# TonyLianLong/LLM-groundedDiffusion

Measured on AMD Instinct MI355X. Metric: images/sec (50-step SD1.5 512^2, LMD+ guidance), higher is better.
Workload: dtype fp16; 1 GPU; LMD+ stage 2, 4 cached 2-box layouts/GPU/step (lmd_v0.1 cache), 50 DDIM steps, 512x512, sd14_gligen (SD1.4+GLIGEN architecture, seeded random weights), VAE decodes included; per-box masks = box masks; mask_refinement=box, layouts_per_gpu=4, num_inference_steps=50, parallelism=dp1, rccl_ranks=1, lanes_per_gpu=4, gemm_tuning=throughput

## Files before the change

include/lgd_hip.h:

```cpp
#ifndef LGD_HIP_H
#define LGD_HIP_H
#include <stdint.h>
#ifdef __cplusplus
extern "C" {
#endif

#define LGD_ABI_VERSION 12
int lgd_abi_version(void);
int lgd_set_option(const char* name, int value);
int lgd_get_option(const char* name);

#define LGD_EPI_GEGLU 1
#define LGD_EPI_OUT_F32 2
#define LGD_EPI_RES_F32 4
#define LGD_EPI_ROWNORM 8

typedef struct LgdGemmDesc {
  const void* a0;
  const void* a1;
  int64_t lda0, lda1;
  int32_t c0, c1;
  int32_t taps;
  int32_t hin, win, hout, wout, stride, ups;
  const void* w;
  int64_t ldw;
  int32_t M, N, K;
  int32_t nb_o, nb_i;
  int64_t a_bs_o, a_bs_i, w_bs_o, w_bs_i, c_bs_o, c_bs_i, r_bs_o, r_bs_i;
  const float* bias;
  const float* bias2;
  const void* res;
  int64_t ldr;
  float alpha;
  int32_t epi;
  void* c;
  int64_t ldc;
  int32_t splits;
  float* ws;
  int32_t tile;
  int32_t* cnt;
  const float* rowstat;
  const float* colsum;
  int32_t pair;
} LgdGemmDesc;
#define LGD_PAIR_HALF 1
#define LGD_PAIR_DUP 2

int lgd_gemm_f16(const LgdGemmDesc* desc , void* stream);
int lgd_gemm_check(const LgdGemmDesc* desc );

int lgd_conv_in_f16(const float* x_nchw, const void* w, const float* bias, void* y, int B, int Cin,
                    int L, int Cout, void* stream);
int lgd_conv_out_f16(const void* x, const void* w, const float* bias, float* y_nchw, int B, int Cin,
                     int L, int Cout, float out_scale, void* stream);

int lgd_groupnorm_f16(const void* x0, const void* x1, int c0, int c1, int B, int HW, int G,
                      float eps, const float* gamma, const float* beta, int silu, void* y,
                      float* part, int nchunk, float* stats, void* stream);
int lgd_groupnorm_pair_f16(const void* x0, const void* x1, int c0, int c1, int B, int HW, int G,
                           float eps, const float* gamma, const float* beta, int silu, void* y,
                           float* part, int nchunk, int pair, void* stream);
int lgd_groupnorm_bwd_f16(const void* gy, const void* x0, const void* x1, int c0, int c1, int B,
                          int HW, int G, const float* gamma, const float* beta, int silu,
                          const float* stats, void* gx0, void* gx1, float* part, int nchunk,
                          int accumulate, void* stream);

int lgd_layernorm_f16(const void* x, int64_t ldx, void* y, int64_t ldy, int rows, int C, float eps,
                      const float* gamma, const float* beta, float* stats, int rows_per_batch,
                      int64_t x_bs, int64_t y_bs, void* stream);
int lgd_layernorm_pair_f16(const void* x, int64_t ldx, void* y, int64_t ldy, int rows, int C, float eps,
                           const float* gamma, const float* beta, float* stats, int rows_per_batch,
                           int64_t x_bs, int64_t y_bs, int pair, void* stream);
int lgd_layernorm_bwd_f16(const void* gy, int64_t ldgy, const void* x, int64_t ldx, void* gx,
                          int64_t ldgx, int rows, int C, const float* gamma, const float* stats,
                          int rows_per_batch, int64_t gy_bs, int64_t x_bs, int64_t gx_bs,
                          int accumulate, void* stream);

int lgd_attn_fwd_f16(const void* q, int64_t ldq, int64_t q_bs, const void* k, int64_t ldk,
                     int64_t k_bs, const void* v, int64_t ldv, int64_t v_bs, void* o, int64_t ldo,
                     int64_t o_bs, float* lse, int B, int H, int Sq, int Sk, int d, float scale,
                     void* stream);
int lgd_attn_fwd_pair_f16(const void* q, int64_t ldq, int64_t q_bs, const void* k, int64_t ldk,
                          int64_t k_bs, const void* v, int64_t ldv, int64_t v_bs, void* o, int64_t ldo,
                          int64_t o_bs, float* lse, int B, int H, int Sq, int Sk, int d, float scale,
                          int pair, void* stream);
int lgd_attn_bwd_f16(const void* q, int64_t ldq, int64_t q_bs, const void* k, int64_t ldk,
                     int64_t k_bs, const void* v, int64_t ldv, int64_t v_bs, const void* o,
                     int64_t ldo, int64_t o_bs, const void* go, int64_t ldgo, int64_t go_bs,
                     const float* lse, float* delta, void* gq, int64_t ldgq, int64_t gq_bs, void* gk,
                     int64_t ldgk, int64_t gk_bs, void* gv, int64_t ldgv, int64_t gv_bs, int B, int H,
                     int Sq, int Sk, int d, float scale, void* stream);
int lgd_attn_bwd_keys_f16(const void* q, int64_t ldq, int64_t q_bs, const void* k, int64_t ldk,
                          int64_t k_bs, const void* v, int64_t ldv, int64_t v_bs, const void* o,
                          int64_t ldo, int64_t o_bs, const void* go, int64_t ldgo, int64_t go_bs,
                          const float* lse, float* delta, void* gq, int64_t ldgq, int64_t gq_bs, void* gk,
                          int64_t ldgk, int64_t gk_bs, void* gv, int64_t ldgv, int64_t gv_bs, int B, int H,
                          int Sq, int Sk, int Sk_grad, int d, float scale, void* stream);

int lgd_cross_attn_fwd_f16(const void* q, int64_t ldq, int64_t q_bs, const void* k, int64_t ldk,
                           int64_t k_bs, const void* v, int64_t ldv, int64_t v_bs, void* o,
                           int64_t ldo, int64_t o_bs, float* probs, int tok, int cond_only, int B,
                           int H, int Sq, int Sk, int d, float scale, void* stream);
int lgd_cross_attn_bwd_f16(const void* q, int64_t ldq, int64_t q_bs, const void* k, int64_t ldk,
                           int64_t k_bs, const void* v, int64_t ldv, int64_t v_bs, const void* go,
                           int64_t ldgo, int64_t go_bs, const float* gp, void* gq, int64_t ldgq,
                           int64_t gq_bs, int B, int H, int Sq, int Sk, int d, float scale,
                           void* stream);

int lgd_attn_causal_fwd_f16(const void* q, int64_t ldq, int64_t q_bs, const void* k, int64_t ldk, int64_t k_bs,
                            const void* v, int64_t ldv, int64_t v_bs, void* o, int64_t ldo, int64_t o_bs, int B,
                            int H, int S, int d, float scale, void* stream);

#define LGD_ATTN_OP_FWD 0
#define LGD_ATTN_OP_BWD 1
#define LGD_ATTN_OP_CROSS_BWD 2
int lgd_attn_plan(int op, int B, int H, int Sq, int Sk, int Sk_grad, int d, int probs, int causal, int pair,
                  int aligned);

int lgd_geglu_bwd_f16(const void* h, const void* gy, void* gh, int64_t rows, int n, void* stream);
int lgd_geglu_fwd_f16(const void* h, void* y, int64_t rows, int n, void* stream);
int lgd_quick_gelu_f16(const void* x, void* y, int64_t n, void* stream);
int lgd_nchw_to_nhwc8_f16(const float* x, void* y, int B, int C, int HW, void* stream);
int lgd_add_f16(const void* a, const void* b, void* y, int64_t n, void* stream);
int lgd_scale_f16(const void* x, void* y, float alpha, int64_t n, void* stream);
int lgd_image_u8_to_nhwc8_f16(const void* img, const float* table, void* y, int B, int HW, void* stream);
int lgd_vae_sample_f32(const void* moments, const float* noise, float* out, int B, int z, int HW, float scale,
                       void* stream);
int lgd_softmax_rows_f16(const void* x, void* y, int64_t rows, int n, float scale, void* stream);
int lgd_upsample2x_bwd_f16(const void* gy, void* gx, int B, int H, int W, int C, void* stream);

int lgd_cfg_ddim_step_f32(const float* eps, const float* x, float* x_out, const float* coef_table,
                          const int32_t* dyn, const float* frozen_ref, const float* mask, float* hist,
                          int B, int C, int HW, void* stream);
int lgd_cfg_multistep_step_f32(const float* eps, const float* x, float* x_out, float* x0_prev,
                               const float* coef_table, const int32_t* dyn, const float* frozen_ref,
                               const float* mask, float* hist, int B, int C, int HW, void* stream);
int lgd_cfg_plms_step_f32(const float* eps, const float* x, float* x_out, float* ets, float* cur_sample,
                          const float* coef_table, const int32_t* dyn, float* hist, int B, int C, int HW, void* stream);
int lgd_multidiffusion_step_f32(const float* eps, float* x_in, float* latent, const float* masks, const float* bg,
                                const float* noise, const int32_t* picks, const float* coef_table, const int32_t* dyn,
                                float* hist, int P, int Pp, int C, int HW, int n_steps, int n_boot, int prep,
                                void* stream);
int lgd_multidiffusion_views_f32(const float* eps, float* x_in, float* latent, float* value, float* count,
                                 const float* masks, const float* bg, const float* noise, const int32_t* picks,
                                 const float* coef_table, const int32_t* dyn, float* hist, int P, int Pp, int C, int Hp,
                                 int Wp, int V, int v0, int nv, int nvc, int n_steps, int n_boot, int indep_uncond,
                                 int normalization, int prep, void* stream);
int lgd_scale_rows_f32(const float* x, float* out, const float* table, const int32_t* dyn, int row_stride, int col,
                       int64_t n, int reps, void* stream);
int lgd_axpy_f32(const float* g, float* x, const float* coef_table, const int32_t* step_idx, int col,
                 const float* active, int64_t per_sample, int64_t n, void* stream);
int lgd_select_row_f32(const float* table, const int32_t* idx, float* out, int n, void* stream);

#define LGD_ACT_GELU 1
#define LGD_ACT_RELU 2
int lgd_act_f16(const void* x, void* y, int64_t n, int mode, void* stream);
int lgd_sam_relpos_qkv_f16(const void* qkv, const float* qkv_bias, const float* rel_h, const float* rel_w, int B,
                           int Hs, int Ws, int window, int NH, int d, int DA, float scale, void* qa, void* ka,
                           void* va, void* stream);
int lgd_sam_window_merge_f16(const void* oa, void* out, int B, int Hs, int Ws, int window, int NH, int d, int DA,
                             void* stream);

int lgd_ca_energy_f32(const float* const* maps, float* const* gmaps, const int32_t* map_hw,
                      const int32_t* items, const float* coefs, const float* masks, const float* refs,
                      int64_t refs_step_stride, const int32_t* dyn, const int32_t* groups, int n_groups,
                      int n_items, int n_samples, int H, int T, int max_hw, float grad_scale, float* partial,
                      float* loss, void* stream);

int lgd_boxdiff_energy_f32(const float* const* maps, float* const* gmaps, int n_maps, int side, const int32_t* items,
                           const float* masks, const float* smooth, const int32_t* groups, int n_samples,
                           int max_items, int H, int T, float loss_scale, float grad_scale, float* loss, void* stream);

#ifdef __cplusplus
}
#endif
#endif
```

llm-groundeddiffusion_amd/_lib.py:

```python
import ctypes as C
import os

import torch

_HERE = os.path.dirname(os.path.abspath(__file__))
LIB_PATH = os.path.join(_HERE, "liblgd_hip.so")
ABI_VERSION = 12

c_void_p, c_int, c_i64, c_float = C.c_void_p, C.c_int, C.c_int64, C.c_float


class LgdGemmDesc(C.Structure):
    _fields_ = [
        ("a0", c_void_p), ("a1", c_void_p),
        ("lda0", c_i64), ("lda1", c_i64),
        ("c0", C.c_int32), ("c1", C.c_int32),
        ("taps", C.c_int32),
        ("hin", C.c_int32), ("win", C.c_int32), ("hout", C.c_int32), ("wout", C.c_int32),
        ("stride", C.c_int32), ("ups", C.c_int32),
        ("w", c_void_p), ("ldw", c_i64),
        ("M", C.c_int32), ("N", C.c_int32), ("K", C.c_int32),
        ("nb_o", C.c_int32), ("nb_i", C.c_int32),
        ("a_bs_o", c_i64), ("a_bs_i", c_i64), ("w_bs_o", c_i64), ("w_bs_i", c_i64),
        ("c_bs_o", c_i64), ("c_bs_i", c_i64), ("r_bs_o", c_i64), ("r_bs_i", c_i64),
        ("bias", c_void_p), ("bias2", c_void_p),
        ("res", c_void_p), ("ldr", c_i64),
        ("alpha", c_float), ("epi", C.c_int32),
        ("c", c_void_p), ("ldc", c_i64),
        ("splits", C.c_int32), ("ws", c_void_p),
        ("tile", C.c_int32),
        ("cnt", c_void_p),
        ("rowstat", c_void_p), ("colsum", c_void_p),
        ("pair", C.c_int32),
    ]


EPI_GEGLU, EPI_OUT_F32, EPI_RES_F32, EPI_ROWNORM = 1, 2, 4, 8
PAIR_HALF, PAIR_DUP = 1, 2

_P, _I, _L, _F = c_void_p, c_int, c_i64, c_float
SIGNATURES = {
    "lgd_abi_version": [],
    "lgd_set_option": [C.c_char_p, _I],
    "lgd_get_option": [C.c_char_p],
    "lgd_gemm_f16": [C.POINTER(LgdGemmDesc), _P],
    "lgd_gemm_check": [C.POINTER(LgdGemmDesc)],
    "lgd_conv_in_f16": [_P, _P, _P, _P, _I, _I, _I, _I, _P],
    "lgd_conv_out_f16": [_P, _P, _P, _P, _I, _I, _I, _I, _F, _P],
    "lgd_groupnorm_f16": [_P, _P, _I, _I, _I, _I, _I, _F, _P, _P, _I, _P, _P, _I, _P, _P],
    "lgd_groupnorm_pair_f16": [_P, _P, _I, _I, _I, _I, _I, _F, _P, _P, _I, _P, _P, _I, _I, _P],
    "lgd_groupnorm_bwd_f16": [_P, _P, _P, _I, _I, _I, _I, _I, _P, _P, _I, _P, _P, _P, _P, _I, _I, _P],
    "lgd_layernorm_f16": [_P, _L, _P, _L, _I, _I, _F, _P, _P, _P, _I, _L, _L, _P],
    "lgd_layernorm_pair_f16": [_P, _L, _P, _L, _I, _I, _F, _P, _P, _P, _I, _L, _L, _I, _P],
    "lgd_layernorm_bwd_f16": [_P, _L, _P, _L, _P, _L, _I, _I, _P, _P, _I, _L, _L, _L, _I, _P],
    "lgd_attn_fwd_f16": [_P, _L, _L, _P, _L, _L, _P, _L, _L, _P, _L, _L, _P, _I, _I, _I, _I, _I, _F, _P],
    "lgd_attn_fwd_pair_f16": [_P, _L, _L, _P, _L, _L, _P, _L, _L, _P, _L, _L, _P, _I, _I, _I, _I, _I, _F, _I, _P],
    "lgd_attn_bwd_f16": [_P, _L, _L, _P, _L, _L, _P, _L, _L, _P, _L, _L, _P, _L, _L, _P, _P,
                         _P, _L, _L, _P, _L, _L, _P, _L, _L, _I, _I, _I, _I, _I, _F, _P],
    "lgd_attn_bwd_keys_f16": [_P, _L, _L, _P, _L, _L, _P, _L, _L, _P, _L, _L, _P, _L, _L, _P, _P,
                              _P, _L, _L, _P, _L, _L, _P, _L, _L, _I, _I, _I, _I, _I, _I, _F, _P],
    "lgd_cross_attn_fwd_f16": [_P, _L, _L, _P, _L, _L, _P, _L, _L, _P, _L, _L, _P, _I, _I,
                               _I, _I, _I, _I, _I, _F, _P],
    "lgd_cross_attn_bwd_f16": [_P, _L, _L, _P, _L, _L, _P, _L, _L, _P, _L, _L, _P, _P, _L, _L,
                               _I, _I, _I, _I, _I, _F, _P],
    "lgd_geglu_bwd_f16": [_P, _P, _P, _L, _I, _P],
    "lgd_geglu_fwd_f16": [_P, _P, _L, _I, _P],
    "lgd_add_f16": [_P, _P, _P, _L, _P],
    "lgd_softmax_rows_f16": [_P, _P, _L, _I, _F, _P],
    "lgd_scale_f16": [_P, _P, _F, _L, _P],
    "lgd_upsample2x_bwd_f16": [_P, _P, _I, _I, _I, _I, _P],
    "lgd_cfg_ddim_step_f32": [_P, _P, _P, _P, _P, _P, _P, _P, _I, _I, _I, _P],
    "lgd_cfg_multistep_step_f32": [_P, _P, _P, _P, _P, _P, _P, _P, _P, _I, _I, _I, _P],
    "lgd_cfg_plms_step_f32": [_P, _P, _P, _P, _P, _P, _P, _P, _I, _I, _I, _P],
    "lgd_multidiffusion_step_f32": [_P, _P, _P, _P, _P, _P, _P, _P, _P, _P, _I, _I, _I, _I, _I, _I, _I, _P],
    "lgd_multidiffusion_views_f32": [_P] * 12 + [_I] * 14 + [_P],
    "lgd_axpy_f32": [_P, _P, _P, _P, _I, _P, _L, _L, _P],
    "lgd_select_row_f32": [_P, _P, _P, _I, _P],
    "lgd_scale_rows_f32": [_P, _P, _P, _P, _I, _I, _L, _I, _P],
    "lgd_attn_causal_fwd_f16": [_P, _L, _L, _P, _L, _L, _P, _L, _L, _P, _L, _L, _I, _I, _I, _I, _F, _P],
    "lgd_attn_plan": [_I] * 11,
    "lgd_quick_gelu_f16": [_P, _P, _L, _P],
    "lgd_act_f16": [_P, _P, _L, _I, _P],
    "lgd_nchw_to_nhwc8_f16": [_P, _P, _I, _I, _I, _P],
    "lgd_image_u8_to_nhwc8_f16": [_P, _P, _P, _I, _I, _P],
    "lgd_vae_sample_f32": [_P, _P, _P, _I, _I, _I, _F, _P],
    "lgd_sam_relpos_qkv_f16": [_P, _P, _P, _P, _I, _I, _I, _I, _I, _I, _I, _F, _P, _P, _P, _P],
    "lgd_sam_window_merge_f16": [_P, _P, _I, _I, _I, _I, _I, _I, _I, _P],
    "lgd_ca_energy_f32": [_P, _P, _P, _P, _P, _P, _P, _L, _P, _P, _I, _I, _I, _I, _I, _I, _F, _P, _P, _P],
    "lgd_boxdiff_energy_f32": [_P, _P, _I, _I, _P, _P, _P, _P, _I, _I, _I, _I, _F, _F, _P, _P],
}

_lib = None


def load():
    global _lib
    if _lib is not None:
        return _lib
    if not os.path.exists(LIB_PATH):
        raise RuntimeError(
            f"{LIB_PATH} not found: build it with `python __graft_entry__.py` "
            "(there is no CPU/PyTorch fallback for the HIP kernels)")
    lib = C.CDLL(LIB_PATH)
    for name, argtypes in SIGNATURES.items():
        try:
            fn = getattr(lib, name)
        except AttributeError as e:
            raise RuntimeError(f"liblgd_hip.so does not export {name}") from e
        fn.argtypes = argtypes
        fn.restype = c_int
    if lib.lgd_abi_version() != ABI_VERSION:
        raise RuntimeError("liblgd_hip.so ABI version mismatch; rebuild")
    for item in filter(None, os.environ.get("LGD_OPTIONS", "").split(",")):
        name, _, value = item.partition("=")
        check(lib.lgd_set_option(name.strip().encode(), int(value)), f"lgd_set_option({name})")
    _lib = lib
    return lib


_ERR = {-1: "invalid argument", -2: "kernel launch failed", -3: "unsupported shape"}


def check(rc, name):
    if rc != 0:
        raise RuntimeError(f"{name} failed: {_ERR.get(rc, rc)}")
```

llm-groundeddiffusion_amd/csrc/attn.hip:

```cpp
#include <atomic>
#include "common.h"
#include "../../include/lgd_hip.h"
#include "attn_w4.h"
#include "attn_plan.h"
#include <stdlib.h>
#include <string.h>

namespace {

int g_attn32_nw = -1;
int attn32_nw() {
  if (g_attn32_nw < 0) { const char* e = getenv("LGD_ATTN32_NW"); g_attn32_nw = e ? atoi(e) : 8; }
  return g_attn32_nw;
}
int g_attn32_var = 0;
int attn32_var() { return g_attn32_var; }
int g_attn32 = -1;
int attn32_mode() {
  if (g_attn32 < 0) { const char* e = getenv("LGD_ATTN32"); g_attn32 = e ? atoi(e) : 1; }
  return g_attn32;
}

std::atomic<int> g_attn_w4{-1};
int attn_w4_mode() {
// ... 830 lines not shown
    for (int dt = 0; dt < NDT; ++dt)
#pragma unroll
      for (int r = 0; r < 16; ++r)
        if (dt == dt_l && r == r_l) lv = oacc[dt][r];
    l = __shfl(lv, h_l * 32 + qi, 64);
  }
  const int qrow = q0 + qi;
  if (qrow < a.Sq) {
    const float inv = 1.f / l;
    half_t* orow = a.o + (long)b * a.o_bs + (long)qrow * a.ldo + (long)h * d;
#pragma unroll
    for (int dt = 0; dt < NDT; ++dt)
#pragma unroll
      for (int g4 = 0; g4 < 4; ++g4) {
        const int dv = dt * 32 + g4 * 8 + hh * 4;
        if (dv < d) {
          half4_t o;
#pragma unroll
          for (int r = 0; r < 4; ++r) o[r] = (half_t)(oacc[dt][g4 * 4 + r] * inv);
          *reinterpret_cast<half4_t*>(orow + dv) = o;
          if (a.o_dup) *reinterpret_cast<half4_t*>(orow + a.o_dup + dv) = o;
        }
      }
    if (a.lse && hh == 0) {
      float* lp = a.lse + ((long)b * a.H + h) * a.Sq + qrow;
      const float lv2 = m_ref + log2f(l);
      *lp = lv2;
      if (a.lse_dup) lp[a.lse_dup] = lv2;
    }
  }
}

int attn_nw_env() {
  static const int nw_env = [] { const char* e = getenv("LGD_ATTN_NW"); return e ? atoi(e) : 0; }();
  return nw_env;
}
int attn160_wide_env() {
  static const int wide = [] { const char* e = getenv("LGD_ATTN160"); return e ? atoi(e) : 1; }();
  return wide;
}

int attn_dp_of(int d) { return d <= 32 ? 32 : d <= 64 ? 64 : d <= 96 ? 96 : d <= 128 ? 128 : d <= 160 ? 160 : d <= 192 ? 192 : 0; }

int plan_fwd(int B, int H, int Sq, int Sk, int d, bool two_pass) {
  const int DP = attn_dp_of(d);
  if (!DP) return LGD_ERR_UNSUPPORTED;
  if (two_pass) return attn_code(ATTN_FAM_TWOPASS, DP, 0);
  const long blocks256 = (long)((Sq + 255) / 256) * H * B;
  const int w4 = attn_w4_mode();
  if (w4 && d == 40 && (w4 == 2 || (blocks256 >= 256 && Sk >= 256)))
    return attn_code(ATTN_FAM_W4, 64, lgd_attn_w4_pipe() ? 1 : 0);
  if (DP == 64 || DP == 96) {
    const int a32 = attn32_mode();
    const int dk = ((d + 2 + 15) / 16) * 16;
    if (a32 && d % 8 == 0 && (a32 == 2 || (dk == 96 && blocks256 >= 128)) && (dk == 48 || dk == 96)) {
      const int var = attn32_var();
      const int sub = (attn32_nw() == 4 || (a32 != 2 && blocks256 < 256)) ? ATTN32_NW4
                      : var == 1 ? ATTN32_NW8_PF4 : var == 2 ? ATTN32_NW8_FREE : ATTN32_NW8;
      return attn_code(ATTN_FAM_SELF32, dk, sub);
    }
  }
  const int mode = (DP == 64 && d < 48) ? SELF_ONES3 : d < DP ? SELF_ONES : SELF_PLAIN;
  const bool qt2 = (long)((Sq + 127) / 128) * H * B >= 1024 && DP <= 96;
  if (qt2) {
    const int nw_env = attn_nw_env();
    const bool nw8 = nw_env ? nw_env == 8 : ((DP == 64 && d < 48) || DP == 96);
    return attn_code(ATTN_FAM_SELF, DP, 10 * mode + (nw8 && blocks256 >= 512 ? SELF_QT2_NW8 : SELF_QT2));
  }
  if (DP == 160 && attn160_wide_env() && d == DP && Sq >= 256 && (long)H * B * ((Sq + 63) / 64) > 256)
    return attn_code(ATTN_FAM_SELF, DP, 10 * SELF_PLAIN + SELF_QT2_NW8);
  return attn_code(ATTN_FAM_SELF, DP, 10 * mode + SELF_QT1);
}

template <int DP, bool ONES, int NDT>
void launch_self_shape(int shape, const AttnArgs& a, hipStream_t st) {
  const int gz = a.pair ? a.B / 2 : a.B;
  if constexpr (DP <= 96 || (DP == 160 && !ONES)) {
    if (shape == SELF_QT2_NW8) {
      hipLaunchKernelGGL((attn_self_kernel<DP, ONES, 2, NDT, 8>), dim3((a.Sq + 255) / 256, a.H, gz), dim3(512), 0, st, a);
      return;
    }
  }
  if constexpr (DP <= 96) {
    if (shape == SELF_QT2) {
      hipLaunchKernelGGL((attn_self_kernel<DP, ONES, 2, NDT>), dim3((a.Sq + 127) / 128, a.H, gz), dim3(256), 0, st, a);
      return;
    }
  }
  hipLaunchKernelGGL((attn_self_kernel<DP, ONES, 1, NDT>), dim3((a.Sq + 63) / 64, a.H, gz), dim3(256), 0, st, a);
}

template <int DP>
void launch_fwd_code(int code, const AttnArgs& a, hipStream_t st) {
  const int fam = attn_code_fam(code), sub = attn_code_sub(code);
  if (fam == ATTN_FAM_TWOPASS) {
    dim3 grid((a.Sq + 63) / 64, a.H, a.B);
    hipLaunchKernelGGL((attn_fwd_kernel<DP>), grid, dim3(256), 0, st, a);
    return;
  }
  if constexpr (DP == 64 || DP == 96) {
    if (fam == ATTN_FAM_SELF32) {
      constexpr int DK = DP == 64 ? 48 : 96, NDT = DP == 64 ? 2 : 3;
      const int gz = a.pair ? a.B / 2 : a.B;
      auto go = [&](auto kern, int nw) {
        dim3 g32((a.Sq + 32 * nw - 1) / (32 * nw), a.H, gz);
        hipLaunchKernelGGL(kern, g32, dim3(64 * nw), 0, st, a);
      };
      switch (sub) {
        case ATTN32_NW4: go(&attn_self32_kernel<DK, NDT, 4>, 4); return;
        case ATTN32_NW8_PF4: go(&attn_self32_kernel<DK, NDT, 8, 4, true>, 8); return;
        case ATTN32_NW8_FREE: go(&attn_self32_kernel<DK, NDT, 8, 2, false>, 8); return;
        default: go(&attn_self32_kernel<DK, NDT, 8>, 8); return;
      }
    }
  }
  const int mode = sub / 10, shape = sub % 10;
  if constexpr (DP == 64) {
    if (mode == SELF_ONES3) return launch_self_shape<DP, true, 3>(shape, a, st);
  }
  if (mode == SELF_PLAIN) launch_self_shape<DP, false, DP / 16>(shape, a, st);
  else launch_self_shape<DP, true, DP / 16>(shape, a, st);
}

int launch_attn(const AttnArgs& a, hipStream_t st, bool two_pass) {
  AttnW4Args w;
  w.q = a.q; w.ldq = a.ldq; w.q_bs = a.q_bs; w.k = a.k; w.ldk = a.ldk; w.k_bs = a.k_bs;
  w.v = a.v; w.ldv = a.ldv; w.v_bs = a.v_bs; w.o = a.o; w.ldo = a.ldo; w.o_bs = a.o_bs; w.lse = a.lse;
  w.B = a.B; w.H = a.H; w.Sq = a.Sq; w.Sk = a.Sk; w.d = a.d; w.scale_log2 = a.scale_log2;
  w.pair = a.pair; w.o_dup = a.o_dup; w.lse_dup = a.lse_dup;
  const int code = plan_fwd(a.B, a.H, a.Sq, a.Sk, a.d, two_pass);
  if (code < 0) return code;
  if (attn_code_fam(code) == ATTN_FAM_W4) return lgd_attn_w4_launch(w, st, attn_code_sub(code));
  switch (attn_dp_of(a.d)) {
    case 32: launch_fwd_code<32>(code, a, st); break;
    case 64: launch_fwd_code<64>(code, a, st); break;
    case 96: launch_fwd_code<96>(code, a, st); break;
    case 128: launch_fwd_code<128>(code, a, st); break;
    case 160: launch_fwd_code<160>(code, a, st); break;
    default: launch_fwd_code<192>(code, a, st); break;
  }
  return lgd_check_launch();
}

bool bad_view(const void* p, int64_t ld, int64_t bs, int d) {
  return (ld % 8) != 0 || (d % 8) != 0 || (bs % 8) != 0 || (reinterpret_cast<uintptr_t>(p) & 15) != 0;
}
bool bad_out(const void* p, int64_t ld, int64_t bs) {
  return (ld % 4) != 0 || (bs % 4) != 0 || (reinterpret_cast<uintptr_t>(p) & 7) != 0;
}

}

void lgd_gn_set_fused_hw(int hw);
void lgd_gn_set_slab(int on);
void lgd_ln_set_stream(int on);
void lgd_gn_set_apply_wgs(int n);

static std::atomic<int> g_cfg_pair{1};

extern "C" int lgd_get_option(const char* name) {
  if (name && !strcmp(name, "cfg_pair")) return g_cfg_pair.load(std::memory_order_relaxed);
  return LGD_ERR_ARG;
}

extern "C" int lgd_set_option(const char* name, int value) {
  if (!name) return LGD_ERR_ARG;
  if (!strcmp(name, "cfg_pair") && (value == 0 || value == 1)) { g_cfg_pair.store(value, std::memory_order_relaxed); return LGD_OK; }
  if (!strcmp(name, "gn_fused") && value >= 0 && value <= 4096) { lgd_gn_set_fused_hw(value); return LGD_OK; }
  if (!strcmp(name, "gn_slab") && (value == 0 || value == 1)) { lgd_gn_set_slab(value); return LGD_OK; }
  if (!strcmp(name, "ln_stream") && (value == 0 || value == 1)) { lgd_ln_set_stream(value); return LGD_OK; }
  if (!strcmp(name, "gn_apply_wgs") && value >= 64 && value <= 8192) { lgd_gn_set_apply_wgs(value); return LGD_OK; }
  if (!strcmp(name, "attn32")) { g_attn32 = value; return LGD_OK; }
  if (!strcmp(name, "attn_w4") && value >= 0 && value <= 2) { g_attn_w4.store(value, std::memory_order_relaxed); return LGD_OK; }
  if (!strcmp(name, "attn_w4_pipe") && (value == 0 || value == 1)) { lgd_attn_w4_set_pipe(value); return LGD_OK; }
  if (!strcmp(name, "attn32_nw") && (value == 4 || value == 8)) { g_attn32_nw = value; return LGD_OK; }
  if (!strcmp(name, "attn32_var") && value >= 0 && value <= 2) { g_attn32_var = value; return LGD_OK; }
  return LGD_ERR_ARG;
}

extern "C" int lgd_attn_fwd_f16(const void* q, int64_t ldq, int64_t q_bs, const void* k,
                                int64_t ldk, int64_t k_bs, const void* v, int64_t ldv, int64_t v_bs,
                                void* o, int64_t ldo, int64_t o_bs, float* lse, int B, int H, int Sq,
                                int Sk, int d, float scale, void* stream) {
  if (B < 1 || H < 1 || Sq < 1 || Sk < 1 || d < 8) return LGD_ERR_ARG;
  if (!attn_dp_of(d)) return LGD_ERR_UNSUPPORTED;
  if (bad_view(q, ldq, q_bs, d) || bad_view(k, ldk, k_bs, d) || bad_view(v, ldv, v_bs, d) || bad_out(o, ldo, o_bs)) return LGD_ERR_ARG;
  (void)hipGetLastError();
  AttnArgs a;
  a.q = (const half_t*)q; a.ldq = ldq; a.q_bs = q_bs;
  a.k = (const half_t*)k; a.ldk = ldk; a.k_bs = k_bs;
  a.v = (const half_t*)v; a.ldv = ldv; a.v_bs = v_bs;
  a.o = (half_t*)o; a.ldo = ldo; a.o_bs = o_bs;
  a.lse = lse; a.probs = nullptr; a.tok = -1; a.cond_only = 0; a.causal = 0;
  a.pair = 0; a.o_dup = 0; a.lse_dup = 0;
  a.B = B; a.H = H; a.Sq = Sq; a.Sk = Sk; a.d = d;
  a.scale_log2 = scale * 1.4426950408889634f;
  return launch_attn(a, reinterpret_cast<hipStream_t>(stream), false);
}

extern "C" int lgd_attn_fwd_pair_f16(const void* q, int64_t ldq, int64_t q_bs, const void* k,
                                     int64_t ldk, int64_t k_bs, const void* v, int64_t ldv, int64_t v_bs,
                                     void* o, int64_t ldo, int64_t o_bs, float* lse, int B, int H, int Sq,
                                     int Sk, int d, float scale, int pair, void* stream) {
  if (B < 2 || (B % 2) || H < 1 || Sq < 1 || Sk < 1 || d < 8) return LGD_ERR_ARG;
  if (pair != LGD_PAIR_HALF && pair != LGD_PAIR_DUP) return LGD_ERR_ARG;
  if (!attn_dp_of(d)) return LGD_ERR_UNSUPPORTED;
  if (bad_view(q, ldq, q_bs, d) || bad_view(k, ldk, k_bs, d) || bad_view(v, ldv, v_bs, d) || bad_out(o, ldo, o_bs)) return LGD_ERR_ARG;
  (void)hipGetLastError();
  AttnArgs a;
  a.q = (const half_t*)q; a.ldq = ldq; a.q_bs = q_bs;
  a.k = (const half_t*)k; a.ldk = ldk; a.k_bs = k_bs;
  a.v = (const half_t*)v; a.ldv = ldv; a.v_bs = v_bs;
  a.o = (half_t*)o; a.ldo = ldo; a.o_bs = o_bs;
  a.lse = lse; a.probs = nullptr; a.tok = -1; a.cond_only = 0; a.causal = 0;
  a.pair = pair;
  a.o_dup = pair == LGD_PAIR_DUP ? (long)(B / 2) * o_bs : 0;
  a.lse_dup = pair == LGD_PAIR_DUP ? (long)(B / 2) * H * Sq : 0;
  a.B = B; a.H = H; a.Sq = Sq; a.Sk = Sk; a.d = d;
  a.scale_log2 = scale * 1.4426950408889634f;
  return launch_attn(a, reinterpret_cast<hipStream_t>(stream), false);
}

extern "C" int lgd_cross_attn_fwd_f16(const void* q, int64_t ldq, int64_t q_bs, const void* k,
                                      int64_t ldk, int64_t k_bs, const void* v, int64_t ldv,
                                      int64_t v_bs, void* o, int64_t ldo, int64_t o_bs, float* probs,
                                      int tok, int cond_only, int B, int H, int Sq, int Sk, int d,
                                      float scale, void* stream) {
  if (B < 1 || H < 1 || Sq < 1 || Sk < 1 || d < 8) return LGD_ERR_ARG;
  if (!attn_dp_of(d)) return LGD_ERR_UNSUPPORTED;
  if (bad_view(q, ldq, q_bs, d) || bad_view(k, ldk, k_bs, d) || bad_view(v, ldv, v_bs, d) || bad_out(o, ldo, o_bs)) return LGD_ERR_ARG;
  if (cond_only && (B % 2)) return LGD_ERR_ARG;
  if (tok >= Sk) return LGD_ERR_ARG;
  (void)hipGetLastError();
  AttnArgs a;
  a.q = (const half_t*)q; a.ldq = ldq; a.q_bs = q_bs;
  a.k = (const half_t*)k; a.ldk = ldk; a.k_bs = k_bs;
  a.v = (const half_t*)v; a.ldv = ldv; a.v_bs = v_bs;
  a.o = (half_t*)o; a.ldo = ldo; a.o_bs = o_bs;
  a.lse = nullptr; a.probs = probs; a.tok = tok; a.cond_only = cond_only; a.causal = 0;
  a.pair = 0; a.o_dup = 0; a.lse_dup = 0;
  a.B = B; a.H = H; a.Sq = Sq; a.Sk = Sk; a.d = d;
  a.scale_log2 = scale * 1.4426950408889634f;
  hipStream_t st = reinterpret_cast<hipStream_t>(stream);
  return launch_attn(a, st, probs != nullptr);
}

extern "C" int lgd_attn_causal_fwd_f16(const void* q, int64_t ldq, int64_t q_bs, const void* k, int64_t ldk,
                                       int64_t k_bs, const void* v, int64_t ldv, int64_t v_bs, void* o,
                                       int64_t ldo, int64_t o_bs, int B, int H, int S, int d, float scale,
                                       void* stream) {
  if (B < 1 || H < 1 || S < 1 || d < 8) return LGD_ERR_ARG;
  if (!attn_dp_of(d)) return LGD_ERR_UNSUPPORTED;
  if (bad_view(q, ldq, q_bs, d) || bad_view(k, ldk, k_bs, d) || bad_view(v, ldv, v_bs, d) || bad_out(o, ldo, o_bs)) return LGD_ERR_ARG;
  (void)hipGetLastError();
  AttnArgs a;
  a.q = (const half_t*)q; a.ldq = ldq; a.q_bs = q_bs;
  a.k = (const half_t*)k; a.ldk = ldk; a.k_bs = k_bs;
  a.v = (const half_t*)v; a.ldv = ldv; a.v_bs = v_bs;
  a.o = (half_t*)o; a.ldo = ldo; a.o_bs = o_bs;
  a.lse = nullptr; a.probs = nullptr; a.tok = -1; a.cond_only = 0; a.causal = 1;
  a.pair = 0; a.o_dup = 0; a.lse_dup = 0;
  a.B = B; a.H = H; a.Sq = S; a.Sk = S; a.d = d;
  a.scale_log2 = scale * 1.4426950408889634f;
  return launch_attn(a, reinterpret_cast<hipStream_t>(stream), true);
}

extern "C" int lgd_attn_plan(int op, int B, int H, int Sq, int Sk, int Sk_grad, int d, int probs, int causal, int pair,
                             int aligned) {
  if (B < 1 || H < 1 || Sq < 1 || Sk < 1 || d < 8 || (d % 8)) return LGD_ERR_ARG;
  if (pair && (pair != LGD_PAIR_HALF && pair != LGD_PAIR_DUP)) return LGD_ERR_ARG;
  switch (op) {
    case LGD_ATTN_OP_FWD:
      if (causal && Sq != Sk) return LGD_ERR_ARG;
      if (pair && ((B % 2) || probs || causal)) return LGD_ERR_ARG;
      return plan_fwd(B, H, Sq, Sk, d, probs || causal);
    case LGD_ATTN_OP_BWD:
      if (Sk_grad < 1 || Sk_grad > Sk || probs || causal || pair) return LGD_ERR_ARG;
      return lgd_attn_bwd_plan(B, H, Sq, Sk, d);
    case LGD_ATTN_OP_CROSS_BWD:
      if (causal || pair) return LGD_ERR_ARG;
      return lgd_cross_attn_bwd_plan(Sk, d, aligned);
    default:
      return LGD_ERR_ARG;
  }
}
```

llm-groundeddiffusion_amd/csrc/gemm.hip:

```cpp
#include "common.h"
#include "../../include/lgd_hip.h"
#include <map>
#include <mutex>
#include <utility>
#include <stdlib.h>

namespace {

constexpr int BK = 64;
constexpr int LDS_LD = BK + 16;

struct GemmArgs {
  LgdGemmDesc d;
  int cin;
  int k_per_split;
  int group_m;
  long c_dup;
#ifdef LGD_GEMM_ABLATION
  int stagger;
#endif
};

__device__ __forceinline__ float4 ld_bias4(const float* p, int n) {
  return *reinterpret_cast<const float4*>(p + n);
}

__device__ __forceinline__ f32x4 rownorm4(const LgdGemmDesc& d, int m, int n_in, f32x4 v) {
  if (d.epi & LGD_EPI_ROWNORM) {
    const float2 st = *reinterpret_cast<const float2*>(d.rowstat + (long)m * 2);
    const float4 cs = *reinterpret_cast<const float4*>(d.colsum + n_in);
    v[0] = st.y * (v[0] - st.x * cs.x); v[1] = st.y * (v[1] - st.x * cs.y);
    v[2] = st.y * (v[2] - st.x * cs.z); v[3] = st.y * (v[3] - st.x * cs.w);
  }
  return v;
}

template <bool GEGLU>
__device__ __forceinline__ f32x4 epilogue_value4(const LgdGemmDesc& d, long r_off, int m, int n_out, f32x4 v, f32x4 g,
                                                 float4 bv, float4 bg, bool res_ready, half4_t res_pre) {
  v[0] += bv.x; v[1] += bv.y; v[2] += bv.z; v[3] += bv.w;
  if (GEGLU) {
    g[0] += bg.x; g[1] += bg.y; g[2] += bg.z; g[3] += bg.w;
#ifdef LGD_GEMM_ABLATION
    if (d.epi & (1 << 16)) {
#pragma unroll
      for (int r = 0; r < 4; ++r) v[r] = v[r] * g[r];
    } else
#endif
    {
      const f32x2_t g01 = gelu2_f((f32x2_t){g[0], g[1]}), g23 = gelu2_f((f32x2_t){g[2], g[3]});
      v[0] *= g01[0]; v[1] *= g01[1]; v[2] *= g23[0]; v[3] *= g23[1];
    }
  }
  const float alpha = d.alpha;
#pragma unroll
  for (int r = 0; r < 4; ++r) v[r] *= alpha;
  if (res_ready) {
#pragma unroll
    for (int r = 0; r < 4; ++r) v[r] += (float)res_pre[r];
  } else if (d.res) {
    if (d.epi & LGD_EPI_RES_F32) {
      const float* rp = reinterpret_cast<const float*>(d.res) + r_off + (long)m * d.ldr + n_out;
      float4 rv = *reinterpret_cast<const float4*>(rp);
      v[0] += rv.x; v[1] += rv.y; v[2] += rv.z; v[3] += rv.w;
    } else {
      const half_t* rp = reinterpret_cast<const half_t*>(d.res) + r_off + (long)m * d.ldr + n_out;
      half4_t rv = *reinterpret_cast<const half4_t*>(rp);
#pragma unroll
      for (int r = 0; r < 4; ++r) v[r] += (float)rv[r];
    }
  }
  return v;
}

template <bool GEGLU>
__device__ __forceinline__ void epilogue_store4(const LgdGemmDesc& d, long c_off, long r_off, int m,
                                                int n_out, f32x4 v, f32x4 g, float4 bv, float4 bg,
                                                bool res_ready = false,
                                                half4_t res_pre = (half4_t){0, 0, 0, 0}, long c_dup = 0) {
  v = epilogue_value4<GEGLU>(d, r_off, m, n_out, v, g, bv, bg, res_ready, res_pre);
  if (d.epi & LGD_EPI_OUT_F32) {
    float* cp = reinterpret_cast<float*>(d.c) + c_off + (long)m * d.ldc + n_out;
    *reinterpret_cast<float4*>(cp) = make_float4(v[0], v[1], v[2], v[3]);
    if (c_dup) *reinterpret_cast<float4*>(cp + c_dup) = make_float4(v[0], v[1], v[2], v[3]);
  } else {
    half_t* cp = reinterpret_cast<half_t*>(d.c) + c_off + (long)m * d.ldc + n_out;
    half4_t o;
#pragma unroll
    for (int r = 0; r < 4; ++r) o[r] = (half_t)v[r];
    *reinterpret_cast<half4_t*>(cp) = o;
    if (c_dup) *reinterpret_cast<half4_t*>(cp + c_dup) = o;
  }
}

__device__ __forceinline__ float4 ld_bias_sum4(const LgdGemmDesc& d, int n) {
  float4 b = make_float4(0.f, 0.f, 0.f, 0.f);
  if (d.bias) b = ld_bias4(d.bias, n);
  if (d.bias2) {
    float4 b2 = ld_bias4(d.bias2, n);
    b.x += b2.x; b.y += b2.y; b.z += b2.z; b.w += b2.w;
  }
  return b;
}

template <int MI, int NI>
__device__ __forceinline__ void gemm_epilogue(const GemmArgs& ga, f32x4 (&acc)[NI][MI], int m0, int n0,
                                              int wm, int wn, int lane, int batch, int split,
                                              long c_off, long r_off, int* lds_flag = nullptr) {
  const LgdGemmDesc& d = ga.d;
  const int m_l = lane & 15;
  const int n_l = (lane >> 4) * 4;
  if (d.splits > 1) {
    float* ws = ga.d.ws + ((long)batch * d.splits + split) * (long)d.M * d.N;
#pragma unroll
    for (int mi = 0; mi < MI; ++mi) {
      int m = m0 + wm * 16 * MI + mi * 16 + m_l;
      if (m >= d.M) continue;
#pragma unroll
      for (int ni = 0; ni < NI; ++ni) {
        int n = n0 + wn * 16 * NI + ni * 16 + n_l;
        if (n >= d.N) continue;
        f32x4 v = acc[ni][mi];
        *reinterpret_cast<float4*>(ws + (long)m * d.N + n) = make_float4(v[0], v[1], v[2], v[3]);
      }
    }
    if (!d.cnt || !lds_flag) return;
    asm volatile("s_waitcnt vmcnt(0)" ::: "memory");
    __syncthreads();
    int32_t* cnt = d.cnt + (long)batch * gridDim.x + blockIdx.x;
    if (threadIdx.x == 0) {
      __builtin_amdgcn_fence(__ATOMIC_RELEASE, "agent");
      asm volatile("s_waitcnt vmcnt(0)" ::: "memory");
      *lds_flag = __hip_atomic_fetch_add(cnt, 1, __ATOMIC_RELAXED, __HIP_MEMORY_SCOPE_AGENT);
    }
    __syncthreads();
    if (*lds_flag != d.splits - 1) return;
    if (threadIdx.x == 0) {
      __builtin_amdgcn_fence(__ATOMIC_ACQUIRE, "agent");
      __hip_atomic_store(cnt, 0, __ATOMIC_RELAXED, __HIP_MEMORY_SCOPE_AGENT);
    }
    __syncthreads();
    const float* w0 = ga.d.ws + (long)batch * d.splits * (long)d.M * d.N;
#pragma unroll
    for (int mi = 0; mi < MI; ++mi) {
      const int m = m0 + wm * 16 * MI + mi * 16 + m_l;
#pragma unroll
      for (int ni = 0; ni < NI; ++ni) {
        const int n = n0 + wn * 16 * NI + ni * 16 + n_l;
        f32x4 v = {0.f, 0.f, 0.f, 0.f};
        if (m < d.M && n < d.N) {
          for (int s2 = 0; s2 < d.splits; ++s2) {
            const float4 t = *reinterpret_cast<const float4*>(w0 + (long)s2 * d.M * d.N + (long)m * d.N + n);
            v[0] += t.x; v[1] += t.y; v[2] += t.z; v[3] += t.w;
          }
        }
        acc[ni][mi] = v;
      }
    }
  }
  const bool geglu = d.epi & LGD_EPI_GEGLU;
  if (geglu) {
    if constexpr (NI % 2 == 0) {
#pragma unroll
      for (int ni = 0; ni < NI; ni += 2) {
        const int n_in = n0 + wn * 16 * NI + ni * 16 + n_l;
        if (n_in >= d.N) continue;
        const int n_out = (n0 + wn * 16 * NI + ni * 16) / 2 + n_l;
        const float4 bv = ld_bias_sum4(d, n_in);
        float4 bg = make_float4(0.f, 0.f, 0.f, 0.f);
        if (d.bias) bg = ld_bias4(d.bias, n_in + 16);
#pragma unroll
        for (int mi = 0; mi < MI; ++mi) {
          const int m = m0 + wm * 16 * MI + mi * 16 + m_l;
          if (m < d.M)
            epilogue_store4<true>(d, c_off, r_off, m, n_out, rownorm4(d, m, n_in, acc[ni][mi]),
                                  rownorm4(d, m, n_in + 16, acc[ni + 1][mi]), bv, bg, false, (half4_t){0, 0, 0, 0}, ga.c_dup);
        }
      }
    }
    return;
  }
  const bool res16 = d.res && !(d.epi & LGD_EPI_RES_F32);
  constexpr int NCH = NI <= 5 ? NI : (NI % 5 == 0 ? 5 : 4);
  static_assert(NI % NCH == 0, "NI must split into equal prefetch rounds");
#pragma unroll
  for (int nc = 0; nc < NI; nc += NCH) {
    half4_t rpre[NCH][MI];
    if (res16) {
      const half_t* rb = reinterpret_cast<const half_t*>(d.res) + r_off;
#pragma unroll
      for (int nj = 0; nj < NCH; ++nj) {
        int n = n0 + wn * 16 * NI + (nc + nj) * 16 + n_l;
        if (n >= d.N) n = 0;
#pragma unroll
        for (int mi = 0; mi < MI; ++mi) {
          int m = m0 + wm * 16 * MI + mi * 16 + m_l;
          if (m >= d.M) m = d.M - 1;
          rpre[nj][mi] = *reinterpret_cast<const half4_t*>(rb + (long)m * d.ldr + n);
        }
      }
    }
#pragma unroll
    for (int nj = 0; nj < NCH; ++nj) {
      const int ni = nc + nj;
      const int n = n0 + wn * 16 * NI + ni * 16 + n_l;
      if (n >= d.N) continue;
      const float4 bv = ld_bias_sum4(d, n);
#pragma unroll
      for (int mi = 0; mi < MI; ++mi) {
        const int m = m0 + wm * 16 * MI + mi * 16 + m_l;
        if (m < d.M)
          epilogue_store4<false>(d, c_off, r_off, m, n, rownorm4(d, m, n, acc[ni][mi]), acc[ni][mi], bv, bv, res16,
                                 res16 ? rpre[nj][mi] : (half4_t){0, 0, 0, 0}, ga.c_dup);
      }
    }
  }
}

template <int MI, int NI, int WM, int WN, int STAGE_B, bool GEGLU, bool RES_PREFETCH>
__device__ __forceinline__ void gemm_epilogue_lds_generic(const GemmArgs& ga, f32x4 (&acc)[NI][MI], int m0, int n0, int wm,
                                                  int wn, int lane, int tid, long c_off, long r_off,
                                                  unsigned char* lds) {
  const LgdGemmDesc& d = ga.d;
  constexpr int NT = 64 * WM * WN;
  constexpr int BM = WM * 16 * MI, BN = WN * 16 * NI;
  constexpr int BN_OUT = GEGLU ? BN / 2 : BN;
  constexpr int NI_OUT = GEGLU ? NI / 2 : NI;
  constexpr int CROW = BN_OUT * 2 + 16;
  constexpr int R = (BM * CROW <= STAGE_B) ? 1 : ((BM / 2) * CROW <= STAGE_B) ? 2 : 4;
  static_assert(MI % R == 0 && (BM / R) * CROW <= STAGE_B, "staged rows must fit one ring stage");
  constexpr int MI_R = MI / R;
  constexpr int WROWS = 16 * MI_R;
  constexpr int RROWS = WM * WROWS;
  constexpr int CPR = BN_OUT / 8;
  const int m_l = lane & 15, n_l = (lane >> 4) * 4;
  const int n0_out = GEGLU ? n0 / 2 : n0;
  const int n_total_out = GEGLU ? d.N / 2 : d.N;
  const bool res16 = d.res && !(d.epi & LGD_EPI_RES_F32);
  half_t* cbase = reinterpret_cast<half_t*>(d.c) + c_off;
  float4 bv[NI_OUT], bg[NI_OUT];
  const bool rn = d.epi & LGD_EPI_ROWNORM;
  float4 cv[NI_OUT], cg[NI_OUT];
  float2 st[MI];
#pragma unroll
  for (int no = 0; no < NI_OUT; ++no) {
    const int n_out = n0_out + wn * 16 * NI_OUT + no * 16 + n_l;
    const int n_in = GEGLU ? n0 + wn * 16 * NI + no * 32 + n_l : n_out;
    bv[no] = make_float4(0.f, 0.f, 0.f, 0.f);
    bg[no] = bv[no];
    cv[no] = bv[no];
    cg[no] = bv[no];
#ifdef LGD_GEMM_ABLATION
    if (d.epi & (1 << 18)) continue;
#endif
    if (n_out < n_total_out) {
// ... 1181 lines not shown
#pragma unroll
      for (int i = 0; i < MH; ++i) af[kk][i] = (half8_t){1, 1, 1, 1, 1, 1, 1, 1};
#pragma unroll
      for (int i = 0; i < NI0; ++i) bf0[kk][i] = (half8_t){1, 1, 1, 1, 1, 1, 1, 1};
#pragma unroll
      for (int i = 0; i < NI1; ++i) bf1[kk][i] = (half8_t){1, 1, 1, 1, 1, 1, 1, 1};
    }
  }

#define LGD_PH_MMA(BF, NB, NOFF, MOFF)                                                                              \
  {                                                                                                                 \
    asm volatile("s_waitcnt lgkmcnt(0)" ::: "memory");                                                              \
    __builtin_amdgcn_sched_barrier(0);                                                                              \
    if constexpr (!(ABL & 32)) __builtin_amdgcn_s_setprio(1);                                                       \
    _Pragma("unroll") for (int kk = 0; kk < 2; ++kk)                                                                \
      _Pragma("unroll") for (int ni = 0; ni < NB; ++ni)                                                             \
        _Pragma("unroll") for (int mi = 0; mi < MH; ++mi)                                                           \
          if constexpr (ABL & 4) asm volatile("" : "+v"(acc[NOFF + ni][MOFF + mi]) : "v"(BF[kk][ni]), "v"(af[kk][mi]));                \
          else acc[NOFF + ni][MOFF + mi] = __builtin_amdgcn_mfma_f32_16x16x32_f16(BF[kk][ni], af[kk][mi], acc[NOFF + ni][MOFF + mi], 0, 0, 0); \
    if constexpr (!(ABL & 32)) __builtin_amdgcn_s_setprio(0);                                                       \
    __builtin_amdgcn_sched_barrier(0);                                                                              \
  }
#define LGD_PH_BAR()                        \
  {                                         \
    __builtin_amdgcn_sched_barrier(0);      \
    __builtin_amdgcn_s_barrier();           \
    __builtin_amdgcn_sched_barrier(0);      \
  }

  if (nk > 0) {
    {
      unsigned sa, sw; int tap;
      k_pos(0, sa, sw, tap);
      dma_b(0, 0, true, sw, false);
      dma_a(0, 0, true, sa, tap, false);
      dma_b(1, 0, true, sw, false);
      dma_a(1, 0, true, sa, tap, false);
      k_pos(1, sa, sw, tap);
      dma_b(0, STAGE_B, nk > 1, sw, false);
      dma_a(0, STAGE_B, nk > 1, sa, tap, false);
    }
#pragma unroll
    for (int ni = 0; ni < NI; ++ni)
#pragma unroll
      for (int mi = 0; mi < MI; ++mi) acc[ni][mi] = (f32x4){0.f, 0.f, 0.f, 0.f};
    asm volatile("s_waitcnt vmcnt(%0)" ::"n"(T_DMA) : "memory");
    LGD_PH_BAR();
    if (grp == 1 && !(ABL & 64)) LGD_PH_BAR();
    unsigned so_cur = 0, so_nxt = STAGE_B;
    int sdelta = STAGE_B;
    for (int kt = 0; kt < nk; ++kt) {
      unsigned sa1, sw1, sa2, sw2; int tap1, tap2;
      k_pos(kt + 1, sa1, sw1, tap1);
      k_pos(kt + 2, sa2, sw2, tap2);
      const bool live1 = kt + 1 < nk, live2 = kt + 2 < nk;
      if constexpr (!(ABL & 2)) lds_read_frags<0, 64 * 128>(bf0[0], b_ad0, seqB0{});
      if constexpr (!(ABL & 2)) lds_read_frags<0, 64 * 128>(bf0[1], b_ad1, seqB0{});
      if constexpr (!(ABL & 2)) lds_read_frags<0, 16 * 128>(af[0], a_ad0, seqA{});
      if constexpr (!(ABL & 2)) lds_read_frags<0, 16 * 128>(af[1], a_ad1, seqA{});
      dma_b(1, so_nxt, live1, sw1);
      asm volatile("s_waitcnt vmcnt(%0)" ::"n"(T_DMA) : "memory");
      LGD_PH_BAR();
      LGD_PH_MMA(bf0, NI0, 0, 0);
      LGD_PH_BAR();
      if constexpr (!(ABL & 2)) lds_read_frags<BQ0_B, 64 * 128>(bf1[0], b_ad0, seqB1{});
      if constexpr (!(ABL & 2)) lds_read_frags<BQ0_B, 64 * 128>(bf1[1], b_ad1, seqB1{});
      dma_a(1, so_nxt, live1, sa1, tap1);
      asm volatile("s_waitcnt vmcnt(%0)" ::"n"(T_DMA) : "memory");
      LGD_PH_BAR();
      LGD_PH_MMA(bf1, NI1, NI0, 0);
      LGD_PH_BAR();
      if constexpr (!(ABL & 2)) lds_read_frags<OFF_A1, 16 * 128>(af[0], a_ad0, seqA{});
      if constexpr (!(ABL & 2)) lds_read_frags<OFF_A1, 16 * 128>(af[1], a_ad1, seqA{});
      dma_b(0, so_cur, live2, sw2);
      LGD_PH_BAR();
      LGD_PH_MMA(bf1, NI1, NI0, MH);
      LGD_PH_BAR();
      dma_a(0, so_cur, live2, sa2, tap2);
      asm volatile("s_waitcnt vmcnt(%0)" ::"n"(T_DMA) : "memory");
      LGD_PH_BAR();
      LGD_PH_MMA(bf0, NI0, 0, MH);
      LGD_PH_BAR();
      a_ad0 += sdelta; a_ad1 += sdelta; b_ad0 += sdelta; b_ad1 += sdelta;
      sdelta = -sdelta;
      const unsigned t = so_cur; so_cur = so_nxt; so_nxt = t;
    }
    if (grp == 0 && !(ABL & 64)) LGD_PH_BAR();
    asm volatile("s_waitcnt vmcnt(0) lgkmcnt(0)" ::: "memory");
    LGD_PH_BAR();
  }
  else {
#pragma unroll
    for (int ni = 0; ni < NI; ++ni)
#pragma unroll
      for (int mi = 0; mi < MI; ++mi) acc[ni][mi] = (f32x4){0.f, 0.f, 0.f, 0.f};
  }
#undef LGD_PH_MMA
#undef LGD_PH_BAR

  if constexpr (ABL & 16) {
#pragma unroll
    for (int ni = 0; ni < NI; ++ni)
#pragma unroll
      for (int mi = 0; mi < MI; ++mi) asm volatile("" ::"v"(acc[ni][mi]));
    return;
  }
  if (d.splits > 1) {
    const int m_l = lane & 15, n_l = (lane >> 4) * 4;
    float* ws = d.ws + ((long)batch * d.splits + split) * (long)d.M * d.N;
#pragma unroll
    for (int mi = 0; mi < MI; ++mi) {
      const int m = m0 + grp * 16 * MI + mi * 16 + m_l;
      if (m >= d.M) continue;
#pragma unroll
      for (int ni = 0; ni < NI; ++ni) {
        const int n = n0 + wn * 16 * NI + ni * 16 + n_l;
        if (n >= d.N) continue;
        const f32x4 v = acc[ni][mi];
        *reinterpret_cast<float4*>(ws + (long)m * d.N + n) = make_float4(v[0], v[1], v[2], v[3]);
      }
    }
    return;
  }
#define LGD_EPI_LDS(G, RS, RNORM) \
  gemm_epilogue_lds<MI, NI, WM, WN, (MI * NI > 32 ? STAGE_B : 2 * STAGE_B), G, true, RS, RNORM>(ga, acc, m0, n0, grp, wn, lane, tid, c_off, r_off, lds)
  const bool rn_ = d.epi & LGD_EPI_ROWNORM;
  if (d.epi & LGD_EPI_GEGLU) {
    if constexpr (NI % 2 == 0) {
      if (rn_) LGD_EPI_LDS(true, false, true); else LGD_EPI_LDS(true, false, false);
    }
  } else if (d.res) {
    if (rn_) LGD_EPI_LDS(false, true, true); else LGD_EPI_LDS(false, true, false);
  } else {
    if (rn_) LGD_EPI_LDS(false, false, true); else LGD_EPI_LDS(false, false, false);
  }
#undef LGD_EPI_LDS
}

__global__ __launch_bounds__(256) void splitk_reduce_kernel(const GemmArgs ga) {
  const LgdGemmDesc& d = ga.d;
  const bool geglu = d.epi & LGD_EPI_GEGLU;
  const int n_out_cols = geglu ? d.N / 2 : d.N;
  const long groups_per_row = n_out_cols / 4;
  const long total = (long)d.M * groups_per_row;
  const int batch = blockIdx.z;
  const int b_o = batch / d.nb_i, b_i = batch - b_o * d.nb_i;
  const long c_off = b_o * d.c_bs_o + b_i * d.c_bs_i;
  const long r_off = b_o * d.r_bs_o + b_i * d.r_bs_i;
  const float* ws = d.ws + (long)batch * d.splits * (long)d.M * d.N;
  for (long idx = blockIdx.x * 256L + threadIdx.x; idx < total; idx += (long)gridDim.x * 256L) {
    int m = (int)(idx / groups_per_row);
    int gcol = (int)(idx - (long)m * groups_per_row) * 4;
    int n_in = geglu ? (gcol / 16) * 32 + (gcol % 16) : gcol;
    f32x4 v = {0.f, 0.f, 0.f, 0.f}, g = {0.f, 0.f, 0.f, 0.f};
    for (int s = 0; s < d.splits; ++s) {
      const float* p = ws + (long)s * d.M * d.N + (long)m * d.N + n_in;
      float4 t = *reinterpret_cast<const float4*>(p);
      v[0] += t.x; v[1] += t.y; v[2] += t.z; v[3] += t.w;
      if (geglu) {
        float4 u = *reinterpret_cast<const float4*>(p + 16);
        g[0] += u.x; g[1] += u.y; g[2] += u.z; g[3] += u.w;
      }
    }
    const float4 bv = ld_bias_sum4(d, n_in);
    v = rownorm4(d, m, n_in, v);
    if (geglu) {
      float4 bg = make_float4(0.f, 0.f, 0.f, 0.f);
      if (d.bias) bg = ld_bias4(d.bias, n_in + 16);
      epilogue_store4<true>(d, c_off, r_off, m, gcol, v, rownorm4(d, m, n_in + 16, g), bv, bg);
    } else {
      epilogue_store4<false>(d, c_off, r_off, m, gcol, v, g, bv, bv);
    }
  }
}

enum GemmLoop : int {
  LOOP_REG,
  LOOP_DMA,
  LOOP_DMA8,
  LOOP_PIPE,
  LOOP_PHASE,
};
enum : unsigned {
  TILE_GEGLU = 1,
  TILE_PLAIN = 2,
  TILE_ONE_SPLIT = 4,
  TILE_LDS_EPI = 8,
  TILE_CONV_SAME = 16,
  TILE_CNT = 32,
};
struct GemmTile {
  int code;
  GemmLoop loop;
  int bm, bn;
  unsigned flags;
};
constexpr unsigned TILE_STD = TILE_GEGLU | TILE_CNT;
constexpr GemmTile GEMM_TILES[] = {
    {1, LOOP_REG, 128, 128, TILE_STD},   {2, LOOP_REG, 128, 64, TILE_STD},     {3, LOOP_REG, 64, 128, TILE_STD},
    {4, LOOP_REG, 64, 64, TILE_STD},     {5, LOOP_REG, 32, 128, TILE_STD},     {6, LOOP_REG, 128, 160, TILE_CNT},
    {7, LOOP_REG, 64, 160, TILE_CNT},
    {17, LOOP_DMA, 128, 128, TILE_STD},  {18, LOOP_DMA, 128, 64, TILE_STD},    {19, LOOP_DMA, 64, 128, TILE_STD},
    {20, LOOP_DMA, 64, 64, TILE_STD},    {21, LOOP_DMA, 32, 128, TILE_STD},    {22, LOOP_DMA, 128, 160, TILE_CNT},
    {23, LOOP_DMA, 64, 160, TILE_CNT},
    {25, LOOP_DMA8, 256, 320, TILE_CNT}, {26, LOOP_DMA8, 256, 128, TILE_STD},
    {33, LOOP_PIPE, 256, 160, TILE_CNT}, {34, LOOP_PIPE, 256, 128, TILE_STD}, {35, LOOP_PIPE, 256, 64, TILE_STD},
    {37, LOOP_PIPE, 128, 160, TILE_CNT}, {38, LOOP_PIPE, 128, 128, TILE_STD}, {39, LOOP_PIPE, 128, 64, TILE_STD},
    {40, LOOP_PIPE, 64, 160, TILE_CNT},  {41, LOOP_PIPE, 64, 128, TILE_STD},  {42, LOOP_PIPE, 64, 64, TILE_STD},
    {44, LOOP_PIPE, 256, 256, TILE_GEGLU | TILE_PLAIN | TILE_ONE_SPLIT | TILE_LDS_EPI},
    {45, LOOP_PIPE, 128, 128, TILE_STD | TILE_PLAIN},
    {46, LOOP_PHASE, 256, 256, TILE_GEGLU | TILE_LDS_EPI | TILE_CONV_SAME},
    {47, LOOP_PHASE, 256, 320, TILE_LDS_EPI | TILE_CONV_SAME},
};

const GemmTile* gemm_check(const LgdGemmDesc& desc, GemmArgs& ga) {
  ga.d = desc;
  LgdGemmDesc& d = ga.d;
  if (d.M <= 0 || d.N <= 0 || d.K <= 0) return nullptr;
  if (d.taps != 1 && d.taps != 9) return nullptr;
  ga.cin = d.c0 + d.c1;
  if (d.K != d.taps * ga.cin) return nullptr;
  if ((d.c0 % 8) || (d.c1 % 8) || (d.N % 4) || (d.ldw % 8) || (d.lda0 % 8) || (d.lda1 % 8) ||
      (d.ldc % 4))
    return nullptr;
  if (d.c1 > 0 && !d.a1) return nullptr;
  if (d.res && (d.ldr % 4)) return nullptr;
  if (d.nb_o < 1) d.nb_o = 1;
  if (d.nb_i < 1) d.nb_i = 1;
  if (d.splits < 1) d.splits = 1;
  const bool geglu = d.epi & LGD_EPI_GEGLU;
  if (geglu && (d.N % 32)) return nullptr;
  if (d.splits > 1 && !d.ws) return nullptr;
  if ((d.epi & LGD_EPI_ROWNORM) && (!d.rowstat || !d.colsum || d.taps != 1 || d.nb_o * d.nb_i != 1 || d.c1 > 0))
    return nullptr;
  int ktiles = (d.K + BK - 1) / BK;
  int tps = (ktiles + d.splits - 1) / d.splits;
  ga.k_per_split = tps * BK;
  d.splits = (ktiles + tps - 1) / tps;

  int code = d.tile;
  if (code == 0) {
    long batches = (long)d.nb_o * d.nb_i * d.splits;
    auto wgs = [&](int bm, int bn) {
      return batches * ((d.M + bm - 1) / bm) * ((d.N + bn - 1) / bn);
    };
    if (d.M <= 32) code = 21;
    else if (!geglu && d.N % 160 == 0 && wgs(128, 160) >= 384) code = 22;
    else if (!geglu && d.N % 160 == 0 && wgs(64, 160) >= 256) code = 23;
    else if (wgs(128, 128) >= 384 && d.N % 128 == 0) code = 17;
    else if (wgs(64, 128) >= 256 && d.N % 128 == 0) code = 19;
    else code = 20;
  }
  const GemmTile* t = nullptr;
  for (const GemmTile& e : GEMM_TILES)
    if (e.code == code) t = &e;
  if (!t) return nullptr;
  const unsigned f = t->flags;
  if (geglu && !(f & TILE_GEGLU)) return nullptr;
  if (t->loop == LOOP_DMA8 && (d.K % BK)) return nullptr;
  if ((t->loop == LOOP_PIPE || t->loop == LOOP_PHASE) && ((d.K % BK) || (ga.cin % BK) || (d.c0 % BK))) return nullptr;
  if ((f & TILE_PLAIN) && (d.taps != 1 || d.c1 > 0)) return nullptr;
  if (t->loop == LOOP_PHASE) {
    if (d.c1 > 0 || d.nb_o * d.nb_i != 1) return nullptr;
    if (((long)d.M + 2L * d.win + 2) * d.lda0 * 2 + 2L * d.K >= (1L << 31) || (long)d.N * d.ldw * 2 >= (1L << 31))
      return nullptr;
  }
  if ((f & TILE_CONV_SAME) && d.taps == 9 && (d.stride != 1 || d.ups != 0 || d.hin != d.hout || d.win != d.wout))
    return nullptr;
  if ((f & TILE_ONE_SPLIT) && d.splits != 1) return nullptr;
  if ((f & TILE_LDS_EPI) && d.splits == 1) {
    const long c_off_max = (long)(d.nb_o - 1) * d.c_bs_o + (long)(d.nb_i - 1) * d.c_bs_i;
    if ((d.epi & LGD_EPI_OUT_F32) || (d.N & 7) || (d.ldc & 7) || (c_off_max & 7) || (d.c_bs_o & 7) || (d.c_bs_i & 7) ||
        (reinterpret_cast<uintptr_t>(d.c) & 15) || (d.res && (d.epi & (LGD_EPI_RES_F32 | LGD_EPI_GEGLU))))
      return nullptr;
  }
  if (d.splits > 1 && d.cnt && !(f & TILE_CNT)) return nullptr;
  ga.c_dup = 0;
  if (d.pair) {
    if ((d.pair != LGD_PAIR_HALF && d.pair != LGD_PAIR_DUP) || d.splits != 1 || d.nb_o * d.nb_i != 1 || (d.M & 1))
      return nullptr;
    d.M /= 2;
    if (d.pair == LGD_PAIR_DUP) {
      ga.c_dup = (long)d.M * d.ldc;
      if ((f & TILE_LDS_EPI) && (ga.c_dup & 7)) return nullptr;
    }
  }
  return t;
}

using GemmKernel = void (*)(GemmArgs);

int lds_kernel(GemmKernel kern, int smem, int threads, long* resident = nullptr) {
  static std::mutex mu;
  static std::map<std::pair<GemmKernel, int>, long> ready;
  int dev = 0;
  if (hipGetDevice(&dev) != hipSuccess) return LGD_ERR_LAUNCH;
  std::lock_guard<std::mutex> lock(mu);
  auto it = ready.find({kern, dev});
  if (it == ready.end()) {
    if (hipFuncSetAttribute(reinterpret_cast<const void*>(kern), hipFuncAttributeMaxDynamicSharedMemorySize, smem) !=
        hipSuccess)
      return LGD_ERR_LAUNCH;
    it = ready.emplace(std::make_pair(kern, dev), -1L).first;
  }
  if (resident) {
    if (it->second < 0) {
      int per_cu = 0, cus = 0;
      if (hipDeviceGetAttribute(&cus, hipDeviceAttributeMultiprocessorCount, dev) != hipSuccess ||
          hipOccupancyMaxActiveBlocksPerMultiprocessor(&per_cu, reinterpret_cast<const void*>(kern), threads, smem) !=
              hipSuccess)
        return LGD_ERR_LAUNCH;
      it->second = (long)(cus / 8) * 8 * (per_cu > 0 ? per_cu : 1);
    }
    *resident = it->second;
  }
  return LGD_OK;
}

template <int MI, int NI, int WM = 2>
int launch_gemm(const GemmArgs& ga, hipStream_t st, bool dma) {
  constexpr int BM = WM * 16 * MI, BN = 32 * NI;
  const LgdGemmDesc& d = ga.d;
  long tiles = (long)((d.M + BM - 1) / BM) * ((d.N + BN - 1) / BN);
  dim3 grid((unsigned)tiles, 1, (unsigned)(d.nb_o * d.nb_i * d.splits));
  if constexpr (WM == 2) {
    if (dma) hipLaunchKernelGGL((gemm_dma_kernel<MI, NI, 2>), grid, dim3(256), 0, st, ga);
    else hipLaunchKernelGGL((gemm_kernel<MI, NI>), grid, dim3(256), 0, st, ga);
  } else {
    hipLaunchKernelGGL((gemm_dma_kernel<MI, NI, WM>), grid, dim3(128 * WM), 0, st, ga);
  }
  return lgd_check_launch();
}

template <int MI, int NI, int WM, int WN, int NS, bool CM>
int launch_gemm_pipe_cm(const GemmArgs& ga, hipStream_t st) {
  constexpr int BM = WM * 16 * MI, BN = WN * 16 * NI;
  constexpr int SMEM = NS * (BM + BN) * BK * 2;
  constexpr int THREADS = 64 * WM * WN;
  constexpr bool HAS_PERSIST = !CM && !(MI == 4 && NI == 5) && NS != 2;
  const LgdGemmDesc& d = ga.d;
  long tiles = (long)((d.M + BM - 1) / BM) * ((d.N + BN - 1) / BN);
  GemmKernel kern = &gemm_pipe_kernel<MI, NI, WM, WN, NS, CM>;
  long resident = 0;
  if constexpr (HAS_PERSIST) {
    static const bool persist_on = [] { const char* e = getenv("LGD_GEMM_PERSIST"); return !(e && e[0] == '0'); }();
    if (persist_on)
      if (int rc = lds_kernel(&gemm_pipe_kernel<MI, NI, WM, WN, NS, false, true>, SMEM, THREADS, &resident)) return rc;
  }
  const bool persist = resident > 0 && d.nb_o * d.nb_i * d.splits == 1 && tiles > resident && d.K <= 10 * BK && d.taps == 1;
  dim3 grid((unsigned)(persist ? resident : tiles), 1, (unsigned)(d.nb_o * d.nb_i * d.splits));
  if constexpr (HAS_PERSIST)
    if (persist) kern = &gemm_pipe_kernel<MI, NI, WM, WN, NS, false, true>;
#ifdef LGD_GEMM_ABLATION
  static const int abl = [] { const char* e = getenv("LGD_GEMM_ABL"); return e ? atoi(e) : 0; }();
  if (abl) {
    switch (abl) {
      case 1: kern = &gemm_pipe_kernel<MI, NI, WM, WN, NS, CM, false, 1>; break;
      case 2: kern = &gemm_pipe_kernel<MI, NI, WM, WN, NS, CM, false, 2>; break;
      case 3: kern = &gemm_pipe_kernel<MI, NI, WM, WN, NS, CM, false, 3>; break;
      case 4: kern = &gemm_pipe_kernel<MI, NI, WM, WN, NS, CM, false, 4>; break;
      case 6: kern = &gemm_pipe_kernel<MI, NI, WM, WN, NS, CM, false, 6>; break;
      case 8: kern = &gemm_pipe_kernel<MI, NI, WM, WN, NS, CM, false, 8>; break;
      case 11: kern = &gemm_pipe_kernel<MI, NI, WM, WN, NS, CM, false, 11>; break;
      case 16: kern = &gemm_pipe_kernel<MI, NI, WM, WN, NS, CM, false, 16>; break;
      case 17: kern = &gemm_pipe_kernel<MI, NI, WM, WN, NS, CM, false, 17>; break;
      case 20: kern = &gemm_pipe_kernel<MI, NI, WM, WN, NS, CM, false, 20>; break;
      default: return lgd_check_launch();
    }
  }
#endif
  if (int rc = lds_kernel(kern, SMEM, THREADS)) return rc;
  hipLaunchKernelGGL(kern, grid, dim3(THREADS), SMEM, st, ga);
  return lgd_check_launch();
}

template <int MI, int NI, int WM, int WN, int NS>
int launch_gemm_pipe(const GemmArgs& ga, hipStream_t st) {
  const LgdGemmDesc& d = ga.d;
  static const int no_cm = [] { const char* e = getenv("LGD_GEMM_NO_CM"); return (e && e[0] == '1') ? 1 : 0; }();
  if constexpr (NS != 2) {
    if (d.taps == 9 && d.stride == 1 && d.ups == 0 && d.c1 == 0 && !no_cm)
      return launch_gemm_pipe_cm<MI, NI, WM, WN, NS, true>(ga, st);
  }
  return launch_gemm_pipe_cm<MI, NI, WM, WN, NS, false>(ga, st);
}

template <int MI, int NI>
int launch_gemm_phase(const GemmArgs& ga, hipStream_t st) {
  constexpr int BM = 32 * MI, BN = 64 * NI;
  constexpr int SMEM = 2 * (BM + BN) * BK * 2;
  const LgdGemmDesc& d = ga.d;
  const bool conv = d.taps == 9;
  long tiles = (long)((d.M + BM - 1) / BM) * ((d.N + BN - 1) / BN);
  dim3 grid((unsigned)tiles, 1, (unsigned)(d.nb_o * d.nb_i * d.splits));
  GemmKernel kern = conv ? &gemm_phase_kernel<MI, NI, true> : &gemm_phase_kernel<MI, NI, false>;
#ifdef LGD_GEMM_ABLATION
  static const int abl = [] { const char* e = getenv("LGD_GEMM_ABL"); return e ? atoi(e) : 0; }();
  if (abl) {
#define LGD_PH_ABL(A) case A: kern = conv ? &gemm_phase_kernel<MI, NI, true, A> : &gemm_phase_kernel<MI, NI, false, A>; break;
    switch (abl) {
      LGD_PH_ABL(1) LGD_PH_ABL(2) LGD_PH_ABL(3) LGD_PH_ABL(4) LGD_PH_ABL(6) LGD_PH_ABL(16) LGD_PH_ABL(17) LGD_PH_ABL(20) LGD_PH_ABL(32) LGD_PH_ABL(64) LGD_PH_ABL(96)
      default: return lgd_check_launch();
    }
#undef LGD_PH_ABL
  }
#endif
  if (int rc = lds_kernel(kern, SMEM, 512)) return rc;
  hipLaunchKernelGGL(kern, grid, dim3(512), SMEM, st, ga);
  return lgd_check_launch();
}

int launch_tile(const GemmTile& t, const GemmArgs& ga, hipStream_t st) {
  const bool dma = t.loop == LOOP_DMA && ga.d.K % BK == 0;
  switch (t.code) {
    case 33: return launch_gemm_pipe<4, 5, 4, 2, 3>(ga, st);
    case 34: return launch_gemm_pipe<4, 4, 4, 2, 3>(ga, st);
    case 35: return launch_gemm_pipe<4, 2, 4, 2, 4>(ga, st);
    case 37: return launch_gemm_pipe<2, 5, 4, 2, 4>(ga, st);
    case 38: return launch_gemm_pipe<2, 4, 4, 2, 4>(ga, st);
    case 39: return launch_gemm_pipe<2, 2, 4, 2, 5>(ga, st);
    case 40: return launch_gemm_pipe<1, 5, 4, 2, 5>(ga, st);
    case 41: return launch_gemm_pipe<1, 4, 4, 2, 5>(ga, st);
    case 42: return launch_gemm_pipe<1, 2, 4, 2, 6>(ga, st);
    case 44: return launch_gemm_pipe<4, 8, 4, 2, 2>(ga, st);
    case 45: return launch_gemm_pipe<2, 4, 4, 2, 2>(ga, st);
    case 46: return launch_gemm_phase<8, 4>(ga, st);
    case 47: return launch_gemm_phase<8, 5>(ga, st);
    case 1: case 17: return launch_gemm<4, 4>(ga, st, dma);
    case 2: case 18: return launch_gemm<4, 2>(ga, st, dma);
    case 3: case 19: return launch_gemm<2, 4>(ga, st, dma);
    case 4: case 20: return launch_gemm<2, 2>(ga, st, dma);
    case 5: case 21: return launch_gemm<1, 4>(ga, st, dma);
    case 6: case 22: return launch_gemm<4, 5>(ga, st, dma);
    case 7: case 23: return launch_gemm<2, 5>(ga, st, dma);
    case 25: return launch_gemm<4, 10, 4>(ga, st, true);
    case 26: return launch_gemm<4, 4, 4>(ga, st, true);
  }
  return LGD_ERR_ARG;
}

}

extern "C" int lgd_abi_version(void) { return LGD_ABI_VERSION; }

extern "C" int lgd_gemm_check(const LgdGemmDesc* desc) {
  GemmArgs ga;
  return desc && gemm_check(*desc, ga) ? LGD_OK : LGD_ERR_ARG;
}

extern "C" int lgd_gemm_f16(const LgdGemmDesc* desc, void* stream) {
  (void)hipGetLastError();
  GemmArgs ga;
  const GemmTile* t = desc ? gemm_check(*desc, ga) : nullptr;
  if (!t) return LGD_ERR_ARG;
  const LgdGemmDesc& d = ga.d;
  hipStream_t st = reinterpret_cast<hipStream_t>(stream);
#ifdef LGD_GEMM_ABLATION
  { const char* e = getenv("LGD_GEMM_STAGGER"); ga.stagger = e ? atoi(e) : 0; }
#endif
  {
    static const int forced = [] { const char* e = getenv("LGD_GEMM_GROUP_M"); return e ? atoi(e) : 0; }();
    ga.group_m = 1;
    const long w_bytes = (long)d.N * d.K * 2;
    if (d.taps == 1 && d.nb_o * d.nb_i == 1 && w_bytes > (5L << 19)) {
      long g = (3L << 20) / (256L * d.K * 2);
      ga.group_m = forced > 0 ? forced : (int)(g < 1 ? 1 : g > 8 ? 8 : g);
    }
  }
  int rc = launch_tile(*t, ga, st);
  if (rc || d.splits == 1 || d.cnt) return rc;
  int n_out = (d.epi & LGD_EPI_GEGLU) ? d.N / 2 : d.N;
  long total = (long)d.M * (n_out / 4);
  int blocks = (int)((total + 255) / 256);
  if (blocks > 2048) blocks = 2048;
  dim3 grid(blocks, 1, d.nb_o * d.nb_i);
  hipLaunchKernelGGL(splitk_reduce_kernel, grid, dim3(256), 0, st, ga);
  return lgd_check_launch();
}
```

llm-groundeddiffusion_amd/csrc/norm.hip:

```cpp
#include "common.h"
#include "../../include/lgd_hip.h"

namespace {

constexpr int GN_MAXC = 4096;

constexpr int GN_PASS_C = 2048;
constexpr int GN_UNROLL = 4;
constexpr int GN_UNROLL_S = 8;

__device__ __forceinline__ void gn_group_reduce(float* s_a, float* s_b, const float (&a)[8],
                                                const float (&b)[8], bool active, int slot, int c_lo,
                                                int c_n, int pl, int cpg, int G, float& acc_a,
                                                float& acc_b) {
  if (active) {
#pragma unroll
    for (int e = 0; e < 8; ++e) { s_a[slot + e] = a[e]; s_b[slot + e] = b[e]; }
  }
  __syncthreads();
  __shared__ float s_tot[64][2];
  int T = 1;
  while (T * 2 * G <= 256 && T < 64) T *= 2;
  {
    const int g = threadIdx.x / T, j = threadIdx.x - g * T;
    float pa = 0.f, pb = 0.f;
    if (g < G) {
      int lo = g * cpg, hi = lo + cpg;
      if (lo < c_lo) lo = c_lo;
      if (hi > c_lo + c_n) hi = c_lo + c_n;
      const int n_e = hi > lo ? (hi - lo) * pl : 0;
      for (int e = j; e < n_e; e += T) {
        const int c = lo + e / pl, p_ = e - (e / pl) * pl;
        pa += s_a[p_ * c_n + (c - c_lo)];
        pb += s_b[p_ * c_n + (c - c_lo)];
      }
    }
    for (int o = 1; o < T; o <<= 1) {
      pa += __shfl_xor(pa, o, 64);
      pb += __shfl_xor(pb, o, 64);
    }
    if (g < G && j == 0) { s_tot[g][0] = pa; s_tot[g][1] = pb; }
  }
  __syncthreads();
  if (threadIdx.x < G) {
    acc_a += s_tot[threadIdx.x][0];
    acc_b += s_tot[threadIdx.x][1];
  }
}

__global__ __launch_bounds__(256) void gn_stats_kernel(const half_t* __restrict__ x0,
                                                        const half_t* __restrict__ x1, int c0,
                                                        int c1, int HW, int G, float* part,
                                                        int nchunk) {
  __shared__ float s_a[GN_PASS_C], s_b[GN_PASS_C];
  const int C = c0 + c1;
  const int cpg = C / G;
  const int b = blockIdx.y, chunk = blockIdx.x;
  const int p_per = (HW + nchunk - 1) / nchunk;
  const int p_beg = chunk * p_per;
  int p_end = p_beg + p_per;
  if (p_end > HW) p_end = HW;
  const int nvec = C / 8;
  const int vs = nvec < 256 ? nvec : 256;
  const int pl = 256 / vs;
  const int plane = threadIdx.x / vs;
  const int n_pass = (nvec + vs - 1) / vs;
  float acc_s = 0.f, acc_q = 0.f;
  for (int pass = 0; pass < n_pass; ++pass) {
    const int v = threadIdx.x % vs + pass * vs;
    const bool active = v < nvec && plane < pl;
    const int c_lo = pass * vs * 8;
    const int c_n = (nvec - pass * vs < vs ? nvec - pass * vs : vs) * 8;
    float s[8], q[8];
#pragma unroll
    for (int e = 0; e < 8; ++e) { s[e] = 0.f; q[e] = 0.f; }
    if (active) {
      const int c = v * 8;
      const bool second = c >= c0;
      const half_t* src = second ? x1 : x0;
      const int cc = second ? c - c0 : c;
      const int ld = second ? c1 : c0;
      for (int p = p_beg + plane; p < p_end; p += GN_UNROLL_S * pl) {
        half8_t h[GN_UNROLL_S];
#pragma unroll
        for (int u = 0; u < GN_UNROLL_S; ++u) {
          const int pp = p + u * pl;
          h[u] = pp < p_end ? *reinterpret_cast<const half8_t*>(src + ((long)b * HW + pp) * ld + cc)
                            : (half8_t){0, 0, 0, 0, 0, 0, 0, 0};
        }
#pragma unroll
        for (int u = 0; u < GN_UNROLL_S; ++u)
#pragma unroll
          for (int e = 0; e < 8; ++e) {
            float f = (float)h[u][e];
            s[e] += f;
            q[e] += f * f;
          }
      }
    }
    gn_group_reduce(s_a, s_b, s, q, active, plane * c_n + (v * 8 - c_lo), c_lo, c_n, pl, cpg, G, acc_s, acc_q);
  }
  if (threadIdx.x < G) {
    float* o = part + (((long)b * nchunk + chunk) * G + threadIdx.x) * 2;
    o[0] = acc_s;
    o[1] = acc_q;
  }
}

__global__ __launch_bounds__(256) void gn_apply_kernel(const half_t* __restrict__ x0,
                                                        const half_t* __restrict__ x1, int c0,
                                                        int c1, int HW, int G, float eps,
                                                        const float* __restrict__ gamma,
                                                        const float* __restrict__ beta, int silu,
                                                        half_t* __restrict__ y,
                                                        const float* __restrict__ part, int nchunk,
                                                        float* stats, int napply, long y_dup) {
  __shared__ float s_mean[64], s_rstd[64];
  const int C = c0 + c1;
  const int cpg = C / G;
  const int b = blockIdx.y;
  __shared__ float s_ps[256], s_pq[256];
  {
    const int gi = threadIdx.x % G, sl = threadIdx.x / G, nsl = 256 / G;
    float s = 0.f, q = 0.f;
    if (sl < nsl)
      for (int ch = sl; ch < nchunk; ch += nsl) {
        const float* p = part + (((long)b * nchunk + ch) * G + gi) * 2;
        s += p[0];
        q += p[1];
      }
    s_ps[threadIdx.x] = s;
    s_pq[threadIdx.x] = q;
  }
  __syncthreads();
  if (threadIdx.x < G) {
    float s = 0.f, q = 0.f;
    for (int sl = 0; sl < 256 / G; ++sl) { s += s_ps[sl * G + threadIdx.x]; q += s_pq[sl * G + threadIdx.x]; }
    float n = (float)HW * cpg;
    float mean = s / n;
    float var = q / n - mean * mean;
    if (var < 0.f) var = 0.f;
    float rstd = rsqrtf(var + eps);
    s_mean[threadIdx.x] = mean;
    s_rstd[threadIdx.x] = rstd;
    if (stats && blockIdx.x == 0) {
      stats[((long)b * G + threadIdx.x) * 2 + 0] = mean;
      stats[((long)b * G + threadIdx.x) * 2 + 1] = rstd;
    }
  }
  __syncthreads();
  const int p_per = (HW + napply - 1) / napply;
  const int p_beg = blockIdx.x * p_per;
  int p_end = p_beg + p_per;
  if (p_end > HW) p_end = HW;
  const int nvec = C / 8;
  const int vs = nvec < 256 ? nvec : 256;
  const int pl = 256 / vs;
  const int plane = threadIdx.x / vs;
  const int n_pass = (nvec + vs - 1) / vs;
  for (int pass = 0; pass < n_pass; ++pass) {
    const int v = threadIdx.x % vs + pass * vs;
    if (v >= nvec || plane >= pl) continue;
    const int c = v * 8;
    float sa[8], sb[8];
#pragma unroll
    for (int e = 0; e < 8; ++e) {
      const int g = (c + e) / cpg;
      sa[e] = s_rstd[g] * gamma[c + e];
      sb[e] = beta[c + e] - s_mean[g] * sa[e];
    }
    const bool second = c >= c0;
    const half_t* src = second ? x1 : x0;
    const int cc = second ? c - c0 : c;
    const int ld = second ? c1 : c0;
    for (int p = p_beg + plane; p < p_end; p += GN_UNROLL * pl) {
      half8_t h[GN_UNROLL];
#pragma unroll
      for (int u = 0; u < GN_UNROLL; ++u) {
        const int pp = p + u * pl;
        if (pp < p_end) h[u] = *reinterpret_cast<const half8_t*>(src + ((long)b * HW + pp) * ld + cc);
      }
#pragma unroll
      for (int u = 0; u < GN_UNROLL; ++u) {
        const int pp = p + u * pl;
        if (pp < p_end) {
          half8_t o;
#pragma unroll
          for (int e = 0; e < 8; ++e) {
            float f = (float)h[u][e] * sa[e] + sb[e];
            if (silu) f = silu_f(f);
            o[e] = (half_t)f;
          }
          half_t* yp = y + ((long)b * HW + pp) * C + c;
          *reinterpret_cast<half8_t*>(yp) = o;
          if (y_dup) *reinterpret_cast<half8_t*>(yp + y_dup) = o;
        }
      }
    }
  }
}

template <int MAXP>
__global__ __launch_bounds__(256) void gn_fused_kernel(const half_t* __restrict__ x0, const half_t* __restrict__ x1,
                                                        int c0, int c1, int HW, int G, float eps,
                                                        const float* __restrict__ gamma, const float* __restrict__ beta,
                                                        int silu, half_t* __restrict__ y, float* stats, int kg,
                                                        long y_dup) {
  __shared__ float s_part[256 * 8];
  __shared__ float s_ch[256];
  __shared__ float s_g[8][2];
  const int tid = threadIdx.x;
  const int C = c0 + c1, cpg = C / G;
  const int b = blockIdx.y, g_lo = blockIdx.x * kg;
  const int W = kg * cpg, nv = W / 8, pl = 256 / nv;
  const int vcol = tid % nv, plane = tid / nv;
  const bool active = plane < pl;
  const int c = g_lo * cpg + vcol * 8;
  const bool second = c >= c0;
  const half_t* src = second ? x1 : x0;
  const int cc = second ? c - c0 : c;
  const int ld = second ? c1 : c0;
  half8_t h[MAXP];
#pragma unroll
  for (int u = 0; u < MAXP; ++u) {
    const int pp = plane + u * pl;
    h[u] = (active && pp < HW) ? *reinterpret_cast<const half8_t*>(src + ((long)b * HW + pp) * ld + cc)
                               : (half8_t){0, 0, 0, 0, 0, 0, 0, 0};
  }
  auto group_sum = [&](const float (&v)[8], int slot) {
#pragma unroll
    for (int e = 0; e < 8; ++e) s_part[tid * 8 + e] = active ? v[e] : 0.f;
    __syncthreads();
    if (tid < W) {
      float t = 0.f;
      for (int p = 0; p < pl; ++p) t += s_part[p * W + tid];
      s_ch[tid] = t;
    }
    __syncthreads();
    if (tid < kg) {
      float t = 0.f;
      for (int j = 0; j < cpg; ++j) t += s_ch[tid * cpg + j];
      s_g[tid][slot] = t / ((float)HW * cpg);
    }
    __syncthreads();
  };
  float a[8];
#pragma unroll
  for (int e = 0; e < 8; ++e) a[e] = 0.f;
#pragma unroll
  for (int u = 0; u < MAXP; ++u)
#pragma unroll
    for (int e = 0; e < 8; ++e) a[e] += (float)h[u][e];
  group_sum(a, 0);
  float mean[8];
#pragma unroll
  for (int e = 0; e < 8; ++e) { mean[e] = s_g[(vcol * 8 + e) / cpg][0]; a[e] = 0.f; }
#pragma unroll
  for (int u = 0; u < MAXP; ++u) {
    const bool ok = plane + u * pl < HW;
#pragma unroll
    for (int e = 0; e < 8; ++e) {
      const float dlt = (float)h[u][e] - mean[e];
      a[e] += ok ? dlt * dlt : 0.f;
    }
  }
  group_sum(a, 1);
  if (tid < kg && stats) {
    stats[((long)b * G + g_lo + tid) * 2 + 0] = s_g[tid][0];
    stats[((long)b * G + g_lo + tid) * 2 + 1] = rsqrtf(s_g[tid][1] + eps);
  }
  if (!active) return;
  float sa[8], sb[8];
#pragma unroll
  for (int e = 0; e < 8; ++e) {
    const float rstd = rsqrtf(s_g[(vcol * 8 + e) / cpg][1] + eps);
    sa[e] = rstd * gamma[c + e];
    sb[e] = beta[c + e] - mean[e] * sa[e];
  }
#pragma unroll
  for (int u = 0; u < MAXP; ++u) {
    const int pp = plane + u * pl;
    if (pp < HW) {
      half8_t o;
#pragma unroll
      for (int e = 0; e < 8; ++e) {
        float f = (float)h[u][e] * sa[e] + sb[e];
        if (silu) f = silu_f(f);
        o[e] = (half_t)f;
      }
      half_t* yp = y + ((long)b * HW + pp) * C + c;
      *reinterpret_cast<half8_t*>(yp) = o;
      if (y_dup) *reinterpret_cast<half8_t*>(yp + y_dup) = o;
    }
  }
}

int g_gn_fused_hw = 256;

template <int NT>
__device__ __forceinline__ void gn_slab_reduce(float* s_col, float* s_tot, float (*s_g)[2], bool active, int plane,
                                               int vcol, int nv, int pl, int cpg, int kg, float lo_a, float lo_b,
                                               float hi_a, float hi_b) {
  const int ncol = 2 * nv;
  if (active) {
    s_col[(2 * vcol + 0) * pl + plane] = lo_a;
    s_col[(2 * vcol + 1) * pl + plane] = hi_a;
    s_col[(ncol + 2 * vcol + 0) * pl + plane] = lo_b;
    s_col[(ncol + 2 * vcol + 1) * pl + plane] = hi_b;
  }
  __syncthreads();
  {
    const int w = threadIdx.x >> 6, lane = threadIdx.x & 63;
    for (int c = w; c < ncol; c += NT / 64) {
      float pa = 0.f, pb = 0.f;
      for (int i = lane; i < pl; i += 64) {
        pa += s_col[c * pl + i];
        pb += s_col[(ncol + c) * pl + i];
      }
#pragma unroll
      for (int o = 32; o >= 1; o >>= 1) {
        pa += __shfl_xor(pa, o, 64);
        pb += __shfl_xor(pb, o, 64);
      }
      if (lane == 0) { s_tot[c] = pa; s_tot[64 + c] = pb; }
    }
  }
  __syncthreads();
  if (threadIdx.x < kg) {
    const int t = threadIdx.x;
    const int v_lo = (t * cpg) / 8, v_hi = ((t + 1) * cpg - 1) / 8;
    float a = 0.f, b = 0.f;
    for (int v = v_lo; v <= v_hi; ++v) {
      const int which = t - (8 * v) / cpg;
      a += s_tot[2 * v + which];
      b += s_tot[64 + 2 * v + which];
    }
    s_g[t][0] = a;
    s_g[t][1] = b;
  }
  __syncthreads();
}

template <int NT, int MAXP, bool SILU>
__global__ __launch_bounds__(NT) void gn_bwd_slab_kernel(const half_t* __restrict__ gy, const half_t* __restrict__ x0,
                                                          const half_t* __restrict__ x1, int c0, int c1, int HW, int G,
                                                          const float* __restrict__ gamma, const float* __restrict__ beta,
                                                          const float* __restrict__ stats, half_t* gx0,
                                                          half_t* gx1, int accumulate, int kg) {
  __shared__ float s_col[4 * NT];
  __shared__ float s_tot[128];
  __shared__ float s_g[8][2];
  const int tid = threadIdx.x;
  const int C = c0 + c1, cpg = C / G;
  const int b = blockIdx.y, g_lo = blockIdx.x * kg;
  const int W = kg * cpg, nv = W / 8, pl = NT / nv;
  const int vcol = tid % nv, plane = tid / nv;
  const bool active = plane < pl;
  const int c = g_lo * cpg + vcol * 8;
  const bool second = c >= c0;
  const int ld = second ? c1 : c0;
  const long xoff = (long)b * HW * ld + (second ? c - c0 : c);
  const half_t* src = (second ? x1 : x0) + xoff;
  const half_t* gsrc = gy + (long)b * HW * C + c;
  half8_t hx[MAXP], hg[MAXP];
  {
    const half_t* lp = src + (long)plane * ld;
    const half_t* gp = gsrc + (long)plane * C;
    const long lstep = (long)pl * ld, gstep = (long)pl * C;
#pragma unroll
    for (int u = 0; u < MAXP; ++u) {
      const int pp = plane + u * pl;
      const bool ok = active && pp < HW;
      hx[u] = *reinterpret_cast<const half8_t*>(ok ? lp : src);
      hg[u] = *reinterpret_cast<const half8_t*>(ok ? gp : gsrc);
      lp += lstep;
      gp += gstep;
      asm volatile("" : "+v"(lp), "+v"(gp));
    }
  }
  const int gl = (8 * vcol) / cpg;
// ... 395 lines not shown
      const int v = lane + j * 64;
      if (v < nvec) {
        half8_t o;
#pragma unroll
        for (int e = 0; e < 8; ++e) o[e] = (half_t)(((float)h[r][j][e] - mean) * rstd * gm[j][e] + bt[j][e]);
        *reinterpret_cast<half8_t*>(yr + v * 8) = o;
      }
    }
  }
}

template <int CTRL>
__device__ __forceinline__ float dpp_add(float v) {
  const int t = __builtin_amdgcn_update_dpp(0, __builtin_bit_cast(int, v), CTRL, 0xf, 0xf, false);
  return v + __builtin_bit_cast(float, t);
}
template <int L>
__device__ __forceinline__ float lane_group_sum(float v) {
  v = dpp_add<0xB1>(v);
  v = dpp_add<0x4E>(v);
  v = dpp_add<0x141>(v);
  if constexpr (L >= 16) v = dpp_add<0x140>(v);
  if constexpr (L >= 32) v += __shfl_xor(v, 16, 64);
  if constexpr (L >= 64) v += __shfl_xor(v, 32, 64);
  return v;
}

template <int L, int R>
__global__ __launch_bounds__(256) void ln_stats_kernel(const half_t* __restrict__ x, long ldx, int rows, int C, float eps,
                                                        float* __restrict__ stats, int rpb, long x_bs) {
  constexpr int V = 5;
  constexpr int RPW = 64 / L;
  const int lane = threadIdx.x & 63, li = lane % L, lr = lane / L;
  const int row0 = (blockIdx.x * 4 + (threadIdx.x >> 6)) * (RPW * R) + lr;
  const int nvec = C / 8;
  half8_t h[R][V];
#pragma unroll
  for (int r = 0; r < R; ++r) {
    const int row = row0 + r * RPW;
    const int rc = row < rows ? row : rows - 1;
    const int bb = rc / rpb, rr = rc - bb * rpb;
    const half_t* xr = x + bb * x_bs + (long)rr * ldx;
#pragma unroll
    for (int j = 0; j < V; ++j) {
      const int v = li + j * L;
      h[r][j] = v < nvec ? *reinterpret_cast<const half8_t*>(xr + v * 8) : (half8_t){0, 0, 0, 0, 0, 0, 0, 0};
    }
  }
  const float inv_c = 1.f / C;
  float mean[R], var[R];
#pragma unroll
  for (int r = 0; r < R; ++r) {
    float s = 0.f;
#pragma unroll
    for (int j = 0; j < V; ++j)
#pragma unroll
      for (int e = 0; e < 8; ++e) s += (float)h[r][j][e];
    mean[r] = s;
  }
#pragma unroll
  for (int r = 0; r < R; ++r) mean[r] = lane_group_sum<L>(mean[r]) * inv_c;
#pragma unroll
  for (int r = 0; r < R; ++r)
#pragma unroll
    for (int j = 0; j < V; ++j) asm volatile("" : "+v"(h[r][j]));
#pragma unroll
  for (int r = 0; r < R; ++r) {
    float q = 0.f;
#pragma unroll
    for (int j = 0; j < V; ++j)
      if (li + j * L < nvec) {
#pragma unroll
        for (int e = 0; e < 8; ++e) {
          const float dlt = (float)h[r][j][e] - mean[r];
          q += dlt * dlt;
        }
      }
    var[r] = q;
  }
#pragma unroll
  for (int r = 0; r < R; ++r) var[r] = lane_group_sum<L>(var[r]) * inv_c;
#pragma unroll
  for (int r = 0; r < R; ++r) {
    const int row = row0 + r * RPW;
    if (li == 0 && row < rows) *reinterpret_cast<float2*>(stats + (long)row * 2) = make_float2(mean[r], rsqrtf(var[r] + eps));
  }
}

__global__ __launch_bounds__(256) void layernorm_bwd_kernel(
    const half_t* __restrict__ gy, long ldgy, const half_t* __restrict__ x, long ldx, half_t* gx,
    long ldgx, int rows, int C, const float* __restrict__ gamma, const float* __restrict__ stats,
    int rpb, long gy_bs, long x_bs, long gx_bs, int accumulate) {
  const int lane = threadIdx.x & 63;
  const int row = blockIdx.x * 4 + (threadIdx.x >> 6);
  if (row >= rows) return;
  const int bb = row / rpb, rr = row - bb * rpb;
  const half_t* gr = gy + bb * gy_bs + (long)rr * ldgy;
  const half_t* xr = x + bb * x_bs + (long)rr * ldx;
  half_t* dr = gx + bb * gx_bs + (long)rr * ldgx;
  const float mean = stats[(long)row * 2], rstd = stats[(long)row * 2 + 1];
  const int nvec = C / 8;
  float dxh[LN_MAXV][8], xh[LN_MAXV][8];
  float s1 = 0.f, s2 = 0.f;
#pragma unroll
  for (int j = 0; j < LN_MAXV; ++j) {
    int v = lane + j * 64;
    if (v < nvec) {
      half8_t hx = *reinterpret_cast<const half8_t*>(xr + v * 8);
      half8_t hg = *reinterpret_cast<const half8_t*>(gr + v * 8);
#pragma unroll
      for (int e = 0; e < 8; ++e) {
        float a = ((float)hx[e] - mean) * rstd;
        float d = (float)hg[e] * gamma[v * 8 + e];
        xh[j][e] = a;
        dxh[j][e] = d;
        s1 += d;
        s2 += d * a;
      }
    }
  }
  s1 = wave_sum(s1) / C;
  s2 = wave_sum(s2) / C;
#pragma unroll
  for (int j = 0; j < LN_MAXV; ++j) {
    int v = lane + j * 64;
    if (v < nvec) {
      half8_t o;
      if (accumulate) o = *reinterpret_cast<const half8_t*>(dr + v * 8);
#pragma unroll
      for (int e = 0; e < 8; ++e) {
        float dx = rstd * (dxh[j][e] - s1 - xh[j][e] * s2);
        if (accumulate) dx += (float)o[e];
        o[e] = (half_t)dx;
      }
      *reinterpret_cast<half8_t*>(dr + v * 8) = o;
    }
  }
}

int g_gn_apply_wgs = 1024;
int gn_apply_blocks(int B, int HW, int C) {
  const int nvec = C / 8;
  const int pl = nvec < 256 ? 256 / nvec : 1;
  int px = GN_UNROLL * pl;
  const int want = (int)(((long)HW * B + g_gn_apply_wgs - 1) / g_gn_apply_wgs);
  if (px < want) px = want;
  int n = (HW + px - 1) / px;
  return n < 1 ? 1 : n;
}

}

void lgd_gn_set_fused_hw(int hw) { g_gn_fused_hw = hw; }
void lgd_ln_set_stream(int on) { g_ln_stream = on; }
void lgd_gn_set_slab(int on) { g_gn_slab = on; }
void lgd_gn_set_apply_wgs(int n) { g_gn_apply_wgs = n; }

static int groupnorm_launch(const void* x0, const void* x1, int c0, int c1, int B, int HW, int G, float eps,
                            const float* gamma, const float* beta, int silu, void* y, float* part, int nchunk,
                            float* stats, int pair, void* stream) {
  (void)hipGetLastError();
  const int C = c0 + c1;
  if (G > 64 || C > GN_MAXC || (C % G) || (c0 % 8) || (c1 % 8) || nchunk < 1) return LGD_ERR_ARG;
  if (c1 > 0 && !x1) return LGD_ERR_ARG;
  if (pair && ((pair != LGD_PAIR_HALF && pair != LGD_PAIR_DUP) || B < 2 || (B % 2) || stats)) return LGD_ERR_ARG;
  const int Bg = pair ? B / 2 : B;
  const long y_dup = pair == LGD_PAIR_DUP ? (long)Bg * HW * C : 0L;
  hipStream_t st = reinterpret_cast<hipStream_t>(stream);
  {
    const int cpg = C / G;
    int kg = 1;
    while ((kg * cpg) % 8) kg *= 2;
    const int W = kg * cpg, nv = W / 8;
    if (HW <= g_gn_fused_hw && kg <= 8 && (G % kg) == 0 && W <= 256) {
      const int pl = 256 / nv, npx = (HW + pl - 1) / pl;
      if (npx <= 32) {
#define GN_FUSED(P)                                                                                                 \
  hipLaunchKernelGGL(gn_fused_kernel<P>, dim3(G / kg, Bg), dim3(256), 0, st, (const half_t*)x0, (const half_t*)x1,   \
                     c0, c1, HW, G, eps, gamma, beta, silu, (half_t*)y, stats, kg, y_dup)
        if (npx <= 4) GN_FUSED(4);
        else if (npx <= 8) GN_FUSED(8);
        else if (npx <= 16) GN_FUSED(16);
        else GN_FUSED(32);
#undef GN_FUSED
        return lgd_check_launch();
      }
    }
  }
  hipLaunchKernelGGL(gn_stats_kernel, dim3(nchunk, Bg), dim3(256), 0, st, (const half_t*)x0,
                     (const half_t*)x1, c0, c1, HW, G, part, nchunk);
  const int napply = gn_apply_blocks(B, HW, C);
  hipLaunchKernelGGL(gn_apply_kernel, dim3(napply, Bg), dim3(256), 0, st, (const half_t*)x0,
                     (const half_t*)x1, c0, c1, HW, G, eps, gamma, beta, silu, (half_t*)y, part,
                     nchunk, stats, napply, y_dup);
  return lgd_check_launch();
}

extern "C" int lgd_groupnorm_f16(const void* x0, const void* x1, int c0, int c1, int B, int HW,
                                 int G, float eps, const float* gamma, const float* beta, int silu,
                                 void* y, float* part, int nchunk, float* stats, void* stream) {
  return groupnorm_launch(x0, x1, c0, c1, B, HW, G, eps, gamma, beta, silu, y, part, nchunk, stats, 0, stream);
}

extern "C" int lgd_groupnorm_pair_f16(const void* x0, const void* x1, int c0, int c1, int B, int HW,
                                      int G, float eps, const float* gamma, const float* beta, int silu,
                                      void* y, float* part, int nchunk, int pair, void* stream) {
  if (pair != LGD_PAIR_HALF && pair != LGD_PAIR_DUP) return LGD_ERR_ARG;
  return groupnorm_launch(x0, x1, c0, c1, B, HW, G, eps, gamma, beta, silu, y, part, nchunk, nullptr, pair, stream);
}

extern "C" int lgd_groupnorm_bwd_f16(const void* gy, const void* x0, const void* x1, int c0, int c1,
                                     int B, int HW, int G, const float* gamma, const float* beta,
                                     int silu, const float* stats, void* gx0, void* gx1, float* part,
                                     int nchunk, int accumulate, void* stream) {
  (void)hipGetLastError();
  const int C = c0 + c1;
  if (G > 64 || C > GN_MAXC || (C % G) || (c0 % 8) || (c1 % 8) || nchunk < 1) return LGD_ERR_ARG;
  hipStream_t st = reinterpret_cast<hipStream_t>(stream);
  {
    int kg, nv;
    if (g_gn_slab && gn_slab_geometry(C, G, kg, nv)) {
#define GN_BWD_SLAB_(NT, P, S)                                                                                      \
  hipLaunchKernelGGL((gn_bwd_slab_kernel<NT, P, S>), dim3(G / kg, B), dim3(NT), 0, st, (const half_t*)gy,             \
                     (const half_t*)x0, (const half_t*)x1, c0, c1, HW, G, gamma, beta, stats, (half_t*)gx0,           \
                     (half_t*)gx1, accumulate, kg)
#define GN_BWD_SLAB(NT, P) do { if (silu) GN_BWD_SLAB_(NT, P, true); else GN_BWD_SLAB_(NT, P, false); } while (0)
      const long slab_bytes = 2L * HW * (8 * nv) * 2;
      if (slab_bytes <= 96 * 1024) {
        if (HW <= 8 * (256 / nv)) { GN_BWD_SLAB(256, 8); return lgd_check_launch(); }
        if (HW <= 11 * (512 / nv)) { GN_BWD_SLAB(512, 11); return lgd_check_launch(); }
      }
#undef GN_BWD_SLAB
#undef GN_BWD_SLAB_
    }
  }
  hipLaunchKernelGGL(gn_bwd_stats_kernel, dim3(nchunk, B), dim3(256), 0, st, (const half_t*)gy,
                     (const half_t*)x0, (const half_t*)x1, c0, c1, HW, G, gamma, beta, silu, stats,
                     part, nchunk);
  const int napply = gn_apply_blocks(B, HW, C);
  hipLaunchKernelGGL(gn_bwd_apply_kernel, dim3(napply, B), dim3(256), 0, st, (const half_t*)gy,
                     (const half_t*)x0, (const half_t*)x1, c0, c1, HW, G, gamma, beta, silu, stats,
                     (half_t*)gx0, (half_t*)gx1, part, nchunk, accumulate, napply);
  return lgd_check_launch();
}

static int layernorm_launch(const void* x, int64_t ldx, void* y, int64_t ldy, int rows, int rows_all, int C,
                            float eps, const float* gamma, const float* beta, float* stats,
                            int rows_per_batch, int64_t x_bs, int64_t y_bs, void* stream) {
  (void)hipGetLastError();
  if ((C % 8) || C > 64 * 8 * LN_MAXV || rows < 1) return LGD_ERR_ARG;
  if (!y && (!stats || C > (g_ln_stream ? 64 * 5 * 8 : 192 * 8))) return LGD_ERR_ARG;
  if (rows_per_batch < 1) rows_per_batch = rows_all;
  hipStream_t st = reinterpret_cast<hipStream_t>(stream);
  const half_t* xp = (const half_t*)x;
  half_t* yp = (half_t*)y;
  const int nvec = C / 8;
  if (!y && g_ln_stream && ((long)rows_all * C >= (8L << 20) || nvec > 192)) {
#define LGD_LN_STATS(L, R)                                                                                         \
  hipLaunchKernelGGL((ln_stats_kernel<L, R>), dim3((rows + 4 * (64 / L) * R - 1) / (4 * (64 / L) * R)), dim3(256), 0, st, xp, \
                     (long)ldx, rows, C, eps, stats, rows_per_batch, (long)x_bs)
    if (nvec <= 40) LGD_LN_STATS(8, 4);
    else if (nvec <= 80) LGD_LN_STATS(16, 4);
    else if (nvec <= 160) LGD_LN_STATS(32, 4);
    else LGD_LN_STATS(64, 2);
#undef LGD_LN_STATS
    return lgd_check_launch();
  }
#define LGD_LN_LAUNCH(MAXV, ROWS)                                                                   \
  hipLaunchKernelGGL((layernorm_rows_kernel<MAXV, ROWS>), dim3((rows + 4 * ROWS - 1) / (4 * ROWS)), \
                     dim3(256), 0, st, xp, (long)ldx, yp, (long)ldy, rows, C, eps, gamma, beta,      \
                     stats, rows_per_batch, (long)x_bs, (long)y_bs)
  if (nvec <= 64) LGD_LN_LAUNCH(1, 4);
  else if (nvec <= 128) LGD_LN_LAUNCH(2, 4);
  else if (nvec <= 192) LGD_LN_LAUNCH(3, 2);
  else
    hipLaunchKernelGGL(layernorm_kernel, dim3((rows + 3) / 4), dim3(256), 0, st, xp, (long)ldx, yp,
                       (long)ldy, rows, C, eps, gamma, beta, stats, rows_per_batch, (long)x_bs,
                       (long)y_bs);
#undef LGD_LN_LAUNCH
  return lgd_check_launch();
}

extern "C" int lgd_layernorm_f16(const void* x, int64_t ldx, void* y, int64_t ldy, int rows, int C,
                                 float eps, const float* gamma, const float* beta, float* stats,
                                 int rows_per_batch, int64_t x_bs, int64_t y_bs, void* stream) {
  return layernorm_launch(x, ldx, y, ldy, rows, rows, C, eps, gamma, beta, stats, rows_per_batch, x_bs, y_bs, stream);
}

extern "C" int lgd_layernorm_pair_f16(const void* x, int64_t ldx, void* y, int64_t ldy, int rows, int C,
                                      float eps, const float* gamma, const float* beta, float* stats,
                                      int rows_per_batch, int64_t x_bs, int64_t y_bs, int pair, void* stream) {
  if (pair != LGD_PAIR_HALF || rows < 2 || (rows % 2)) return LGD_ERR_ARG;
  if (rows_per_batch >= 1 && ((rows / 2) % rows_per_batch)) return LGD_ERR_ARG;
  return layernorm_launch(x, ldx, y, ldy, rows / 2, rows, C, eps, gamma, beta, stats, rows_per_batch, x_bs, y_bs, stream);
}

extern "C" int lgd_layernorm_bwd_f16(const void* gy, int64_t ldgy, const void* x, int64_t ldx,
                                     void* gx, int64_t ldgx, int rows, int C, const float* gamma,
                                     const float* stats, int rows_per_batch, int64_t gy_bs,
                                     int64_t x_bs, int64_t gx_bs, int accumulate, void* stream) {
  (void)hipGetLastError();
  if ((C % 8) || C > 64 * 8 * LN_MAXV || rows < 1 || !stats) return LGD_ERR_ARG;
  if (rows_per_batch < 1) rows_per_batch = rows;
  hipStream_t st = reinterpret_cast<hipStream_t>(stream);
  hipLaunchKernelGGL(layernorm_bwd_kernel, dim3((rows + 3) / 4), dim3(256), 0, st,
                     (const half_t*)gy, (long)ldgy, (const half_t*)x, (long)ldx, (half_t*)gx,
                     (long)ldgx, rows, C, gamma, stats, rows_per_batch, (long)gy_bs, (long)x_bs,
                     (long)gx_bs, accumulate);
  return lgd_check_launch();
}
```

llm-groundeddiffusion_amd/ops.py:

```python
import contextlib
import ctypes as C

import torch

from . import _lib
from ._lib import EPI_GEGLU, EPI_OUT_F32, EPI_RES_F32, EPI_ROWNORM, PAIR_DUP, PAIR_HALF, LgdGemmDesc

F16, F32 = torch.float16, torch.float32


def _stream():
    return C.c_void_p(torch.cuda.current_stream().cuda_stream)


def _p(t):
    return C.c_void_p(t.data_ptr()) if t is not None else C.c_void_p(0)


def _call(name, *args):
    lib = _lib.load()
    rc = getattr(lib, name)(*args)
    _lib.check(rc, name)


def set_option(name: str, value: int):
    _call("lgd_set_option", name.encode(), int(value))


def get_option(name: str) -> int:
    v = _lib.load().lgd_get_option(name.encode())
    if v < 0:
        raise RuntimeError(f"lgd_get_option({name}) failed")
    return v


import threading as _threading
_TLS = _threading.local()
WS_FLOATS = 1 << 26


def workspace(device) -> torch.Tensor:
    dev = torch.device(device)
    ws = getattr(_TLS, "ws", None)
    if ws is None or ws.device != dev:
        ws = _TLS.ws = torch.empty(WS_FLOATS, device=dev, dtype=F32)
    return ws


N_COUNTERS = 1 << 16
import os as _os
SPLITK_IN_LAUNCH = _os.environ.get("LGD_SPLITK_IN_LAUNCH", "0") == "1"


def splitk_counters(device):
    dev = torch.device(device)
    cnt = getattr(_TLS, "cnt", None)
    if cnt is None or cnt.device != dev:
        cnt = _TLS.cnt = torch.zeros(N_COUNTERS, device=dev, dtype=torch.int32)
    return cnt


def choose_splits(M, N, K, batches=1):
    wgs = ((M + 127) // 128) * ((N + 63) // 64) * batches
    if wgs >= 256:
        return 1
    ktiles = K // 64
    s = min((512 + wgs - 1) // wgs, max(1, ktiles // 4), 16)
    return max(1, s)


def gemm_desc(a0, w, c, M, N, K, *, a1=None, lda0=None, lda1=0, c0=None, c1=0, taps=1,
              hin=0, win=0, hout=0, wout=0, stride=1, ups=0, ldw=None, bias=None, bias2=None,
              res=None, ldr=0, alpha=1.0, epi=0, ldc=None, splits=None, ws=None, tile=0,
              nb_o=1, nb_i=1, a_bs=(0, 0), w_bs=(0, 0), c_bs=(0, 0), r_bs=(0, 0), rowstat=None, colsum=None):
    d = LgdGemmDesc()
    ptr = lambda t: (t.data_ptr() if torch.is_tensor(t) else (t or 0))
    d.a0, d.a1 = ptr(a0), ptr(a1)
    cin = K // taps
    d.c0 = cin - c1 if c0 is None else c0
    d.c1 = c1
    d.lda0 = d.c0 if lda0 is None else lda0
    d.lda1 = lda1 if lda1 else max(c1, 0)
    d.taps, d.hin, d.win, d.hout, d.wout, d.stride, d.ups = taps, hin, win, hout, wout, stride, ups
    d.w = ptr(w)
    d.ldw = K if ldw is None else ldw
    d.M, d.N, d.K = M, N, K
    d.nb_o, d.nb_i = nb_o, nb_i
    d.a_bs_o, d.a_bs_i = a_bs
    d.w_bs_o, d.w_bs_i = w_bs
    d.c_bs_o, d.c_bs_i = c_bs
    d.r_bs_o, d.r_bs_i = r_bs
    d.bias, d.bias2 = ptr(bias), ptr(bias2)
    d.res, d.ldr = ptr(res), ldr
    if rowstat is not None:
        epi |= EPI_ROWNORM
    d.rowstat, d.colsum = ptr(rowstat), ptr(colsum)
    d.alpha, d.epi = alpha, epi
    d.c = ptr(c)
    n_out = N // 2 if (epi & EPI_GEGLU) else N
    d.ldc = n_out if ldc is None else ldc
    ent = tuning_table().get(shape_key(d)) if (splits is None or not tile) else None
    if splits is None:
        splits = ent["splits"] if ent else choose_splits(M, N, K, nb_o * nb_i)
    if splits > 1 and ws is None:
        need = splits * M * N * nb_o * nb_i
        ws = workspace(c.device if torch.is_tensor(c) else "cuda")
        if need > ws.numel():
            raise RuntimeError(f"split-K workspace too small for {splits}x{M}x{N}")
    d.splits, d.ws = splits, ptr(ws)
    d.cnt = 0
    d.tile = tile
    if not tile:
        if ent and ent["splits"] == splits:
            d.tile = ent["tile"]
        if not d.tile or not gemm_accepts(d):
            d.tile = choose_tile(M, N, nb_o * nb_i * max(splits, 1), bool(epi & EPI_GEGLU), K,
                                 pipe_ok=(K % 64 == 0 and d.c0 % 64 == 0 and d.c1 % 64 == 0))
    log = getattr(_TUNING_TLS, "log", None)
    if log is not None:
        log.append((shape_key(d), d.tile, splits))
    if splits > 1 and SPLITK_IN_LAUNCH and torch.is_tensor(c) and c.is_cuda:
        if nb_o * nb_i * ((M + 31) // 32) * ((N + 63) // 64) <= N_COUNTERS:
            d.cnt = splitk_counters(c.device).data_ptr()
            if not gemm_accepts(d):
                d.cnt = 0
    return d


def gemm_accepts(d) -> bool:
    return _lib.load().lgd_gemm_check(C.byref(d)) == 0


def gemm_set_pair(d, mode) -> bool:
    prev, d.pair = d.pair, mode
    if mode and not gemm_accepts(d):
        d.pair = prev
        return False
    return True


TILE_NAMES = {
    1: "gemm_kernel<4,4> 128x128", 2: "gemm_kernel<4,2> 128x64", 3: "gemm_kernel<2,4> 64x128", 4: "gemm_kernel<2,2> 64x64",
    5: "gemm_kernel<1,4> 32x128", 6: "gemm_kernel<4,5> 128x160", 7: "gemm_kernel<2,5> 64x160",
    17: "gemm_dma_kernel<4,4,2> 128x128", 18: "gemm_dma_kernel<4,2,2> 128x64", 19: "gemm_dma_kernel<2,4,2> 64x128",
    20: "gemm_dma_kernel<2,2,2> 64x64", 21: "gemm_dma_kernel<1,4,2> 32x128", 22: "gemm_dma_kernel<4,5,2> 128x160",
    23: "gemm_dma_kernel<2,5,2> 64x160", 25: "gemm_dma_kernel<4,10,4> 256x320", 26: "gemm_dma_kernel<4,4,4> 256x128",
    33: "gemm_pipe_kernel<4,5,4,2,3> 256x160", 34: "gemm_pipe_kernel<4,4,4,2,3> 256x128",
    35: "gemm_pipe_kernel<4,2,4,2,4> 256x64", 37: "gemm_pipe_kernel<2,5,4,2,4> 128x160",
    38: "gemm_pipe_kernel<2,4,4,2,4> 128x128", 39: "gemm_pipe_kernel<2,2,4,2,5> 128x64",
    40: "gemm_pipe_kernel<1,5,4,2,5> 64x160", 41: "gemm_pipe_kernel<1,4,4,2,5> 64x128",
    42: "gemm_pipe_kernel<1,2,4,2,6> 64x64", 44: "gemm_pipe_kernel<4,8,4,2,2> 256x256",
    45: "gemm_pipe_kernel<2,4,4,2,2> 128x128 x2/CU", 46: "gemm_phase_kernel<8,4> 256x256",
    47: "gemm_phase_kernel<8,5> 256x320",
}


def choose_tile(M, N, batches=1, geglu=False, K=64, pipe_ok=False):
    wgs = lambda bm, bn: batches * ((M + bm - 1) // bm) * ((N + bn - 1) // bn)
    if M <= 32:
        return 21
    if pipe_ok:
        if not geglu and N % 160 == 0 and wgs(256, 160) >= 256:
            return 33
        if N % 128 == 0 and wgs(256, 128) >= 256:
            return 34
        if not geglu and N % 160 == 0 and wgs(128, 160) >= 256:
            return 37
        if N % 128 == 0 and wgs(128, 128) >= 256:
            return 38
    if not geglu and N % 160 == 0:
        if wgs(128, 160) >= 384:
            return 22
        if wgs(64, 160) >= 256:
            return 23
    if wgs(128, 128) >= 384 and N % 128 == 0:
        return 17
    if wgs(64, 128) >= 256 and N % 128 == 0:
        return 19
    return 20


def shape_key(d) -> str:
    return (f"M{d.M}_N{d.N}_K{d.K}_t{d.taps}_c{d.c0}+{d.c1}_h{d.hin}x{d.hout}_s{d.stride}_u{d.ups}"
            f"_e{d.epi & 1}_b{d.nb_o * d.nb_i}")


_TUNING = {}
TUNING_MODE = _os.environ.get("LGD_TUNING_MODE", "latency")
_TUNING_FILES = {"latency": ("tuning_gfx950.json",), "throughput": ("tuning_gfx950.json", "tuning_gfx950_lanes.json"),
                 "heuristic": ()}
_TUNING_TLS = _threading.local()


def set_tuning_mode(mode: str):
    global TUNING_MODE
    if mode not in _TUNING_FILES:
        raise ValueError(f"tuning mode {mode!r}: expected one of {sorted(_TUNING_FILES)}")
    if _os.environ.get("LGD_TUNING_MODE"):
        return
    TUNING_MODE = mode


def current_tuning_mode() -> str:
    if _os.environ.get("LGD_TUNING_MODE"):
        return TUNING_MODE
    return getattr(_TUNING_TLS, "mode", None) or TUNING_MODE


@contextlib.contextmanager
def tuning(mode):
    if mode is not None and mode not in _TUNING_FILES:
        raise ValueError(f"tuning mode {mode!r}: expected one of {sorted(_TUNING_FILES)}")
    prev = getattr(_TUNING_TLS, "mode", None)
    if mode is not None:
        _TUNING_TLS.mode = mode
    try:
        yield
    finally:
        _TUNING_TLS.mode = prev


@contextlib.contextmanager
def desc_log():
    prev, _TUNING_TLS.log = getattr(_TUNING_TLS, "log", None), []
    try:
        yield _TUNING_TLS.log
    finally:
        _TUNING_TLS.log = prev


def tuning_table():
    mode = current_tuning_mode()
    if mode not in _TUNING:
        import json
        tab = {}
        for fname in _TUNING_FILES[mode]:
            path = _os.path.join(_os.path.dirname(_os.path.abspath(__file__)), fname)
            if _os.path.exists(path):
                tab.update(json.load(open(path)))
        _TUNING[mode] = tab
    return _TUNING[mode]


class LaunchProfiler:

    def __init__(self, max_records=20000):
        self.recs = []
        self.max = max_records
        self.enabled = True

    def wrap(self, name, flops, nbytes, fn, tag=None, shape=None):
        if not self.enabled or len(self.recs) >= self.max:
            return fn()
        e0, e1 = torch.cuda.Event(enable_timing=True), torch.cuda.Event(enable_timing=True)
        e0.record()
        r = fn()
        e1.record()
        self.recs.append((name, flops, nbytes, e0, e1, tag, shape))
        return r

    def summary(self, by_tag=False, by_shape=False):
        torch.cuda.synchronize()
        agg = {}
        for name, fl, nb, e0, e1, tag, shape in self.recs:
            if by_tag and tag is None:
                continue
            key = tag if by_tag else (f"{name} | {shape}" if by_shape else name)
            a = agg.setdefault(key, dict(ms=0.0, flops=0.0, bytes=0.0, n=0))
            a["ms"] += e0.elapsed_time(e1)
            a["flops"] += fl
            a["bytes"] += nb
            a["n"] += 1
        return agg


PROFILER = None


def _prof(name, nbytes, fn, *, flops=0.0, tag=None, shape=None):
    if PROFILER is not None:
        return PROFILER.wrap(name, flops, nbytes, fn, tag, shape)
    return fn()


def copy_(dst, src):
    return _prof("copy", 2.0 * dst.numel() * dst.element_size(), lambda: dst.copy_(src))


def zero_(t):
    return _prof("fill", float(t.numel() * t.element_size()), lambda: t.zero_())


def gemm_launch(desc, tag=None, flops=None):
    if PROFILER is not None:
        nb = desc.nb_o * desc.nb_i
        if flops is None:
            flops = 2.0 * desc.M * desc.N * desc.K * nb
        if desc.pair:
            flops *= 0.5
        m_in, m_out = (desc.M // 2 if desc.pair else desc.M), (desc.M // 2 if desc.pair == PAIR_HALF else desc.M)
        nbytes = 2.0 * nb * (m_in * desc.K / max(desc.taps, 1) + desc.N * desc.K + m_out * desc.N)
        return PROFILER.wrap(TILE_NAMES.get(desc.tile, "gemm"), flops, nbytes,
                             lambda: _call("lgd_gemm_f16", C.byref(desc), _stream()), tag,
                             shape=f"{shape_key(desc)} splits={desc.splits}")
    _call("lgd_gemm_f16", C.byref(desc), _stream())


def linear(x, w, bias=None, res=None, out=None, *, alpha=1.0, geglu=False, out_f32=False,
           splits=None, ws=None, tile=0, bias2=None, rowstat=None, colsum=None):
    M, K = x.shape
    N = w.shape[0]
    n_out = N // 2 if geglu else N
    if out is None:
        out = torch.empty((M, n_out), device=x.device, dtype=F32 if out_f32 else F16)
    epi = (EPI_GEGLU if geglu else 0) | (EPI_OUT_F32 if out_f32 else 0)
    if res is not None and res.dtype == F32:
        epi |= EPI_RES_F32
    d = gemm_desc(x, w, out, M, N, K, bias=bias, bias2=bias2, res=res,
                  ldr=(res.stride(0) if res is not None else 0), alpha=alpha, epi=epi,
                  splits=splits, ws=ws, tile=tile, lda0=x.stride(0), ldw=w.stride(0),
                  ldc=out.stride(0), rowstat=rowstat, colsum=colsum)
    gemm_launch(d)
    return out


def conv3x3(x, w, B, H, W, *, x1=None, bias=None, bias2=None, res=None, stride=1, ups=False,
            out=None, splits=None, ws=None, tile=0, alpha=1.0):
    c0 = x.shape[1]
    c1 = x1.shape[1] if x1 is not None else 0
    Cout = w.shape[0]
    K = 9 * (c0 + c1)
    assert w.shape[1] == K
    if ups:
        Hl, Wl = 2 * H, 2 * W
    else:
        Hl, Wl = H, W
    Ho, Wo = (Hl - 1) // stride + 1, (Wl - 1) // stride + 1
    M = B * Ho * Wo
    if out is None:
        out = torch.empty((M, Cout), device=x.device, dtype=F16)
    d = gemm_desc(x, w, out, M, Cout, K, a1=x1, c0=c0, c1=c1, lda0=x.stride(0),
                  lda1=(x1.stride(0) if x1 is not None else 0), taps=9, hin=H, win=W, hout=Ho,
                  wout=Wo, stride=stride, ups=int(ups), bias=bias, bias2=bias2, res=res,
                  ldr=(res.stride(0) if res is not None else 0), splits=splits, ws=ws, tile=tile,
                  alpha=alpha, ldc=out.stride(0))
    gemm_launch(d)
    return out


def conv_in(x_nchw, w, bias, out=None):
    B, Cin, L, _ = x_nchw.shape
    Cout = w.shape[0]
    if out is None:
        out = torch.empty((B * L * L, Cout), device=x_nchw.device, dtype=F16)
    _call("lgd_conv_in_f16", _p(x_nchw), _p(w), _p(bias), _p(out), B, Cin, L, Cout, _stream())
    return out


def nchw_to_nhwc8(x_nchw, out=None):
    B, C_, H, W = x_nchw.shape
    if out is None:
        out = torch.empty((B * H * W, 8), device=x_nchw.device, dtype=F16)
    _prof("nchw_to_nhwc8_kernel", 4.0 * x_nchw.numel() + 2.0 * out.numel(),
          lambda: _call("lgd_nchw_to_nhwc8_f16", _p(x_nchw), _p(out), B, C_, H * W, _stream()))
    return out


_U8_TABLES = {}


def u8_table(device) -> torch.Tensor:
    key = str(device)
    if key not in _U8_TABLES:
        u = torch.arange(256, dtype=F32)
        _U8_TABLES[key] = (2.0 * (u / 255.0) - 1.0).to(device)
    return _U8_TABLES[key]


def image_u8_to_nhwc8(img_u8, out=None):
    B, H, W, C_ = img_u8.shape
    if C_ != 3 or img_u8.dtype != torch.uint8 or not img_u8.is_contiguous():
        raise RuntimeError("image_u8_to_nhwc8 takes a contiguous uint8 (B, H, W, 3) tensor")
    if out is None:
        out = torch.empty((B * H * W, 8), device=img_u8.device, dtype=F16)
    _call("lgd_image_u8_to_nhwc8_f16", _p(img_u8), _p(u8_table(img_u8.device)), _p(out), B, H * W, _stream())
    return out


def vae_sample(moments, noise, scale, out=None):
    B, z, H, W = noise.shape
    if tuple(moments.shape) != (B * H * W, 2 * z) or moments.dtype != F16 or noise.dtype != F32:
        raise RuntimeError(f"vae_sample: moments {tuple(moments.shape)} {moments.dtype} for noise {tuple(noise.shape)}")
    if out is None:
        out = torch.empty_like(noise)
    _call("lgd_vae_sample_f32", _p(moments), _p(noise), _p(out), B, z, H * W, float(scale), _stream())
    return out


def conv_out(x, w, bias, B, L, out=None, out_scale=1.0):
    Cin = x.shape[1]
    Cout = w.shape[0]
    if out is None:
        out = torch.empty((B, Cout, L, L), device=x.device, dtype=F32)
    _prof("conv_out_kernel", 2.0 * x.numel() + 4.0 * out.numel(),
          lambda: _call("lgd_conv_out_f16", _p(x), _p(w), _p(bias), _p(out), B, Cin, L, Cout, float(out_scale), _stream()),
          flops=2.0 * B * L * L * Cout * 9 * Cin)
    return out


GN_STATS_WGS = int(_os.environ.get("LGD_GN_STATS_WGS", "1024"))


def gn_chunks(B, HW):
    return max(1, min(HW // 8, GN_STATS_WGS // max(B, 1), 64))


def groupnorm(x, B, HW, G, eps, gamma, beta, silu, *, x1=None, out=None, part=None, stats=None, pair=0):
    c0 = x.shape[1]
    c1 = x1.shape[1] if x1 is not None else 0
    C_ = c0 + c1
    nchunk = gn_chunks(B, HW)
    if out is None:
        out = torch.empty((B * HW, C_), device=x.device, dtype=F16)
    if part is None:
        part = torch.empty((B, nchunk, G, 2), device=x.device, dtype=F32)
    if pair:
        assert stats is None, "pair mode is a no-grad forward: no statistics output"
        _prof("groupnorm (gn_stats + gn_apply | gn_fused)", (2.0 + (2.0 if pair == PAIR_DUP else 1.0)) * B * HW * C_,
              lambda: _call("lgd_groupnorm_pair_f16", _p(x), _p(x1), c0, c1, B, HW, G, float(eps), _p(gamma), _p(beta),
                            1 if silu else 0, _p(out), _p(part), nchunk, int(pair), _stream()), shape=f"B{B}_HW{HW}_C{C_}")
        return out
    _prof("groupnorm (gn_stats + gn_apply | gn_fused)", 6.0 * B * HW * C_,
          lambda: _call("lgd_groupnorm_f16", _p(x), _p(x1), c0, c1, B, HW, G, float(eps), _p(gamma), _p(beta),
                        1 if silu else 0, _p(out), _p(part), nchunk, _p(stats), _stream()), shape=f"B{B}_HW{HW}_C{C_}")
    return out


def groupnorm_bwd(gy, x, B, HW, G, gamma, beta, silu, stats, *, x1=None, gx0=None, gx1=None,
                  part=None, accumulate=False):
    c0 = x.shape[1]
    c1 = x1.shape[1] if x1 is not None else 0
    nchunk = gn_chunks(B, HW)
    if gx0 is None:
        gx0 = torch.empty_like(x)
    if x1 is not None and gx1 is None:
        gx1 = torch.empty_like(x1)
    if part is None:
        part = torch.empty((B, nchunk, G, 2), device=x.device, dtype=F32)
    _prof("groupnorm_bwd (gn_bwd_stats + gn_bwd_apply)", (10.0 + (2.0 if accumulate else 0.0)) * B * HW * (c0 + c1),
          lambda: _call("lgd_groupnorm_bwd_f16", _p(gy), _p(x), _p(x1), c0, c1, B, HW, G, _p(gamma), _p(beta),
                        1 if silu else 0, _p(stats), _p(gx0), _p(gx1), _p(part), nchunk, 1 if accumulate else 0, _stream()),
          shape=f"B{B}_HW{HW}_C{c0 + c1}")
    return gx0, gx1


def layernorm(x, gamma, beta, eps=1e-5, *, out=None, ldy=None, stats=None, rows_per_batch=0,
              x_bs=0, y_bs=0, rows=None, ldx=None, pair=0):
    C_ = gamma.shape[0]
    if rows is None:
        rows = x.numel() // C_
    if out is None:
        out = torch.empty((rows, C_), device=x.device, dtype=F16)
    if pair:
        _prof("layernorm_rows_kernel", 2.0 * rows * C_,
              lambda: _call("lgd_layernorm_pair_f16", _p(x), ldx or C_, _p(out), ldy or C_, rows, C_, float(eps), _p(gamma),
                            _p(beta), _p(stats), rows_per_batch, x_bs, y_bs, int(pair), _stream()), shape=f"R{rows}_C{C_}")
        return out
    _prof("layernorm_rows_kernel", 4.0 * rows * C_,
          lambda: _call("lgd_layernorm_f16", _p(x), ldx or C_, _p(out), ldy or C_, rows, C_, float(eps), _p(gamma),
                        _p(beta), _p(stats), rows_per_batch, x_bs, y_bs, _stream()), shape=f"R{rows}_C{C_}")
    return out


def layernorm_stats(x, C_, eps=1e-5, *, stats=None, rows=None, ldx=None, pair=0):
    if rows is None:
        rows = x.numel() // C_
    if stats is None:
        stats = torch.empty((rows, 2), device=x.device, dtype=torch.float32)
    if pair:
        _prof("ln_stats_kernel (LayerNorm statistics only)", 1.0 * rows * C_,
              lambda: _call("lgd_layernorm_pair_f16", _p(x), ldx or C_, _p(None), C_, rows, C_, float(eps), _p(None),
                            _p(None), _p(stats), 0, 0, 0, int(pair), _stream()), shape=f"R{rows}_C{C_}")
        return stats
    _prof("ln_stats_kernel (LayerNorm statistics only)", 2.0 * rows * C_,
          lambda: _call("lgd_layernorm_f16", _p(x), ldx or C_, _p(None), C_, rows, C_, float(eps), _p(None), _p(None),
                        _p(stats), 0, 0, 0, _stream()), shape=f"R{rows}_C{C_}")
    return stats


def layernorm_bwd(gy, x, gamma, stats, *, gx=None, rows=None, ldgy=None, ldx=None, ldgx=None,
                  rows_per_batch=0, gy_bs=0, x_bs=0, gx_bs=0, accumulate=False):
    C_ = gamma.shape[0]
    if rows is None:
        rows = x.numel() // C_
    if gx is None:
        gx = torch.empty((rows, C_), device=x.device, dtype=F16)
    _prof("layernorm_bwd_kernel", (6.0 + (2.0 if accumulate else 0.0)) * rows * C_,
          lambda: _call("lgd_layernorm_bwd_f16", _p(gy), ldgy or C_, _p(x), ldx or C_, _p(gx), ldgx or C_, rows, C_,
                        _p(gamma), _p(stats), rows_per_batch, gy_bs, x_bs, gx_bs, 1 if accumulate else 0, _stream()),
          shape=f"R{rows}_C{C_}")
    return gx


def attn_fwd(q, k, v, o, B, H, Sq, Sk, d, scale, *, lse=None, q_view=None, k_view=None,
             v_view=None, o_view=None, pair=0):
    qv = q_view or (H * d, Sq * H * d)
    kv = k_view or (H * d, Sk * H * d)
    vv = v_view or (H * d, Sk * H * d)
    ov = o_view or (H * d, Sq * H * d)
    if pair:
        fn = lambda: _call("lgd_attn_fwd_pair_f16", _p(q), qv[0], qv[1], _p(k), kv[0], kv[1], _p(v), vv[0], vv[1],
                           _p(o), ov[0], ov[1], _p(lse), B, H, Sq, Sk, d, float(scale), int(pair), _stream())
    else:
        fn = lambda: _call("lgd_attn_fwd_f16", _p(q), qv[0], qv[1], _p(k), kv[0], kv[1], _p(v), vv[0], vv[1],
                           _p(o), ov[0], ov[1], _p(lse), B, H, Sq, Sk, d, float(scale), _stream())
    if PROFILER is not None:
        Bc = B // 2 if pair else B
        PROFILER.wrap(f"attn_self_kernel d={d}", 4.0 * Bc * H * Sq * Sk * d, 2.0 * Bc * H * d * (2 * Sq + 2 * Sk), fn,
                      "attn_path", shape=f"B{B}_H{H}_Sq{Sq}_Sk{Sk}")
    else:
        fn()
    return o


def attn_bwd(q, k, v, o, go, lse, delta, gq, gk, gv, B, H, Sq, Sk, d, scale, *, q_view=None,
             k_view=None, v_view=None, o_view=None, go_view=None, gq_view=None, gk_view=None,
             gv_view=None, sk_grad=None):
    skg = Sk if sk_grad is None else int(sk_grad)
    dq_ = (H * d, Sq * H * d)
    dk_ = (H * d, Sk * H * d)
    qv, kv, vv = q_view or dq_, k_view or dk_, v_view or dk_
    ov, gov = o_view or dq_, go_view or dq_
    gqv, gkv, gvv = gq_view or dq_, gk_view or dk_, gv_view or dk_
    _prof(f"attn_bwd_dq + attn_bwd_dkv d={d}", 2.0 * B * H * d * (4 * Sq + 4 * Sk),
          lambda: _call("lgd_attn_bwd_keys_f16", _p(q), qv[0], qv[1], _p(k), kv[0], kv[1], _p(v), vv[0], vv[1], _p(o),
                        ov[0], ov[1], _p(go), gov[0], gov[1], _p(lse), _p(delta), _p(gq), gqv[0], gqv[1], _p(gk),
                        gkv[0], gkv[1], _p(gv), gvv[0], gvv[1], B, H, Sq, Sk, skg, d, float(scale), _stream()),
          flops=6.0 * B * H * Sq * Sk * d + 4.0 * B * H * Sq * skg * d, tag="attn_path_bwd", shape=f"B{B}_H{H}_Sq{Sq}_Sk{Sk}")


def cross_attn_fwd(q, k, v, o, B, H, Sq, Sk, d, scale, *, probs=None, tok=-1, cond_only=False,
                   q_view=None, k_view=None, v_view=None, o_view=None):
    qv = q_view or (H * d, Sq * H * d)
    kv = k_view or (H * d, Sk * H * d)
    vv = v_view or (H * d, Sk * H * d)
    ov = o_view or (H * d, Sq * H * d)
    fn = lambda: _call("lgd_cross_attn_fwd_f16", _p(q), qv[0], qv[1], _p(k), kv[0], kv[1], _p(v), vv[0], vv[1],
                       _p(o), ov[0], ov[1], _p(probs), int(tok), 1 if cond_only else 0, B, H, Sq, Sk, d,
                       float(scale), _stream())
    if PROFILER is not None:
        PROFILER.wrap(f"attn_fwd_kernel(cross) d={d}", 4.0 * B * H * Sq * Sk * d,
                      2.0 * B * H * d * (2 * Sq + 2 * Sk), fn, "attn_path")
    else:
        fn()
    return o


def attn_causal_fwd(q, k, v, o, B, H, S, d, scale, *, view=None):
    vw = view or (H * d, S * H * d)
    _call("lgd_attn_causal_fwd_f16", _p(q), vw[0], vw[1], _p(k), vw[0], vw[1], _p(v), vw[0], vw[1], _p(o),
          H * d, S * H * d, B, H, S, d, float(scale), _stream())
    return o


ATTN_OP_FWD, ATTN_OP_BWD, ATTN_OP_CROSS_BWD = 0, 1, 2


def _attn_variant_names():
    names = {}
    shapes = {0: "4 waves x 1 query tile", 1: "4 waves x 2 query tiles", 2: "8 waves x 2 query tiles"}
    for dp in (32, 64, 96, 128, 160, 192):
        modes = {0: f"d = {dp}", 1: f"d < {dp}, row of ones"}
        if dp == 64:
            modes[2] = "d < 48, row of ones, 3 dv tiles"
        for m, mname in modes.items():
            for s, sname in shapes.items():
                if s == 0 or dp <= 96 or (dp == 160 and m == 0 and s == 2):
                    names[100000 + dp * 100 + 10 * m + s] = f"attn_self_kernel DP={dp} ({mname}) {sname}"
        names[400000 + dp * 100] = f"attn_fwd_kernel DP={dp} (two-pass softmax: map capture, causal)"
    for dk in (48, 96):
        for s, sname in {0: "4 waves", 1: "8 waves", 2: "8 waves, prefetch 4 ahead", 3: "8 waves, compiler's slot order"}.items():
            names[200000 + dk * 100 + s] = f"attn_self32_kernel DK={dk} {sname}"
    names[306400] = "attn_w4_kernel d=40, two waves per SIMD"
    names[306401] = "attn_w4_kernel d=40, one wave per SIMD (in-wave pipeline)"
    bshapes = {0: "1 tile per wave", 1: "2 tiles per wave", 2: "2 tiles per wave, double-buffered",
               3: "2 tiles per wave, double-buffered, 8 waves"}
    for dp in (32, 64, 96, 128, 160):
# ... 200 lines not shown
```

llm-groundeddiffusion_amd/unet.py:

```python
import math
import os
from collections import OrderedDict
from typing import Dict, List, Optional, Sequence, Tuple

import torch

from . import ops
from ._lib import EPI_GEGLU, PAIR_DUP, PAIR_HALF
from .weights import UNetConfig, unet_blocks
from .weightstore import WeightStore

F16, F32 = torch.float16, torch.float32
N_OBJ_TOKENS = 30


class Act:
    __slots__ = ("t", "g", "rows", "C", "pair")

    def __init__(self, t):
        self.t = t
        self.g = None
        self.rows, self.C = t.shape
        self.pair = None


class PairMode:
    __slots__ = ("mode", "desc", "on_dup")

    def __init__(self, mode, desc=None):
        self.mode, self.desc, self.on_dup = mode, desc, None
        if desc is not None:
            desc.pair = mode

    def dup(self):
        self.mode = PAIR_DUP
        if self.desc is not None:
            self.desc.pair = PAIR_DUP
        if self.on_dup is not None:
            self.on_dup()


class Op:
    def __init__(self, fwd, make_bwd=None, gouts=(), passthrough=None):
        self.fwd = fwd
        self.make_bwd = make_bwd
        self.gouts = list(gouts)
        self.acc = None
        self.bwd = None
        self.passthrough = passthrough


choose_splits = ops.choose_splits


class Plan:
    def __init__(self, eng: "UNetEngine", B: int, L: int, *, grad: bool, fuser: bool,
                 stop_key: Optional[Tuple] = None, save_keys: Sequence[Tuple] = (),
                 text_batch_offset: int = 0, obj_batch_offset: int = 0, pair_shared: bool = False):
        self.eng, self.B, self.L = eng, B, L
        self.pair_shared = bool(pair_shared)
        self._pair = False
        self.pair_ops = 0
        self.latents_pair = False
        self.obj_off = obj_batch_offset
        self.grad, self.fuser = grad, fuser
        self.stop_key = tuple(stop_key) if stop_key else None
        self.save_keys = [tuple(k) for k in save_keys]
        self.text_off = text_batch_offset
        self.ops: List[Op] = []
        self._buffers: List[torch.Tensor] = []
        self.dbg: Dict[str, Act] = {}
        self.maps: Dict[Tuple, torch.Tensor] = {}
        self.gmaps: Dict[Tuple, torch.Tensor] = {}
        self._cursor = [0, 0]
        self.arena_bytes = 0
        self.latents_in = self._alloc((B, eng.cfg.in_channels, L, L))
        self.eps_out = None
        self.g_latents = None
        self._build()

    def _new(self, rows, C, dtype=F16):
        return self._alloc((rows, C), dtype)

    def _alloc(self, shape, dtype=F32):
        t, self._cursor = self.eng.arena_take(self._cursor, shape, dtype)
        self.arena_bytes += t.numel() * t.element_size()
        self._buffers.append(t)
        return t

    def _act(self, rows, C):
        return Act(self._new(rows, C))

    def _add(self, fwd, make_bwd=None, gouts=(), passthrough=None):
        self.ops.append(Op(fwd, make_bwd if self.grad else None, gouts if self.grad else (),
                           passthrough if self.grad else None))

    def _ws(self, n_floats):
        return self.eng.workspace(n_floats)

    def _need_full(self, *acts):
        for a in acts:
            if a is not None and a.pair is not None:
                a.pair.dup()
                a.pair = None

    def _pair_op(self, inputs, out: Optional[Act], half: bool, desc=None) -> Optional[PairMode]:
        if not self._pair or (desc is not None and not ops.gemm_set_pair(desc, PAIR_DUP)):
            self._need_full(*inputs)
            return None
        pm = PairMode(PAIR_HALF if half else PAIR_DUP, desc)
        if half and out is not None:
            out.pair = pm
        self.pair_ops += 1
        return pm

    def linear(self, x: Act, name: str, *, res: Optional[Act] = None, alpha=1.0, geglu=False,
               bias=True, out: Optional[Act] = None, rows=None, bwd=True, half=False) -> Act:
        W = self.eng.w.h[f"{name}.w"]
        b = self.eng.w.f[f"{name}.b"] if bias else None
        N, K = W.shape
        M = rows or x.rows
        n_out = N // 2 if geglu else N
        y = out or self._act(M, n_out)
        d = ops.gemm_desc(x.t, W, y.t, M, N, K, lda0=x.C, bias=b, res=res.t if res else None,
                          ldr=res.C if res else 0, alpha=alpha, epi=EPI_GEGLU if geglu else 0,
                          ldc=y.C)
        self._pair_op([x, res], y, half, d)
        tag = "attn_path" if any(t in name for t in (".attn1.", ".attn2.", ".fuser.attn.")) else None
        fwd = lambda: ops.gemm_launch(d, tag)
        if not (self.grad and bwd):
            self._add(fwd)
            return y
        assert not geglu, "grad plans keep the GEGLU pre-activation (see ff())"
        Wt = self.eng.w.h[f"{name}.wt"]
        gouts = [x] + ([res] if res else [])

        def make_bwd(acc):
            dd = ops.gemm_desc(y.g, Wt, x.g, M, K, N, lda0=y.C, alpha=alpha, ldc=x.C,
                               res=x.g if acc[0] else None, ldr=x.C)
            if res is None:
                return lambda: ops.gemm_launch(dd)
            racc = acc[1]
            aliased = res.g.data_ptr() == y.g.data_ptr()

            def run():
                ops.gemm_launch(dd)
                if racc:
                    ops.add(res.g, y.g, res.g)
                elif not aliased:
                    ops.copy_(res.g, y.g)
            return run
        self._add(fwd, make_bwd, gouts, passthrough=(res, y) if res is not None else None)
        return y

    def conv(self, x: Act, name: str, H: int, *, x1: Optional[Act] = None, res: Optional[Act] = None,
             temb_off: Optional[int] = None, stride=1, ups=False, half=False) -> Act:
        B = self.B
        W = self.eng.w.h[f"{name}.w"]
        b = self.eng.w.f[f"{name}.b"]
        Cout, K = W.shape
        c0, c1 = x.C, (x1.C if x1 else 0)
        Hl = 2 * H if ups else H
        Ho = (Hl - 1) // stride + 1
        M = B * Ho * Ho
        y = self._act(M, Cout)
        eng = self.eng
        if temb_off is not None and eng.temb_rows > 1:
            assert stride == 1 and not ups and res is None and not self._pair
            ds = []
            for i in range(B):
                row = eng.temb_cur[self.text_off + i]
                sl = slice(i * H * H, (i + 1) * H * H)
                ds.append(ops.gemm_desc(x.t[sl], W, y.t[sl], H * H, Cout, K, a1=x1.t[sl] if x1 else None, c0=c0, c1=c1,
                                        lda0=c0, lda1=c1, taps=9, hin=H, win=H, hout=H, wout=H, bias=b,
                                        bias2=row[temb_off:temb_off + Cout], ldc=Cout))
            fwd = lambda: [ops.gemm_launch(dd) for dd in ds]
        else:
            bias2 = eng.temb_cur[0, temb_off:temb_off + Cout] if temb_off is not None else None
            d = ops.gemm_desc(x.t, W, y.t, M, Cout, K, a1=x1.t if x1 else None, c0=c0, c1=c1, lda0=c0,
                              lda1=c1, taps=9, hin=H, win=H, hout=Ho, wout=Ho, stride=stride,
                              ups=1 if ups else 0, bias=b, bias2=bias2, res=res.t if res else None,
                              ldr=res.C if res else 0, ldc=Cout)
            self._pair_op([x, x1, res], y, half, d)
            fwd = lambda: ops.gemm_launch(d)
        if not self.grad:
            self._add(fwd)
            return y
        Wd = self.eng.w.h[f"{name}.wd"]
        gouts = [x] + ([x1] if x1 else []) + ([res] if res else [])

        def make_bwd(acc):
            runs = []
            Kd = 9 * Cout
            if stride == 1 and not ups:
                for i, (src, lo, cn) in enumerate([(x, 0, c0)] + ([(x1, c0, c1)] if x1 else [])):
                    dd = ops.gemm_desc(y.g, Wd[lo:lo + cn], src.g, src.rows, cn, Kd, c0=Cout, lda0=Cout,
                                       taps=9, hin=H, win=H, hout=H, wout=H, ldc=cn,
                                       res=src.g if acc[i] else None, ldr=cn)
                    runs.append(lambda dd=dd: ops.gemm_launch(dd))
            elif stride == 2:
                dd = ops.gemm_desc(y.g, Wd, x.g, x.rows, c0, Kd, c0=Cout, lda0=Cout, taps=9, hin=Ho,
                                   win=Ho, hout=H, wout=H, ups=2, ldc=c0,
                                   res=x.g if acc[0] else None, ldr=c0)
                runs.append(lambda: ops.gemm_launch(dd))
            else:
                tmp = self._new(B * Hl * Hl, c0)
                dd = ops.gemm_desc(y.g, Wd, tmp, B * Hl * Hl, c0, Kd, c0=Cout, lda0=Cout, taps=9,
                                   hin=Hl, win=Hl, hout=Hl, wout=Hl, ldc=c0)
                assert not acc[0]
                runs.append(lambda: (ops.gemm_launch(dd), ops.upsample2x_bwd(tmp, B, H, H, c0, out=x.g)))
            if res is not None:
                racc = acc[-1]
                if racc:
                    runs.append(lambda: ops.add(res.g, y.g, res.g))
                elif res.g.data_ptr() != y.g.data_ptr():
                    runs.append(lambda: ops.copy_(res.g, y.g))
            return lambda: [r() for r in runs]
        self._add(fwd, make_bwd, gouts, passthrough=(res, y) if res is not None else None)
        return y

    def shortcut(self, x: Act, x1: Optional[Act], name: str) -> Act:
        W = self.eng.w.h[f"{name}.w"]
        b = self.eng.w.f[f"{name}.b"]
        Cout, K = W.shape
        c0, c1 = x.C, (x1.C if x1 else 0)
        M = x.rows
        self._need_full(x, x1)
        y = self._act(M, Cout)
        d = ops.gemm_desc(x.t, W, y.t, M, Cout, K, a1=x1.t if x1 else None, c0=c0, c1=c1, lda0=c0,
                          lda1=c1, bias=b, ldc=Cout)
        fwd = lambda: ops.gemm_launch(d)
        if not self.grad:
            self._add(fwd)
            return y
        Wt = self.eng.w.h[f"{name}.wt"]
        gouts = [x] + ([x1] if x1 else [])

        def make_bwd(acc):
            runs = []
            for i, (src, lo, cn) in enumerate([(x, 0, c0)] + ([(x1, c0, c1)] if x1 else [])):
                dd = ops.gemm_desc(y.g, Wt[lo:lo + cn], src.g, M, cn, Cout, lda0=Cout, ldc=cn,
                                   res=src.g if acc[i] else None, ldr=cn)
                runs.append(lambda dd=dd: ops.gemm_launch(dd))
            return lambda: [r() for r in runs]
        self._add(fwd, make_bwd, gouts)
        return y

    def groupnorm(self, x: Act, x1: Optional[Act], name: str, HW: int, eps: float, silu: bool, half=False) -> Act:
        eng, B = self.eng, self.B
        G = eng.cfg.norm_num_groups
        gm, bt = eng.w.f[f"{name}.g"], eng.w.f[f"{name}.b"]
        C = x.C + (x1.C if x1 else 0)
        y = self._act(x.rows, C)
        nch = ops.gn_chunks(B, HW)
        part = self._alloc((B, nch, G, 2))
        stats = self._alloc((B, G, 2)) if self.grad else None
        xt1 = x1.t if x1 else None
        pm = self._pair_op([x, x1], y, half)
        if pm is not None:
            fwd = lambda: ops.groupnorm(x.t, B, HW, G, eps, gm, bt, silu, x1=xt1, out=y.t, part=part, pair=pm.mode)
        else:
            fwd = lambda: ops.groupnorm(x.t, B, HW, G, eps, gm, bt, silu, x1=xt1, out=y.t, part=part, stats=stats)
        if not self.grad:
            self._add(fwd)
            return y
        gouts = [x] + ([x1] if x1 else [])

        def make_bwd(acc):
            a = acc[0]
            if x1 is not None:
                assert acc[0] == acc[1], "mixed accumulate modes on a concat GroupNorm"
            return lambda: ops.groupnorm_bwd(y.g, x.t, B, HW, G, gm, bt, silu, stats, x1=xt1, gx0=x.g,
                                             gx1=x1.g if x1 else None, part=part, accumulate=a)
        self._add(fwd, make_bwd, gouts)
        return y

    def layernorm(self, x: Act, name: str, *, out_t=None, ldy=None, S=None, y_bs=0, half=False) -> Act:
        eng = self.eng
        gm, bt = eng.w.f[f"{name}.g"], eng.w.f[f"{name}.b"]
        C = x.C
        y = Act(out_t) if out_t is not None else self._act(x.rows, C)
        stats = self._alloc((x.rows, 2)) if self.grad else None
        rpb = S or 0
        x_bs = (S or 0) * C
        pm = self._pair_op([x], y, True) if half and out_t is None and x.rows % 2 == 0 else None
        if pm is None:
            self._need_full(x)
        else:
            pm.on_dup = lambda: self._need_full(x)
        fwd = lambda: ops.layernorm(x.t, gm, bt, out=y.t, ldy=ldy or C, stats=stats, rows=x.rows,
                                    rows_per_batch=rpb, x_bs=x_bs, y_bs=y_bs, pair=PAIR_HALF if y.pair is not None else 0)
        if not self.grad:
            self._add(fwd)
            return y

        def make_bwd(acc):
            return lambda: ops.layernorm_bwd(y.g, x.t, gm, stats, gx=x.g, rows=x.rows, ldgy=ldy or C,
                                             rows_per_batch=rpb, gy_bs=y_bs, x_bs=x_bs, gx_bs=x_bs,
                                             accumulate=acc[0])
        self._add(fwd, make_bwd, [x])
        return y

    def ln_linear(self, x: Act, norm: str, name: str, *, geglu=False, half=False) -> Act:
        eng = self.eng
        has_b = f"{name}.b" in eng.w.f
        if self.grad or not eng.fold_ln or x.C > 1536:
            y = self.layernorm(x, norm, half=True)
            if geglu:
                return self.linear(y, name, geglu=True, half=half)
            return self.linear(y, name, bias=has_b, half=half)
        W, cs, b = eng.w.h[f"{name}.wln"], eng.w.f[f"{name}.cs"], eng.w.f[f"{name}.bln"]
        N, K = W.shape
        M = x.rows
        stats = self._alloc((M, 2))
        y = self._act(M, N // 2 if geglu else N)
        d = ops.gemm_desc(x.t, W, y.t, M, N, K, lda0=x.C, bias=b, epi=EPI_GEGLU if geglu else 0, ldc=y.C,
                          rowstat=stats, colsum=cs)
        tag = "attn_path" if any(t in name for t in (".attn1.", ".attn2.", ".fuser.attn.")) else None
        xt = x.t
        sp = PAIR_HALF if self._pair_op([x], y, half, d) is not None else 0
        self._add(lambda: (ops.layernorm_stats(xt, K, stats=stats, rows=M, pair=sp), ops.gemm_launch(d, tag)))
        return y

    def self_attn(self, qkv: Act, heads: int, S: int, Sk: Optional[int] = None, half=False) -> Act:
        B = self.B
        Sk = Sk or S
        C = qkv.C // 3
        d = C // heads
        o = self._act(B * S, C)
        view = (3 * C, Sk * 3 * C)
        lse = self._alloc((B, heads, S)) if self.grad else None
        scale = d ** -0.5
        qt, kt, vt = qkv.t, qkv.t[:, C:], qkv.t[:, 2 * C:]
        pm = self._pair_op([qkv], o, half)
        fwd = lambda: ops.attn_fwd(qt, kt, vt, o.t, B, heads, S, Sk, d, scale, lse=lse,
                                   q_view=view, k_view=view, v_view=view, pair=pm.mode if pm is not None else 0)
        if not self.grad:
            self._add(fwd)
            return o

        def make_bwd(acc):
            assert not acc[0]
            delta = self._alloc((B, heads, S))
            g = qkv.g
            gq, gk, gv = g, g[:, C:], g[:, 2 * C:]
            pad = Sk > S

            g_tail = g.view(B, Sk, 3 * C)[:, S:, :] if pad else None

            def run():
                if pad:
                    ops.zero_(g_tail)
                ops.attn_bwd(qt, kt, vt, o.t, o.g, lse, delta, gq, gk, gv, B, heads, S, Sk, d, scale,
                             q_view=view, k_view=view, v_view=view, gq_view=view, gk_view=view, gv_view=view, sk_grad=S)
            return run
        self._add(fwd, make_bwd, [qkv])
        return o

    def cross_attn(self, q: Act, key: Tuple, layer_name: str, heads: int, S: int, last: bool) -> Optional[Act]:
        eng, B = self.eng, self.B
        C = q.C
        d = C // heads
        T = eng.text_len
        kv = eng.text_kv[layer_name]
        kv_t = kv[self.text_off:]
        k_view = (2 * C, T * 2 * C)
        o = self._act(B * S, C)
        scale = d ** -0.5
        probs = None
        if key in self.save_keys:
            probs = self.maps[key] = self._alloc((B, heads, S, T))
            if self.grad:
                self.gmaps[key] = self._alloc((B, heads, S, T))
        kt, vt = kv_t, kv_t[:, :, C:]
        self._need_full(q)

        def fwd():
            ops.cross_attn_fwd(q.t, kt, vt, o.t, B, heads, S, T, d, scale, probs=probs,
                               k_view=k_view, v_view=k_view)
        if not self.grad:
            self._add(fwd)
            return o
        gp = self.gmaps.get(key)

        def make_bwd(acc):
            assert not acc[0]
            return lambda: ops.cross_attn_bwd(q.t, kt, vt, None if last else o.g, gp, q.g, B, heads, S, T,
                                              d, scale, k_view=k_view, v_view=k_view)
        self._add(fwd, make_bwd, [q])
        return o

    def ff(self, x: Act, res: Act, name: str, alpha=1.0, norm: Optional[str] = None) -> Act:
        if not self.grad:
            h = self.ln_linear(x, norm, f"{name}.net.0.proj", geglu=True) if norm else self.linear(x, f"{name}.net.0.proj", geglu=True)
            return self.linear(h, f"{name}.net.2", res=res, alpha=alpha)
        if norm:
            x = self.layernorm(x, norm)
        pre = self.linear(x, f"{name}.net.0.proj")
        act = self._act(x.rows, pre.C // 2)
        self._add(lambda: ops.geglu_fwd(pre.t, out=act.t),
                  lambda acc: (lambda: ops.geglu_bwd(pre.t, act.g, pre.g)), [pre])
        return self.linear(act, f"{name}.net.2", res=res, alpha=alpha)

    def _resnet(self, r, x: Act, skip: Optional[Act], H: int) -> Act:
        eng = self.eng
        eps = eng.cfg.norm_eps
        HW = H * H
        h = self.groupnorm(x, skip, f"{r.prefix}.norm1", HW, eps, True, half=True)
        h = self.conv(h, f"{r.prefix}.conv1", H, temb_off=eng.w.temb_offsets[r.prefix], half=True)
        h = self.groupnorm(h, None, f"{r.prefix}.norm2", HW, eps, True, half=True)
        if r.shortcut:
            sc = self.shortcut(x, skip, f"{r.prefix}.conv_shortcut")
        else:
            assert skip is None
            sc = x
        out = self.conv(h, f"{r.prefix}.conv2", H, res=sc)
        self.dbg[f"{r.prefix}.out"] = out
        return out

    def _transformer(self, a, x: Act, H: int) -> Optional[Act]:
        eng, B = self.eng, self.B
        S = H * H
        C, heads = a.channels, a.heads
        n = self.groupnorm(x, None, f"{a.prefix}.norm", S, 1e-6, False, half=True)
        h = self.linear(n, f"{a.prefix}.proj_in", half=True)
        for dpt in range(a.depth):
            t = f"{a.prefix}.transformer_blocks.{dpt}"
            key = tuple(a.key[:3]) + (dpt,)
            qkv = self.ln_linear(h, f"{t}.norm1", f"{t}.attn1.qkv", half=True)
            h = self.linear(self.self_attn(qkv, heads, S, half=True), f"{t}.attn1.to_out.0", res=h)
            if dpt == 0:
                self.dbg[f"{a.prefix}.after_attn1"] = h
            if self.fuser:
                self._pair = False
                f = f"{t}.fuser"
                Sk = S + N_OBJ_TOKENS
                cat = eng.fuser_cat(eng.kv_name(a.prefix, dpt), B, S, self.obj_off)
                cat_act = self.layernorm(h, f"{f}.norm1", out_t=cat, ldy=C, S=S, y_bs=Sk * C)
                qkv_f = self.linear(cat_act, f"{f}.attn.qkv", bias=False)
                o = self.self_attn(qkv_f, heads, S, Sk)
                h = self.linear(o, f"{f}.attn.to_out.0", res=h, alpha=eng.w.scalars[f"{f}.alpha_attn"])
                self.dbg[f"{a.prefix}.after_fuser_attn"] = h
                h = self.ff(h, h, f"{f}.ff", alpha=eng.w.scalars[f"{f}.alpha_dense"], norm=f"{f}.norm2")
                self.dbg[f"{a.prefix}.after_fuser"] = h
            q = self.ln_linear(h, f"{t}.norm2", f"{t}.attn2.to_q")
            self._pair = False
            last = self.stop_key is not None and key == self.stop_key
            o = self.cross_attn(q, key, eng.kv_name(a.prefix, dpt), heads, S, last)
            if last:
                return None
            h = self.linear(o, f"{t}.attn2.to_out.0", res=h)
            if dpt == 0:
                self.dbg[f"{a.prefix}.after_attn2"] = h
            h = self.ff(h, h, f"{t}.ff", norm=f"{t}.norm3")
        out = self.linear(h, f"{a.prefix}.proj_out", res=x)
        self.dbg[f"{a.prefix}.out"] = out
        return out

    def _build(self):
        eng, B, L = self.eng, self.B, self.L
        cfg = eng.cfg
        w = eng.w
        blocks = eng.blocks
        c0 = cfg.block_out_channels[0]
        x = self._act(B * L * L, c0)
        lat = self.latents_in
        self._x0 = x
        x0 = x
        lat8 = self._new(B * L * L, 8)
        d_in = ops.gemm_desc(lat8, w.h["conv_in.w8"], x0.t, B * L * L, c0, 72, c0=8, lda0=8, taps=9, hin=L, win=L, hout=L,
                             wout=L, bias=w.f["conv_in.b"], ldc=c0, splits=1)
        f_in = 2.0 * B * L * L * c0 * 9 * cfg.in_channels
        self._pair = self.pair_shared
        if self._pair_op([], None, False, d_in) is not None:
            self.latents_pair = True
            lat = lat[:B // 2]
            f_in *= 0.5
        self._add(lambda: (ops.nchw_to_nhwc8(lat, out=lat8), ops.gemm_launch(d_in, None, f_in)))
        skips = [(x, L)]
        H = L
        done = False
        for b in blocks:
            if done:
                break
            if b.kind == "down":
                for j, r in enumerate(b.resnets):
                    x = self._resnet(r, x, None, H)
                    if b.attns:
                        x = self._transformer(b.attns[j], x, H)
                        if x is None:
                            done = True
                            break
                    self._pair = False
                    self._need_full(x)
                    skips.append((x, H))
                if done:
                    break
                if b.sampler:
                    x = self.conv(x, b.sampler, H, stride=2)
                    H = (H - 1) // 2 + 1
                    skips.append((x, H))
            elif b.kind == "mid":
                x = self._resnet(b.resnets[0], x, None, H)
                x = self._transformer(b.attns[0], x, H)
                if x is None:
                    done = True
                    break
                x = self._resnet(b.resnets[1], x, None, H)
            else:
                for j, r in enumerate(b.resnets):
                    sk, _ = skips.pop()
                    x = self._resnet(r, x, sk, H)
                    if b.attns:
                        x = self._transformer(b.attns[j], x, H)
                        if x is None:
                            done = True
                            break
                if done:
                    break
                if b.sampler:
                    x = self.conv(x, b.sampler, H, ups=True)
                    H *= 2
        if not done:
            n = self.groupnorm(x, None, "conv_norm_out", H * H, cfg.norm_eps, True)
            self.eps_out = self._alloc((B, cfg.out_channels, L, L))
            eo = self.eps_out
            self._add(lambda: ops.conv_out(n.t, w.h["conv_out.w"], w.f["conv_out.b"], B, L, out=eo))
        if self.grad:
            self._finalize_backward()

    def _finalize_backward(self):
        seen = set()
        for op in reversed(self.ops):
            if op.make_bwd is None:
                continue
            op.acc = []
            for a in op.gouts:
                if a.g is None:
                    pt = op.passthrough
                    if pt is not None and a is pt[0] and pt[1].g is not None and pt[1].g.shape == a.t.shape \
                            and os.environ.get("LGD_RES_GRAD_ALIAS", "1") != "0":
                        a.g = pt[1].g
                    else:
                        a.g = self._alloc(tuple(a.t.shape), a.t.dtype)
                op.acc.append(id(a) in seen)
                seen.add(id(a))
        for op in self.ops:
            if op.make_bwd is not None:
                op.bwd = op.make_bwd(op.acc)
        self.g_latents = self._alloc(tuple(self.latents_in.shape))
        self._bwd_ops = [op.bwd for op in reversed(self.ops) if op.bwd is not None]

    def forward(self, latents: Optional[torch.Tensor] = None):
        if latents is not None:
            self.latents_in.copy_(latents)
        for op in self.ops:
            op.fwd()
        return self.eps_out

    def backward(self, grad_scale: float = 1.0) -> torch.Tensor:
        for b in self._bwd_ops:
            b()
        eng = self.eng
# ... 23 lines not shown
            self.w = WeightStore(cfg, self.device, fold_ln=self.fold_ln)
            if state_dict is not None:
                self.w.load_state_dict(state_dict)
        self.text_len = text_len
        self.max_text_batch = max_text_batch
        self.temb_rows = max_text_batch if cfg.addition_embed_type == "text_time" else 1
        self.temb_cur = torch.zeros((self.temb_rows, self.w.temb_total), device=self.device, dtype=F32)
        self.temb_table = None
        self.dyn = torch.zeros(4, device=self.device, dtype=torch.int32)
        self.step_idx = self.dyn[:1]
        self.text_kv: Dict[str, torch.Tensor] = {}
        for b in self.blocks:
            for a in b.attns:
                for dpt in range(a.depth):
                    self.text_kv[self.kv_name(a.prefix, dpt)] = torch.zeros((max_text_batch, text_len, 2 * a.channels),
                                                                            device=self.device, dtype=F16)
        self._ws = None
        self._ws_size = 0
        self._fuser_cat: Dict[Tuple, torch.Tensor] = {}
        self._plans: "OrderedDict[Tuple, Plan]" = OrderedDict()
        self._objs = None
        self._arena: List[torch.Tensor] = []

    @staticmethod
    def kv_name(prefix: str, depth_index: int = 0) -> str:
        return prefix if depth_index == 0 else f"{prefix}@{depth_index}"

    def arena_take(self, cursor, shape, dtype):
        n = 1
        for d in shape:
            n *= int(d)
        nbytes = n * torch.empty((), dtype=dtype).element_size()
        if nbytes > self.ARENA_SEGMENT:
            raise RuntimeError(f"plan buffer of {nbytes} bytes exceeds the arena segment size")
        seg, off = cursor
        off = (off + 255) & ~255
        if off + nbytes > self.ARENA_SEGMENT:
            seg, off = seg + 1, 0
        while len(self._arena) <= seg:
            self._arena.append(torch.empty(self.ARENA_SEGMENT, device=self.device, dtype=torch.uint8))
        t = self._arena[seg][off:off + nbytes].view(dtype).view(tuple(int(d) for d in shape))
        return t, [seg, off + nbytes]

    def arena_bytes(self) -> int:
        return len(self._arena) * self.ARENA_SEGMENT

    def poison_arena(self):
        for seg in self._arena:
            seg.fill_(0xFF)

    def workspace(self, n_floats: int = 0) -> torch.Tensor:
        if self._ws is None:
            self._ws = torch.empty(ops.WS_FLOATS, device=self.device, dtype=F32)
        return self._ws

    def fuser_cat(self, prefix: str, B: int, S: int, text_off: int) -> torch.Tensor:
        key = (prefix, B, text_off)
        if key not in self._fuser_cat:
            C = self.text_kv[prefix].shape[-1] // 2
            self._fuser_cat[key] = torch.zeros((B * (S + N_OBJ_TOKENS), C), device=self.device, dtype=F16)
        return self._fuser_cat[key]

    def prepare_timesteps(self, timesteps: Sequence[int], added_cond: Optional[Dict[str, torch.Tensor]] = None):
        self.const_writer = None
        cfg, w = self.cfg, self.w
        c0 = cfg.block_out_channels[0]
        silu = torch.nn.functional.silu

        def sincos(v, dim):
            half = dim // 2
            freqs = torch.exp(-math.log(10000.0) * torch.arange(half, dtype=torch.float32, device=self.device) / half)
            e = v[:, None] * freqs[None]
            return torch.cat([torch.cos(e), torch.sin(e)], dim=-1)

        t = torch.as_tensor(list(timesteps), dtype=torch.float32, device=self.device)
        emb = sincos(t, c0).to(F16)
        T = emb.shape[0]
        h = ops.linear(emb.contiguous(), w.h["time_embedding.linear_1.w"], w.f["time_embedding.linear_1.b"], out_f32=True)
        h = silu(h).to(F16)
        h = ops.linear(h, w.h["time_embedding.linear_2.w"], w.f["time_embedding.linear_2.b"], out_f32=True)[:T]
        if cfg.addition_embed_type == "text_time":
            if added_cond is None:
                raise RuntimeError(f"{cfg.name} needs added_cond (text_embeds, time_ids) for its time embedding")
            te = added_cond["text_embeds"].to(self.device, F32)
            ids = added_cond["time_ids"].to(self.device, F32)
            R = te.shape[0]
            if R > self.temb_rows or te.shape[1] != cfg.pooled_dim or tuple(ids.shape) != (R, 5):
                raise RuntimeError(f"added_cond shapes {tuple(te.shape)} / {tuple(ids.shape)} do not fit {cfg.name}")
            tid = sincos(ids.reshape(-1), cfg.addition_time_embed_dim).reshape(R, -1)
            a = torch.cat([te, tid], dim=-1).to(F16).contiguous()
            a = ops.linear(a, w.h["add_embedding.linear_1.w"], w.f["add_embedding.linear_1.b"], out_f32=True)[:R]
            a = ops.linear(silu(a).to(F16), w.h["add_embedding.linear_2.w"], w.f["add_embedding.linear_2.b"], out_f32=True)[:R]
            h = (h[:, None, :] + a[None, :, :]).reshape(T * R, -1)
            tab = ops.linear(silu(h).to(F16).contiguous(), w.h["temb_proj.w"], w.f["temb_proj.b"], out_f32=True)[:T * R]
            full = torch.zeros((T, self.temb_rows, w.temb_total), device=self.device, dtype=F32)
            full[:, :R] = tab.view(T, R, -1)
            self.temb_table = full.view(T, -1)
        else:
            h = silu(h).to(F16)
            self.temb_table = ops.linear(h, w.h["temb_proj.w"], w.f["temb_proj.b"], out_f32=True)[:T].contiguous()
        return self.temb_table

    def set_step(self, index: int):
        self.step_idx.fill_(index)
        ops.select_row(self.temb_table, self.step_idx, self.temb_cur)

    def prepare_text(self, ehs: torch.Tensor):
        self.const_writer = None
        Bt, T, Cx = ehs.shape
        if Bt > self.max_text_batch or T != self.text_len:
            raise RuntimeError(f"text batch {Bt}x{T} exceeds the engine's text K/V buffers "
                               f"({self.max_text_batch}x{self.text_len}); chunk the jobs (LMDSampler.max_batch)")
        x = ehs.to(self.device, F16).reshape(Bt * T, Cx).contiguous()
        for b in self.blocks:
            for a in b.attns:
                for dpt in range(a.depth):
                    kv = self.text_kv[self.kv_name(a.prefix, dpt)]
                    ops.linear(x, self.w.h[f"{a.prefix}.transformer_blocks.{dpt}.attn2.kv.w"],
                               out=kv.view(-1, kv.shape[-1])[:Bt * T])

    def prepare_gligen(self, boxes: torch.Tensor, masks: torch.Tensor, positive_embeddings: torch.Tensor):
        self.const_writer = None
        w = self.w
        dev = self.device
        boxes, masks, pe = boxes.to(dev, F32), masks.to(dev, F32), positive_embeddings.to(dev, F32)
        Bt = boxes.shape[0]
        m = masks.unsqueeze(-1)
        freq = (100 ** (torch.arange(8, device=dev) / 8)).float()
        xx = freq[None, None, None] * boxes.unsqueeze(-1)
        xyxy = torch.stack((xx.sin(), xx.cos()), dim=-1).permute(0, 1, 3, 4, 2).reshape(Bt, N_OBJ_TOKENS, -1)
        pos = pe * m + (1 - m) * w.f["position_net.null_positive_feature"].view(1, 1, -1)
        xyxy = xyxy * m + (1 - m) * w.f["position_net.null_position_feature"].view(1, 1, -1)
        h = torch.cat([pos, xyxy], dim=-1).reshape(Bt * N_OBJ_TOKENS, -1).to(F16).contiguous()
        silu = torch.nn.functional.silu
        h = silu(ops.linear(h, w.h["position_net.linears.0.w"], w.f["position_net.linears.0.b"], out_f32=True)).to(F16)
        h = silu(ops.linear(h, w.h["position_net.linears.2.w"], w.f["position_net.linears.2.b"], out_f32=True)).to(F16)
        objs = ops.linear(h, w.h["position_net.linears.4.w"], w.f["position_net.linears.4.b"])
        self._objs = objs
        for (prefix, B, toff), cat in self._fuser_cat.items():
            if B not in (Bt, Bt // 2) or toff + B > Bt:
                continue
            pfx, _, dpt = prefix.partition("@")
            f = f"{pfx}.transformer_blocks.{dpt or 0}.fuser"
            C = cat.shape[1]
            S = cat.shape[0] // B - N_OBJ_TOKENS
            o = ops.linear(objs, w.h[f"{f}.linear.w"], w.f[f"{f}.linear.b"])
            o = ops.layernorm(o, w.f[f"{f}.norm1.g"], w.f[f"{f}.norm1.b"])
            cat.view(B, S + N_OBJ_TOKENS, C)[:, S:] = o.view(Bt, N_OBJ_TOKENS, C)[toff:toff + B]

    def plan(self, B: int, L: int, *, grad=False, fuser=False, stop_key=None, save_keys=(),
             text_batch_offset=0, obj_batch_offset=0, pair_shared=False) -> Plan:
        mode = self.tuning_mode or ops.current_tuning_mode()
        pair_shared = bool(pair_shared and not grad and B % 2 == 0 and self.temb_rows == 1 and ops.get_option("cfg_pair"))
        key = (B, L, grad, fuser, tuple(stop_key) if stop_key else None, tuple(map(tuple, save_keys)),
               text_batch_offset, obj_batch_offset, mode, self.fold_ln, pair_shared)
        if B + text_batch_offset > self.max_text_batch:
            raise RuntimeError(f"plan batch {B} (+{text_batch_offset}) exceeds max_text_batch={self.max_text_batch}")
        if key not in self._plans:
            with ops.tuning(mode):
                self._plans[key] = Plan(self, B, L, grad=grad, fuser=fuser, stop_key=stop_key,
                                        save_keys=save_keys, text_batch_offset=text_batch_offset,
                                        obj_batch_offset=obj_batch_offset, pair_shared=pair_shared)
            while len(self._plans) > self.MAX_PLANS:
                self._plans.popitem(last=False)
        self._plans.move_to_end(key)
        return self._plans[key]

    def attn_key_order(self) -> List[Tuple]:
        return [a.key for b in self.blocks for a in b.attns]

    def last_key(self, keys) -> Tuple:
        order = self.attn_key_order()
        return max((tuple(k) for k in keys), key=order.index)
```

Measured before the change: 1.837 images/s.

## Fuse split-K reduction of conv GEMMs into following fused GroupNorm

For conv GEMMs that run with split-K, a new epilogue flag skips the separate reduction kernel and leaves the fp32 partials in the workspace. The fused GroupNorm kernel then sums the partials, applies bias, temb and residual, and normalizes in a single pass. When a later consumer still needs the pre-norm activation, it also writes that out. This removes one kernel launch and a round trip of the fp16 activation, at the cost of the norm kernel reading all split slabs itself and only applying when shape limits (HW, group width, no pairing) allow.

```diff
diff --git a/include/lgd_hip.h b/include/lgd_hip.h
--- a/include/lgd_hip.h
+++ b/include/lgd_hip.h
@@ -14,6 +14,7 @@
 #define LGD_EPI_OUT_F32 2
 #define LGD_EPI_RES_F32 4
 #define LGD_EPI_ROWNORM 8
+#define LGD_EPI_SPLITK_KEEP 16
 
 typedef struct LgdGemmDesc {
   const void* a0;
@@ -60,6 +61,8 @@
 int lgd_groupnorm_pair_f16(const void* x0, const void* x1, int c0, int c1, int B, int HW, int G,
                            float eps, const float* gamma, const float* beta, int silu, void* y,
                            float* part, int nchunk, int pair, void* stream);
+int lgd_groupnorm_splitk_f16(const LgdGemmDesc* gemm , int B, int HW, int G, float eps, const float* gamma,
+                             const float* beta, int silu, void* y, void* h_out, float* stats, void* stream);
 int lgd_groupnorm_bwd_f16(const void* gy, const void* x0, const void* x1, int c0, int c1, int B,
                           int HW, int G, const float* gamma, const float* beta, int silu,
                           const float* stats, void* gx0, void* gx1, float* part, int nchunk,
diff --git a/llm-groundeddiffusion_amd/_lib.py b/llm-groundeddiffusion_amd/_lib.py
--- a/llm-groundeddiffusion_amd/_lib.py
+++ b/llm-groundeddiffusion_amd/_lib.py
@@ -36,6 +36,7 @@
 
 
 EPI_GEGLU, EPI_OUT_F32, EPI_RES_F32, EPI_ROWNORM = 1, 2, 4, 8
+EPI_SPLITK_KEEP = 16
 PAIR_HALF, PAIR_DUP = 1, 2
 
 _P, _I, _L, _F = c_void_p, c_int, c_i64, c_float
@@ -49,6 +50,7 @@
     "lgd_conv_out_f16": [_P, _P, _P, _P, _I, _I, _I, _I, _F, _P],
     "lgd_groupnorm_f16": [_P, _P, _I, _I, _I, _I, _I, _F, _P, _P, _I, _P, _P, _I, _P, _P],
     "lgd_groupnorm_pair_f16": [_P, _P, _I, _I, _I, _I, _I, _F, _P, _P, _I, _P, _P, _I, _I, _P],
+    "lgd_groupnorm_splitk_f16": [C.POINTER(LgdGemmDesc), _I, _I, _I, _F, _P, _P, _I, _P, _P, _P, _P],
     "lgd_groupnorm_bwd_f16": [_P, _P, _P, _I, _I, _I, _I, _I, _P, _P, _I, _P, _P, _P, _P, _I, _I, _P],
     "lgd_layernorm_f16": [_P, _L, _P, _L, _I, _I, _F, _P, _P, _P, _I, _L, _L, _P],
     "lgd_layernorm_pair_f16": [_P, _L, _P, _L, _I, _I, _F, _P, _P, _P, _I, _L, _L, _I, _P],
diff --git a/llm-groundeddiffusion_amd/csrc/attn.hip b/llm-groundeddiffusion_amd/csrc/attn.hip
--- a/llm-groundeddiffusion_amd/csrc/attn.hip
+++ b/llm-groundeddiffusion_amd/csrc/attn.hip
@@ -1006,19 +1006,24 @@
 }
 
 void lgd_gn_set_fused_hw(int hw);
+int lgd_gn_get_fused_hw();
 void lgd_gn_set_slab(int on);
 void lgd_ln_set_stream(int on);
 void lgd_gn_set_apply_wgs(int n);
 
 static std::atomic<int> g_cfg_pair{1};
+static std::atomic<int> g_gn_splitk{1};
 
 extern "C" int lgd_get_option(const char* name) {
   if (name && !strcmp(name, "cfg_pair")) return g_cfg_pair.load(std::memory_order_relaxed);
+  if (name && !strcmp(name, "gn_splitk")) return g_gn_splitk.load(std::memory_order_relaxed);
+  if (name && !strcmp(name, "gn_fused")) return lgd_gn_get_fused_hw();
   return LGD_ERR_ARG;
 }
 
 extern "C" int lgd_set_option(const char* name, int value) {
   if (!name) return LGD_ERR_ARG;
+  if (!strcmp(name, "gn_splitk") && (value == 0 || value == 1)) { g_gn_splitk.store(value, std::memory_order_relaxed); return LGD_OK; }
   if (!strcmp(name, "cfg_pair") && (value == 0 || value == 1)) { g_cfg_pair.store(value, std::memory_order_relaxed); return LGD_OK; }
   if (!strcmp(name, "gn_fused") && value >= 0 && value <= 4096) { lgd_gn_set_fused_hw(value); return LGD_OK; }
   if (!strcmp(name, "gn_slab") && (value == 0 || value == 1)) { lgd_gn_set_slab(value); return LGD_OK; }
diff --git a/llm-groundeddiffusion_amd/csrc/gemm.hip b/llm-groundeddiffusion_amd/csrc/gemm.hip
--- a/llm-groundeddiffusion_amd/csrc/gemm.hip
+++ b/llm-groundeddiffusion_amd/csrc/gemm.hip
@@ -1,5 +1,6 @@
 #include "common.h"
 #include "../../include/lgd_hip.h"
+#include "gemm_epilogue.h"
 #include <map>
 #include <mutex>
 #include <utility>
@@ -21,54 +22,12 @@
 #endif
 };
 
-__device__ __forceinline__ float4 ld_bias4(const float* p, int n) {
-  return *reinterpret_cast<const float4*>(p + n);
-}
-
 __device__ __forceinline__ f32x4 rownorm4(const LgdGemmDesc& d, int m, int n_in, f32x4 v) {
   if (d.epi & LGD_EPI_ROWNORM) {
     const float2 st = *reinterpret_cast<const float2*>(d.rowstat + (long)m * 2);
     const float4 cs = *reinterpret_cast<const float4*>(d.colsum + n_in);
     v[0] = st.y * (v[0] - st.x * cs.x); v[1] = st.y * (v[1] - st.x * cs.y);
     v[2] = st.y * (v[2] - st.x * cs.z); v[3] = st.y * (v[3] - st.x * cs.w);
-  }
-  return v;
-}
-
-template <bool GEGLU>
-__device__ __forceinline__ f32x4 epilogue_value4(const LgdGemmDesc& d, long r_off, int m, int n_out, f32x4 v, f32x4 g,
-                                                 float4 bv, float4 bg, bool res_ready, half4_t res_pre) {
-  v[0] += bv.x; v[1] += bv.y; v[2] += bv.z; v[3] += bv.w;
-  if (GEGLU) {
-    g[0] += bg.x; g[1] += bg.y; g[2] += bg.z; g[3] += bg.w;
-#ifdef LGD_GEMM_ABLATION
-    if (d.epi & (1 << 16)) {
-#pragma unroll
-      for (int r = 0; r < 4; ++r) v[r] = v[r] * g[r];
-    } else
-#endif
-    {
-      const f32x2_t g01 = gelu2_f((f32x2_t){g[0], g[1]}), g23 = gelu2_f((f32x2_t){g[2], g[3]});
-      v[0] *= g01[0]; v[1] *= g01[1]; v[2] *= g23[0]; v[3] *= g23[1];
-    }
-  }
-  const float alpha = d.alpha;
-#pragma unroll
-  for (int r = 0; r < 4; ++r) v[r] *= alpha;
-  if (res_ready) {
-#pragma unroll
-    for (int r = 0; r < 4; ++r) v[r] += (float)res_pre[r];
-  } else if (d.res) {
-    if (d.epi & LGD_EPI_RES_F32) {
-      const float* rp = reinterpret_cast<const float*>(d.res) + r_off + (long)m * d.ldr + n_out;
-      float4 rv = *reinterpret_cast<const float4*>(rp);
-      v[0] += rv.x; v[1] += rv.y; v[2] += rv.z; v[3] += rv.w;
-    } else {
-      const half_t* rp = reinterpret_cast<const half_t*>(d.res) + r_off + (long)m * d.ldr + n_out;
-      half4_t rv = *reinterpret_cast<const half4_t*>(rp);
-#pragma unroll
-      for (int r = 0; r < 4; ++r) v[r] += (float)rv[r];
-    }
   }
   return v;
 }
@@ -91,16 +50,6 @@
     *reinterpret_cast<half4_t*>(cp) = o;
     if (c_dup) *reinterpret_cast<half4_t*>(cp + c_dup) = o;
   }
-}
-
-__device__ __forceinline__ float4 ld_bias_sum4(const LgdGemmDesc& d, int n) {
-  float4 b = make_float4(0.f, 0.f, 0.f, 0.f);
-  if (d.bias) b = ld_bias4(d.bias, n);
-  if (d.bias2) {
-    float4 b2 = ld_bias4(d.bias2, n);
-    b.x += b2.x; b.y += b2.y; b.z += b2.z; b.w += b2.w;
-  }
-  return b;
 }
 
 template <int MI, int NI>
@@ -1588,16 +1537,11 @@
     int m = (int)(idx / groups_per_row);
     int gcol = (int)(idx - (long)m * groups_per_row) * 4;
     int n_in = geglu ? (gcol / 16) * 32 + (gcol % 16) : gcol;
-    f32x4 v = {0.f, 0.f, 0.f, 0.f}, g = {0.f, 0.f, 0.f, 0.f};
-    for (int s = 0; s < d.splits; ++s) {
-      const float* p = ws + (long)s * d.M * d.N + (long)m * d.N + n_in;
-      float4 t = *reinterpret_cast<const float4*>(p);
-      v[0] += t.x; v[1] += t.y; v[2] += t.z; v[3] += t.w;
-      if (geglu) {
-        float4 u = *reinterpret_cast<const float4*>(p + 16);
-        g[0] += u.x; g[1] += u.y; g[2] += u.z; g[3] += u.w;
-      }
-    }
+    const long off = (long)m * d.N + n_in;
+    const long offs[2] = {off, geglu ? off + 16 : -1L};
+    f32x4 vg[2];
+    splitk_sum4<2>(ws, (long)d.M * d.N, d.splits, offs, vg);
+    f32x4 v = vg[0], g = vg[1];
     const float4 bv = ld_bias_sum4(d, n_in);
     v = rownorm4(d, m, n_in, v);
     if (geglu) {
@@ -1711,6 +1655,10 @@
       return nullptr;
   }
   if (d.splits > 1 && d.cnt && !(f & TILE_CNT)) return nullptr;
+  if ((d.epi & LGD_EPI_SPLITK_KEEP) &&
+      (d.splits < 2 || d.cnt || (d.epi & (LGD_EPI_GEGLU | LGD_EPI_OUT_F32 | LGD_EPI_RES_F32 | LGD_EPI_ROWNORM)) ||
+       d.nb_o * d.nb_i != 1 || d.alpha != 1.f || d.pair))
+    return nullptr;
   ga.c_dup = 0;
   if (d.pair) {
     if ((d.pair != LGD_PAIR_HALF && d.pair != LGD_PAIR_DUP) || d.splits != 1 || d.nb_o * d.nb_i != 1 || (d.M & 1))
@@ -1879,6 +1827,13 @@
 
 extern "C" int lgd_abi_version(void) { return LGD_ABI_VERSION; }
 
+bool lgd_gemm_kept_partials(const LgdGemmDesc& desc, LgdGemmDesc& out) {
+  GemmArgs ga;
+  if (!(desc.epi & LGD_EPI_SPLITK_KEEP) || !gemm_check(desc, ga)) return false;
+  out = ga.d;
+  return true;
+}
+
 extern "C" int lgd_gemm_check(const LgdGemmDesc* desc) {
   GemmArgs ga;
   return desc && gemm_check(*desc, ga) ? LGD_OK : LGD_ERR_ARG;
@@ -1904,7 +1859,7 @@
     }
   }
   int rc = launch_tile(*t, ga, st);
-  if (rc || d.splits == 1 || d.cnt) return rc;
+  if (rc || d.splits == 1 || d.cnt || (d.epi & LGD_EPI_SPLITK_KEEP)) return rc;
   int n_out = (d.epi & LGD_EPI_GEGLU) ? d.N / 2 : d.N;
   long total = (long)d.M * (n_out / 4);
   int blocks = (int)((total + 255) / 256);
diff --git a/llm-groundeddiffusion_amd/csrc/gemm_epilogue.h b/llm-groundeddiffusion_amd/csrc/gemm_epilogue.h
--- /dev/null
+++ b/llm-groundeddiffusion_amd/csrc/gemm_epilogue.h
@@ -0,0 +1,78 @@
+#pragma once
+#include "common.h"
+#include "../../include/lgd_hip.h"
+
+__device__ __forceinline__ float4 ld_bias4(const float* p, int n) {
+  return *reinterpret_cast<const float4*>(p + n);
+}
+
+template <bool GEGLU>
+__device__ __forceinline__ f32x4 epilogue_value4(const LgdGemmDesc& d, long r_off, int m, int n_out, f32x4 v, f32x4 g,
+                                                 float4 bv, float4 bg, bool res_ready, half4_t res_pre) {
+  v[0] += bv.x; v[1] += bv.y; v[2] += bv.z; v[3] += bv.w;
+  if (GEGLU) {
+    g[0] += bg.x; g[1] += bg.y; g[2] += bg.z; g[3] += bg.w;
+#ifdef LGD_GEMM_ABLATION
+    if (d.epi & (1 << 16)) {
+#pragma unroll
+      for (int r = 0; r < 4; ++r) v[r] = v[r] * g[r];
+    } else
+#endif
+    {
+      const f32x2_t g01 = gelu2_f((f32x2_t){g[0], g[1]}), g23 = gelu2_f((f32x2_t){g[2], g[3]});
+      v[0] *= g01[0]; v[1] *= g01[1]; v[2] *= g23[0]; v[3] *= g23[1];
+    }
+  }
+  const float alpha = d.alpha;
+#pragma unroll
+  for (int r = 0; r < 4; ++r) v[r] *= alpha;
+  if (res_ready) {
+#pragma unroll
+    for (int r = 0; r < 4; ++r) v[r] += (float)res_pre[r];
+  } else if (d.res) {
+    if (d.epi & LGD_EPI_RES_F32) {
+      const float* rp = reinterpret_cast<const float*>(d.res) + r_off + (long)m * d.ldr + n_out;
+      float4 rv = *reinterpret_cast<const float4*>(rp);
+      v[0] += rv.x; v[1] += rv.y; v[2] += rv.z; v[3] += rv.w;
+    } else {
+      const half_t* rp = reinterpret_cast<const half_t*>(d.res) + r_off + (long)m * d.ldr + n_out;
+      half4_t rv = *reinterpret_cast<const half4_t*>(rp);
+#pragma unroll
+      for (int r = 0; r < 4; ++r) v[r] += (float)rv[r];
+    }
+  }
+  return v;
+}
+
+__device__ __forceinline__ float4 ld_bias_sum4(const LgdGemmDesc& d, int n) {
+  float4 b = make_float4(0.f, 0.f, 0.f, 0.f);
+  if (d.bias) b = ld_bias4(d.bias, n);
+  if (d.bias2) {
+    float4 b2 = ld_bias4(d.bias2, n);
+    b.x += b2.x; b.y += b2.y; b.z += b2.z; b.w += b2.w;
+  }
+  return b;
+}
+
+template <int NV, int SU = 1>
+__device__ __forceinline__ void splitk_sum4(const float* ws, long slab, int splits, const long (&off)[NV], f32x4 (&v)[NV]) {
+#pragma unroll
+  for (int j = 0; j < NV; ++j) v[j] = (f32x4){0.f, 0.f, 0.f, 0.f};
+  for (int s0 = 0; s0 < splits; s0 += SU) {
+    float4 t[SU][NV];
+#pragma unroll
+    for (int k = 0; k < SU; ++k) {
+      const float* p = ws + (long)(s0 + k) * slab;
+#pragma unroll
+      for (int j = 0; j < NV; ++j)
+        if (s0 + k < splits && off[j] >= 0) t[k][j] = *reinterpret_cast<const float4*>(p + off[j]);
+    }
+#pragma unroll
+    for (int k = 0; k < SU; ++k)
+#pragma unroll
+      for (int j = 0; j < NV; ++j)
+        if (s0 + k < splits && off[j] >= 0) {
+          v[j][0] += t[k][j].x; v[j][1] += t[k][j].y; v[j][2] += t[k][j].z; v[j][3] += t[k][j].w;
+        }
+  }
+}
diff --git a/llm-groundeddiffusion_amd/csrc/norm.hip b/llm-groundeddiffusion_amd/csrc/norm.hip
--- a/llm-groundeddiffusion_amd/csrc/norm.hip
+++ b/llm-groundeddiffusion_amd/csrc/norm.hip
@@ -1,5 +1,6 @@
 #include "common.h"
 #include "../../include/lgd_hip.h"
+#include "gemm_epilogue.h"
 
 namespace {
 
@@ -200,12 +201,13 @@
   }
 }
 
-template <int MAXP>
+template <int MAXP, bool SK = false>
 __global__ __launch_bounds__(256) void gn_fused_kernel(const half_t* __restrict__ x0, const half_t* __restrict__ x1,
                                                         int c0, int c1, int HW, int G, float eps,
                                                         const float* __restrict__ gamma, const float* __restrict__ beta,
                                                         int silu, half_t* __restrict__ y, float* stats, int kg,
-                                                        long y_dup) {
+                                                        long y_dup, const LgdGemmDesc sk = LgdGemmDesc(),
+                                                        half_t* __restrict__ h_out = nullptr) {
   __shared__ float s_part[256 * 8];
   __shared__ float s_ch[256];
   __shared__ float s_g[8][2];
@@ -221,11 +223,41 @@
   const int cc = second ? c - c0 : c;
   const int ld = second ? c1 : c0;
   half8_t h[MAXP];
-#pragma unroll
-  for (int u = 0; u < MAXP; ++u) {
-    const int pp = plane + u * pl;
-    h[u] = (active && pp < HW) ? *reinterpret_cast<const half8_t*>(src + ((long)b * HW + pp) * ld + cc)
-                               : (half8_t){0, 0, 0, 0, 0, 0, 0, 0};
+  if constexpr (SK) {
+    long off[2 * MAXP];
+#pragma unroll
+    for (int u = 0; u < MAXP; ++u) {
+      const int pp = plane + u * pl;
+      const bool ok = active && pp < HW;
+      off[2 * u] = ok ? ((long)b * HW + pp) * C + c : -1L;
+      off[2 * u + 1] = ok ? off[2 * u] + 4 : -1L;
+    }
+    f32x4 v[2 * MAXP];
+    splitk_sum4<2 * MAXP, 4>(sk.ws, (long)sk.M * sk.N, sk.splits, off, v);
+    float4 bias[2] = {make_float4(0.f, 0.f, 0.f, 0.f), make_float4(0.f, 0.f, 0.f, 0.f)};
+    if (active) { bias[0] = ld_bias_sum4(sk, c); bias[1] = ld_bias_sum4(sk, c + 4); }
+#pragma unroll
+    for (int u = 0; u < MAXP; ++u) {
+      h[u] = (half8_t){0, 0, 0, 0, 0, 0, 0, 0};
+      if (off[2 * u] >= 0) {
+        const int m = b * HW + plane + u * pl;
+#pragma unroll
+        for (int q = 0; q < 2; ++q) {
+          const f32x4 e = epilogue_value4<false>(sk, 0, m, c + 4 * q, v[2 * u + q], v[2 * u + q], bias[q], bias[q], false,
+                                                 (half4_t){0, 0, 0, 0});
+#pragma unroll
+          for (int r = 0; r < 4; ++r) h[u][4 * q + r] = (half_t)e[r];
+        }
+        if (h_out) *reinterpret_cast<half8_t*>(h_out + off[2 * u]) = h[u];
+      }
+    }
+  } else {
+#pragma unroll
+    for (int u = 0; u < MAXP; ++u) {
+      const int pp = plane + u * pl;
+      h[u] = (active && pp < HW) ? *reinterpret_cast<const half8_t*>(src + ((long)b * HW + pp) * ld + cc)
+                                 : (half8_t){0, 0, 0, 0, 0, 0, 0, 0};
+    }
   }
   auto group_sum = [&](const float (&v)[8], int slot) {
 #pragma unroll
@@ -927,6 +959,7 @@
 }
 
 void lgd_gn_set_fused_hw(int hw) { g_gn_fused_hw = hw; }
+int lgd_gn_get_fused_hw() { return g_gn_fused_hw; }
 void lgd_ln_set_stream(int on) { g_ln_stream = on; }
 void lgd_gn_set_slab(int on) { g_gn_slab = on; }
 void lgd_gn_set_apply_wgs(int n) { g_gn_apply_wgs = n; }
@@ -971,6 +1004,34 @@
   return lgd_check_launch();
 }
 
+bool lgd_gemm_kept_partials(const LgdGemmDesc& desc, LgdGemmDesc& out);
+
+extern "C" int lgd_groupnorm_splitk_f16(const LgdGemmDesc* gemm, int B, int HW, int G, float eps, const float* gamma,
+                                        const float* beta, int silu, void* y, void* h_out, float* stats, void* stream) {
+  (void)hipGetLastError();
+  LgdGemmDesc d;
+  if (!gemm || !y || B < 1 || HW < 1 || G < 1 || !lgd_gemm_kept_partials(*gemm, d)) return LGD_ERR_ARG;
+  const int C = d.N;
+  if ((long)B * HW != d.M || G > 64 || C > GN_MAXC || (C % G) || (C % 8)) return LGD_ERR_ARG;
+  if (d.res && ((d.ldr % 4) || (reinterpret_cast<uintptr_t>(d.res) & 7))) return LGD_ERR_ARG;
+  if (reinterpret_cast<uintptr_t>(y) & 15 || reinterpret_cast<uintptr_t>(h_out) & 15) return LGD_ERR_ARG;
+  const int cpg = C / G;
+  int kg = 1;
+  while ((kg * cpg) % 8) kg *= 2;
+  const int W = kg * cpg, nv = W / 8;
+  if (!(HW <= g_gn_fused_hw && kg <= 8 && (G % kg) == 0 && W <= 256)) return LGD_ERR_UNSUPPORTED;
+  const int pl = 256 / nv, npx = (HW + pl - 1) / pl;
+  if (npx > 4) return LGD_ERR_UNSUPPORTED;
+  hipStream_t st = reinterpret_cast<hipStream_t>(stream);
+#define GN_FUSED_SK(P)                                                                                              \
+  hipLaunchKernelGGL((gn_fused_kernel<P, true>), dim3(G / kg, B), dim3(256), 0, st, (const half_t*)nullptr,            \
+                     (const half_t*)nullptr, C, 0, HW, G, eps, gamma, beta, silu, (half_t*)y, stats, kg, 0L, d,       \
+                     (half_t*)h_out)
+  GN_FUSED_SK(4);
+#undef GN_FUSED_SK
+  return lgd_check_launch();
+}
+
 extern "C" int lgd_groupnorm_f16(const void* x0, const void* x1, int c0, int c1, int B, int HW,
                                  int G, float eps, const float* gamma, const float* beta, int silu,
                                  void* y, float* part, int nchunk, float* stats, void* stream) {
diff --git a/llm-groundeddiffusion_amd/ops.py b/llm-groundeddiffusion_amd/ops.py
--- a/llm-groundeddiffusion_amd/ops.py
+++ b/llm-groundeddiffusion_amd/ops.py
@@ -4,7 +4,7 @@
 import torch
 
 from . import _lib
-from ._lib import EPI_GEGLU, EPI_OUT_F32, EPI_RES_F32, EPI_ROWNORM, PAIR_DUP, PAIR_HALF, LgdGemmDesc
+from ._lib import EPI_GEGLU, EPI_OUT_F32, EPI_RES_F32, EPI_ROWNORM, EPI_SPLITK_KEEP, PAIR_DUP, PAIR_HALF, LgdGemmDesc
 
 F16, F32 = torch.float16, torch.float32
 
@@ -300,6 +300,8 @@
             flops *= 0.5
         m_in, m_out = (desc.M // 2 if desc.pair else desc.M), (desc.M // 2 if desc.pair == PAIR_HALF else desc.M)
         nbytes = 2.0 * nb * (m_in * desc.K / max(desc.taps, 1) + desc.N * desc.K + m_out * desc.N)
+        if desc.epi & EPI_SPLITK_KEEP:
+            nbytes -= 2.0 * m_out * desc.N
         return PROFILER.wrap(TILE_NAMES.get(desc.tile, "gemm"), flops, nbytes,
                              lambda: _call("lgd_gemm_f16", C.byref(desc), _stream()), tag,
                              shape=f"{shape_key(desc)} splits={desc.splits}")
@@ -433,6 +435,37 @@
     _prof("groupnorm (gn_stats + gn_apply | gn_fused)", 6.0 * B * HW * C_,
           lambda: _call("lgd_groupnorm_f16", _p(x), _p(x1), c0, c1, B, HW, G, float(eps), _p(gamma), _p(beta),
                         1 if silu else 0, _p(out), _p(part), nchunk, _p(stats), _stream()), shape=f"B{B}_HW{HW}_C{C_}")
+    return out
+
+
+def gemm_keep_partials(d) -> bool:
+    prev, d.epi = d.epi, d.epi | EPI_SPLITK_KEEP
+    if not gemm_accepts(d):
+        d.epi = prev
+        return False
+    return True
+
+
+def gn_splitk_accepts(HW, C, G) -> bool:
+    if C % G or C % 8:
+        return False
+    cpg, kg = C // G, 1
+    while (kg * cpg) % 8:
+        kg *= 2
+    W = kg * cpg
+    if not (HW <= get_option("gn_fused") and kg <= 8 and G % kg == 0 and W <= 256):
+        return False
+    pl = 256 // (W // 8)
+    return (HW + pl - 1) // pl <= 4
+
+
+def groupnorm_splitk(desc, B, HW, G, eps, gamma, beta, silu, *, out, h_out=None, stats=None):
+    C_ = desc.N
+    nbytes = B * HW * C_ * (4.0 * desc.splits + (2.0 if desc.res else 0.0) + (2.0 if h_out is not None else 0.0) + 2.0)
+    _prof("groupnorm_splitk (gn_fused over split-K partials)", nbytes,
+          lambda: _call("lgd_groupnorm_splitk_f16", C.byref(desc), B, HW, G, float(eps), _p(gamma), _p(beta),
+                        1 if silu else 0, _p(out), _p(h_out), _p(stats), _stream()),
+          shape=f"B{B}_HW{HW}_C{C_} splits={desc.splits}")
     return out
 
 
diff --git a/llm-groundeddiffusion_amd/unet.py b/llm-groundeddiffusion_amd/unet.py
--- a/llm-groundeddiffusion_amd/unet.py
+++ b/llm-groundeddiffusion_amd/unet.py
@@ -15,13 +15,14 @@
 
 
 class Act:
-    __slots__ = ("t", "g", "rows", "C", "pair")
+    __slots__ = ("t", "g", "rows", "C", "pair", "splitk")
 
     def __init__(self, t):
         self.t = t
         self.g = None
         self.rows, self.C = t.shape
         self.pair = None
+        self.splitk = None
 
 
 class PairMode:
@@ -56,8 +57,11 @@
 class Plan:
     def __init__(self, eng: "UNetEngine", B: int, L: int, *, grad: bool, fuser: bool,
                  stop_key: Optional[Tuple] = None, save_keys: Sequence[Tuple] = (),
-                 text_batch_offset: int = 0, obj_batch_offset: int = 0, pair_shared: bool = False):
+                 text_batch_offset: int = 0, obj_batch_offset: int = 0, pair_shared: bool = False,
+                 gn_splitk: bool = True):
         self.eng, self.B, self.L = eng, B, L
+        self.gn_splitk = bool(gn_splitk)
+        self.gn_splitk_ops = 0
         self.pair_shared = bool(pair_shared)
         self._pair = False
         self.pair_ops = 0
@@ -175,6 +179,7 @@
                                         lda0=c0, lda1=c1, taps=9, hin=H, win=H, hout=H, wout=H, bias=b,
                                         bias2=row[temb_off:temb_off + Cout], ldc=Cout))
             fwd = lambda: [ops.gemm_launch(dd) for dd in ds]
+            splitk = None
         else:
             bias2 = eng.temb_cur[0, temb_off:temb_off + Cout] if temb_off is not None else None
             d = ops.gemm_desc(x.t, W, y.t, M, Cout, K, a1=x1.t if x1 else None, c0=c0, c1=c1, lda0=c0,
@@ -183,8 +188,11 @@
                               ldr=res.C if res else 0, ldc=Cout)
             self._pair_op([x, x1, res], y, half, d)
             fwd = lambda: ops.gemm_launch(d)
+            splitk = d if self.gn_splitk and d.splits > 1 and not d.pair else None
         if not self.grad:
             self._add(fwd)
+            if splitk is not None:
+                y.splitk = (self.ops[-1], splitk)
             return y
         Wd = self.eng.w.h[f"{name}.wd"]
         gouts = [x] + ([x1] if x1 else []) + ([res] if res else [])
@@ -217,6 +225,8 @@
                     runs.append(lambda: ops.copy_(res.g, y.g))
             return lambda: [r() for r in runs]
         self._add(fwd, make_bwd, gouts, passthrough=(res, y) if res is not None else None)
+        if splitk is not None:
+            y.splitk = (self.ops[-1], splitk)
         return y
 
     def shortcut(self, x: Act, x1: Optional[Act], name: str) -> Act:
@@ -246,7 +256,8 @@
         self._add(fwd, make_bwd, gouts)
         return y
 
-    def groupnorm(self, x: Act, x1: Optional[Act], name: str, HW: int, eps: float, silu: bool, half=False) -> Act:
+    def groupnorm(self, x: Act, x1: Optional[Act], name: str, HW: int, eps: float, silu: bool, half=False,
+                  sole_reader=False) -> Act:
         eng, B = self.eng, self.B
         G = eng.cfg.norm_num_groups
         gm, bt = eng.w.f[f"{name}.g"], eng.w.f[f"{name}.b"]
@@ -257,7 +268,14 @@
         stats = self._alloc((B, G, 2)) if self.grad else None
         xt1 = x1.t if x1 else None
         pm = self._pair_op([x, x1], y, half)
-        if pm is not None:
+        keep = x.splitk is not None and x1 is None and pm is None and x.splitk[0] is self.ops[-1] \
+            and ops.gn_splitk_accepts(HW, C, G) and ops.gemm_keep_partials(x.splitk[1])
+        if keep:
+            dk = x.splitk[1]
+            h_out = x.t if (self.grad or not sole_reader) else None
+            self.gn_splitk_ops += 1
+            fwd = lambda: ops.groupnorm_splitk(dk, B, HW, G, eps, gm, bt, silu, out=y.t, h_out=h_out, stats=stats)
+        elif pm is not None:
             fwd = lambda: ops.groupnorm(x.t, B, HW, G, eps, gm, bt, silu, x1=xt1, out=y.t, part=part, pair=pm.mode)
         else:
             fwd = lambda: ops.groupnorm(x.t, B, HW, G, eps, gm, bt, silu, x1=xt1, out=y.t, part=part, stats=stats)
@@ -408,7 +426,7 @@
         HW = H * H
         h = self.groupnorm(x, skip, f"{r.prefix}.norm1", HW, eps, True, half=True)
         h = self.conv(h, f"{r.prefix}.conv1", H, temb_off=eng.w.temb_offsets[r.prefix], half=True)
-        h = self.groupnorm(h, None, f"{r.prefix}.norm2", HW, eps, True, half=True)
+        h = self.groupnorm(h, None, f"{r.prefix}.norm2", HW, eps, True, half=True, sole_reader=True)
         if r.shortcut:
             sc = self.shortcut(x, skip, f"{r.prefix}.conv_shortcut")
         else:
@@ -738,15 +756,16 @@
              text_batch_offset=0, obj_batch_offset=0, pair_shared=False) -> Plan:
         mode = self.tuning_mode or ops.current_tuning_mode()
         pair_shared = bool(pair_shared and not grad and B % 2 == 0 and self.temb_rows == 1 and ops.get_option("cfg_pair"))
+        gn_splitk = bool(ops.get_option("gn_splitk"))
         key = (B, L, grad, fuser, tuple(stop_key) if stop_key else None, tuple(map(tuple, save_keys)),
-               text_batch_offset, obj_batch_offset, mode, self.fold_ln, pair_shared)
+               text_batch_offset, obj_batch_offset, mode, self.fold_ln, pair_shared, gn_splitk)
         if B + text_batch_offset > self.max_text_batch:
             raise RuntimeError(f"plan batch {B} (+{text_batch_offset}) exceeds max_text_batch={self.max_text_batch}")
         if key not in self._plans:
             with ops.tuning(mode):
                 self._plans[key] = Plan(self, B, L, grad=grad, fuser=fuser, stop_key=stop_key,
                                         save_keys=save_keys, text_batch_offset=text_batch_offset,
-                                        obj_batch_offset=obj_batch_offset, pair_shared=pair_shared)
+                                        obj_batch_offset=obj_batch_offset, pair_shared=pair_shared, gn_splitk=gn_splitk)
             while len(self._plans) > self.MAX_PLANS:
                 self._plans.popitem(last=False)
         self._plans.move_to_end(key)
```

After: 1.827 images/s. Within noise of the previous version (-0.5%).
